# lab-cosmo/torch-pme

Hardware: AMD Instinct MI355X
Metric: atom-steps/sec (energy+forces) (higher is better)
Workload: dtype f32

## Files before the change

torch-pme_amd/csrc/api.hip:

```cpp
#include <dlfcn.h>

#include <cmath>
#include <cstring>
#include <map>
#include <string>
#include <vector>

#include "host.h"

namespace mipme {

static thread_local char g_error[512] = "";

static thread_local const char* g_last_cosched = "";
void note_cosched_kernel(const char* name) { g_last_cosched = name ? name : ""; }
static thread_local int g_last_slot_fill = 0;
void note_slot_fill(int rider_atoms) { g_last_slot_fill = rider_atoms; }
static thread_local int g_last_cell_riders = 0;
void note_cell_riders(int n) { g_last_cell_riders = n; }
void set_error(const char* fmt, ...) {
  va_list ap;
  va_start(ap, fmt);
  vsnprintf(g_error, sizeof(g_error), fmt, ap);
  va_end(ap);
// ... 572 lines not shown
      qv[u] = i < n ? q[i] : T(0);
    }
#pragma unroll
    for (int u = 0; u < kMatchUnroll; ++u) {
      const double v = fabs(double(qv[u]));
      if (v > best) {
        best = v;
        bi = base + u * stride;
      }
    }
  }
#pragma unroll
  for (int off = 32; off > 0; off >>= 1) {
    const double ov = __shfl_xor(best, off, 64);
    const long long oi = __shfl_xor(bi, off, 64);
    if (ov > best || (ov == best && oi < bi)) { best = ov; bi = oi; }
  }
  if (lane == 0) { s_val[wave] = best; s_idx[wave] = bi; }
  __syncthreads();
  if (threadIdx.x == 0) {
    for (int w = 1; w < int(blockDim.x >> 6); ++w)
      if (s_val[w] > s_val[0] || (s_val[w] == s_val[0] && s_idx[w] < s_idx[0])) { s_val[0] = s_val[w]; s_idx[0] = s_idx[w]; }
  }
  __syncthreads();
  const long long k = s_idx[0];
  const bool usable = s_val[0] > 0.0;
  const T scale = usable ? g[k] / q[k] : T(0);
  const double sd = double(scale);
  const double tol = 8.0 * (sizeof(T) == 4 ? 1.1920929e-7 : 2.220446049250313e-16);
  int bad = (usable && isfinite(sd)) ? 0 : 1;
  for (int64_t base = threadIdx.x; base < n; base += stride * kMatchUnroll) {
    T qv[kMatchUnroll], gv[kMatchUnroll];
#pragma unroll
    for (int u = 0; u < kMatchUnroll; ++u) {
      const int64_t i = base + u * stride;
      qv[u] = i < n ? q[i] : T(0);
      gv[u] = i < n ? g[i] : T(0);
    }
#pragma unroll
    for (int u = 0; u < kMatchUnroll; ++u) {
      const double e = sd * double(qv[u]);
      if (!(fabs(double(gv[u]) - e) <= tol * fabs(e))) bad = 1;
    }
  }
  bad = __any(bad) ? 1 : 0;
  if (lane == 0) s_bad[wave] = bad;
  __syncthreads();
  if (threadIdx.x == 0) {
    int any = 0;
    for (int w = 0; w < int(blockDim.x >> 6); ++w) any |= s_bad[w];
    result[0] = scale;
    result[1] = any ? T(0) : T(1);
    if (host_flag) __hip_atomic_store(host_flag, any ? 0 : 1, __ATOMIC_RELEASE, __HIP_MEMORY_SCOPE_SYSTEM);
  }
}

template <typename T>
__global__ __launch_bounds__(64) void values_equal_kernel(int n, const T* __restrict__ a, const T* __restrict__ b, int* host_flag) {
  bool same = true;
  for (int i = threadIdx.x; i < n; i += 64) same = same && (a[i] == b[i]);
  const bool all = __builtin_amdgcn_ballot_w64(!same) == 0;
  if (threadIdx.x == 0) __hip_atomic_store(host_flag, all ? 1 : 0, __ATOMIC_RELEASE, __HIP_MEMORY_SCOPE_SYSTEM);
}

__device__ __forceinline__ void checksum_words(const uint4 v, unsigned j, unsigned long long& a, unsigned long long& b) {
  constexpr unsigned C1 = 0x9e3779b1u, C2 = 0x85ebca6bu;
  const unsigned k1 = (j + 1u) * C1, k2 = (j + 1u) * C2;
  a += (unsigned long long)v.x * k1 + (unsigned long long)v.y * (k1 + C1) + (unsigned long long)v.z * (k1 + 2u * C1) +
       (unsigned long long)v.w * (k1 + 3u * C1);
  b += (unsigned long long)v.x * k2 + (unsigned long long)v.y * (k2 + C2) + (unsigned long long)v.z * (k2 + 2u * C2) +
       (unsigned long long)v.w * (k2 + 3u * C2);
}

static constexpr int kChecksumBlocks = 256;

__global__ __launch_bounds__(256) void checksum_kernel(const uint4* __restrict__ data, int64_t n_vec, const unsigned* __restrict__ tail,
                                                       int n_tail, unsigned long long* __restrict__ sums,
                                                       const unsigned long long* __restrict__ expect, int* host_flag) {
  unsigned long long a = 0, b = 0;
  const int64_t stride = int64_t(gridDim.x) * blockDim.x;
  int64_t i = int64_t(blockIdx.x) * blockDim.x + threadIdx.x;
  for (; i + 7 * stride < n_vec; i += 8 * stride) {
    uint4 v[8];
#pragma unroll
    for (int u = 0; u < 8; ++u) v[u] = data[i + u * stride];
#pragma unroll
    for (int u = 0; u < 8; ++u) checksum_words(v[u], unsigned(4 * (i + u * stride)), a, b);
  }
  for (; i < n_vec; i += stride) checksum_words(data[i], unsigned(4 * i), a, b);
  if (blockIdx.x == 0 && int(threadIdx.x) < n_tail) {
    const unsigned j = unsigned(4 * n_vec) + threadIdx.x;
    a += (unsigned long long)tail[threadIdx.x] * ((j + 1u) * 0x9e3779b1u);
    b += (unsigned long long)tail[threadIdx.x] * ((j + 1u) * 0x85ebca6bu);
  }
  __shared__ unsigned long long red[4][2];
  __shared__ bool last;
  auto block_sum = [&](unsigned long long& x, unsigned long long& y) {
#pragma unroll
    for (int off = 32; off > 0; off >>= 1) {
      x += __shfl_xor(x, off, 64);
      y += __shfl_xor(y, off, 64);
    }
    __syncthreads();
    if ((threadIdx.x & 63) == 0) {
      red[threadIdx.x >> 6][0] = x;
      red[threadIdx.x >> 6][1] = y;
    }
    __syncthreads();
    x = red[0][0] + red[1][0] + red[2][0] + red[3][0];
    y = red[0][1] + red[1][1] + red[2][1] + red[3][1];
  };
  block_sum(a, b);
  unsigned long long* part = sums + 3;
  if (threadIdx.x == 0) {
    __hip_atomic_store(&part[2 * blockIdx.x], a, __ATOMIC_RELAXED, __HIP_MEMORY_SCOPE_AGENT);
    __hip_atomic_store(&part[2 * blockIdx.x + 1], b, __ATOMIC_RELAXED, __HIP_MEMORY_SCOPE_AGENT);
    last = __hip_atomic_fetch_add(&sums[2], 1ull, __ATOMIC_ACQ_REL, __HIP_MEMORY_SCOPE_AGENT) == (unsigned long long)(gridDim.x - 1);
  }
  __syncthreads();
  if (!last) return;
  unsigned long long ta = 0, tb = 0;
  for (unsigned k = threadIdx.x; k < gridDim.x; k += blockDim.x) {
    ta += __hip_atomic_load(&part[2 * k], __ATOMIC_RELAXED, __HIP_MEMORY_SCOPE_AGENT);
    tb += __hip_atomic_load(&part[2 * k + 1], __ATOMIC_RELAXED, __HIP_MEMORY_SCOPE_AGENT);
  }
  block_sum(ta, tb);
  if (threadIdx.x == 0) {
    const unsigned long long s0 = sums[0] + ta, s1 = sums[1] + tb;
    sums[0] = s0;
    sums[1] = s1;
    sums[2] = 0;
    if (host_flag) {
      const int same = expect && s0 == expect[0] && s1 == expect[1];
      __hip_atomic_store(host_flag, same ? 1 : 0, __ATOMIC_RELEASE, __HIP_MEMORY_SCOPE_SYSTEM);
    }
  }
}

template <typename T>
__global__ __launch_bounds__(256) void energy_select_kernel(int64_t N, const T* __restrict__ verdict, const T* __restrict__ q,
                                                           const T* __restrict__ force, const T* __restrict__ field, T f,
                                                           T* __restrict__ grad_mesh, T* __restrict__ grad_pair) {
  if (verdict[1] != T(1)) return;
  const T s = verdict[0];
  for (int64_t t = int64_t(blockIdx.x) * blockDim.x + threadIdx.x; t < 3 * N; t += int64_t(gridDim.x) * blockDim.x) {
    const T sq = s * q[t / 3];
    if (grad_mesh) grad_mesh[t] = sq * field[t];
    if (grad_pair) grad_pair[t] = sq * f * force[t];
  }
}

template <typename T>
__global__ __launch_bounds__(256) void energy_select_sum_kernel(int64_t N, const T* __restrict__ verdict, const T* __restrict__ q,
                                                               const T* __restrict__ force, const T* __restrict__ field, T f,
                                                               const T* grad_mesh, const T* grad_pair, T* out) {
  const bool match = verdict[1] == T(1);
  const T s = verdict[0];
  for (int64_t t = int64_t(blockIdx.x) * blockDim.x + threadIdx.x; t < 3 * N; t += int64_t(gridDim.x) * blockDim.x)
    out[t] = match ? s * q[t / 3] * (f * force[t] + field[t]) : grad_mesh[t] + grad_pair[t];
}

template <typename T>
__global__ __launch_bounds__(256) void energy_select_contract_kernel(int64_t N, const T* __restrict__ verdict,
                                                                    const T* __restrict__ tail_q, T* grad_q,
                                                                    const T* __restrict__ tail_cell, int cell_off,
                                                                    const T* cell_mesh, const T* cell_pair, T* grad_cell) {
  const bool match = verdict[1] == T(1);
  const T s = verdict[0];
  if (grad_cell && blockIdx.x == 0 && threadIdx.x < 9) {
    const int i = threadIdx.x;
    grad_cell[i] = match ? s * tail_cell[cell_off + i] : cell_mesh[i] + (cell_pair ? cell_pair[i] : T(0));
  }
  if (!grad_q || !match) return;
  const T h = T(0.5) * s;
  for (int64_t t = int64_t(blockIdx.x) * blockDim.x + threadIdx.x; t < N; t += int64_t(gridDim.x) * blockDim.x)
    grad_q[t] = h * tail_q[t];
}

static double axis_length(const mipme_mesh_t* m, int axis) {
  const double* a = m->cell + 3 * axis;
  return std::sqrt(a[0] * a[0] + a[1] * a[1] + a[2] * a[2]);
}

template <typename T>
static int slab_forward_t(hipStream_t st, int axis, const mipme_mesh_t* m, double pref, int64_t N, const void* pos,
                          const void* q, void* moments, void* pot) {
  if (N == 0) return MIPME_OK;
  const int C = m->n_channels;
  const double c0 = pref * 4.0 * 3.14159265358979323846 / m->volume;
  slab_moments_kernel<T><<<1, 1024, 0, st>>>(axis, N, C, (const T*)pos, (const T*)q, (const T*)nullptr, (double*)moments);
  MIPME_LAUNCH_CHECK();
  slab_forward_kernel<T><<<unsigned((N + 255) / 256), 256, 0, st>>>(axis, N, C, c0, axis_length(m, axis), (const T*)pos,
                                                                    (const double*)moments, (T*)pot);
  MIPME_LAUNCH_CHECK();
  return MIPME_OK;
}

template <typename T>
static int slab_backward_t(hipStream_t st, int axis, const mipme_mesh_t* m, double pref, int64_t N, const void* pos,
                           const void* q, const void* g, void* moments, void* grad_pos, void* grad_q, void* grad_cell) {
  if (N == 0) return MIPME_OK;
  const int C = m->n_channels;
  const double c0 = pref * 4.0 * 3.14159265358979323846 / m->volume;
  const double Lz = axis_length(m, axis);
  slab_moments_kernel<T><<<1, 1024, 0, st>>>(axis, N, C, (const T*)pos, (const T*)q, (const T*)g, (double*)moments);
  MIPME_LAUNCH_CHECK();
  if (grad_pos || grad_q) {
    slab_backward_kernel<T><<<unsigned((N + 255) / 256), 256, 0, st>>>(
        axis, N, C, c0, Lz, (const T*)pos, (const T*)q, (const T*)g, (const double*)moments, (T*)grad_pos, (T*)grad_q);
    MIPME_LAUNCH_CHECK();
  }
  if (grad_cell) {
    slab_cell_kernel<T><<<1, 64, 0, st>>>(axis, C, *m, c0, Lz, (const double*)moments, (T*)grad_cell);
    MIPME_LAUNCH_CHECK();
  }
  return MIPME_OK;
}

}

template <typename A>
static int load_args(const A* in, A& out, const char* what) {
  MIPME_REQUIRE(in != nullptr, "%s: NULL argument struct", what);
  MIPME_REQUIRE(in->version == MIPME_ARGS_VERSION, "%s: argument struct version %u, library expects %u", what, in->version,
                unsigned(MIPME_ARGS_VERSION));
  MIPME_REQUIRE(in->size >= 16 && in->size <= 4096, "%s: implausible argument struct size %u", what, in->size);
  memset(&out, 0, sizeof(A));
  memcpy(&out, in, in->size < sizeof(A) ? in->size : sizeof(A));
  return MIPME_OK;
}


using namespace mipme;

static int check_slab(int slab, const mipme_mesh_t* mesh, const mipme_potential_t* pot, bool has_tail, const char* who) {
  if (!slab) return MIPME_OK;
  MIPME_REQUIRE(slab >= 1 && slab <= 3, "%s: slab must be 0 (off) or the non-periodic axis + 1, got %d", who, slab);
  MIPME_REQUIRE(mesh->n_channels == 1, "%s: the slab term of the gather tail serves one channel, the mesh has %d (use "
                "mipme_slab_forward / mipme_slab_backward)", who, int(mesh->n_channels));
  MIPME_REQUIRE(has_tail, "%s: slab rides on the gather tail (out_energy, out_grad_positions); without it use mipme_slab_forward", who);
  MIPME_REQUIRE(pot && (pot->kind == MIPME_COULOMB || pot->exponent == 1), "%s: the slab term exists for 1/r only", who);
  return MIPME_OK;
}

static int md_check(const mipme_md_args_t* in, mipme_md_args_t& a, const char* who) {
  MIPME_REQUIRE(in && in->size >= 16 && in->version == 1, "%s: NULL or unversioned argument struct", who);
  std::memset(&a, 0, sizeof(a));
  std::memcpy(&a, in, std::min<size_t>(in->size, sizeof(a)));
  int rc;
  if ((rc = validate_mesh(a.mesh))) return rc;
  MIPME_REQUIRE(a.dtype == MIPME_F32 || a.dtype == MIPME_F64, "invalid dtype %d", a.dtype);
  MIPME_REQUIRE(a.pot && a.pot->smearing > 0, "Must specify smearing to use a potential with PMECalculator");
  MIPME_REQUIRE(live_supported(a.mesh, a.n_atoms, a.dtype), "%s: mesh / atom count outside the live-bin kernels' range", who);
  MIPME_REQUIRE(a.records && a.atom_bins && a.live_lists, "%s: NULL buffer", who);
  return MIPME_OK;
}

template <typename T>
static int md_step_t(const mipme_md_args_t& a) {
  int rc;
  hipStream_t st = (hipStream_t)a.stream;
  const mipme_mesh_t* m = a.mesh;
  double self_c, bg_c;
  correction_terms(a.pot, self_c, bg_c);
  fft_plan_begin_step(a.plan);
  mipme_sr_job_t job{};
  job.n_atoms = a.n_atoms;
  job.row_ptr = a.row_ptr;
  job.entries_shift = a.words;
  job.entries = a.words;
  job.positions = nullptr;
  job.cell = a.cell;
  job.charges = nullptr;
  job.pot = a.pot;
  job.full_list = 0;
  job.shift_format = a.shift_format;
  job.records = const_cast<void*>(a.records);
  job.out = a.potentials;
  job.force = a.pair_force;
  job.dist_out = nullptr;
  GatherTailHost tail{};
  tail.force = a.pair_force;
  tail.force_scale = 1.0;
  tail.seed = a.grad_seed;
  tail.grad_pos = a.grad_positions;
  tail.energy = a.energy;
  if ((rc = tail_attach_plan_scratch(tail, a.plan))) return rc;
  CellWork cw{};
  if (a.grad_cell) {
    cw = cell_work_layout(m, a.n_atoms, a.cell_work);
    tail.rpart = cw.rpart;
  }
  tail.grad_q = a.grad_charges;
  tail.aux_seed = a.aux_seed;
  tail.live_flags = a.host_flags;
  if (a.slab) {
    tail_attach_slab(tail, m, a.pot, a.slab);
    STAGE(st, "slab_moments", slab_moments_blocks<T>(st, a.n_atoms, (const T*)a.records + (a.slab - 1), 4, (const T*)a.records + 3, 4,
                                                     tail.slab_mom));
  }
  if (a.energy_log && (rc = tail_attach_energy_log(tail, a.energy_log, a.energy_log_cursor, a.energy_log_capacity,
                                                   "energy_log needs energy_log_cursor")))
    return rc;
  STAGE(st, "spread+rspace_forward", live_spread<T>(st, m, a.n_atoms, a.records, a.atom_bins, a.live_lists, a.rho_mesh, &job, a.host_flags,
                                                     a.grad_cell ? cw.cwave : nullptr));
  int64_t n_sr_part = 0;
  const void* sr_part = bins_epart(m, a.n_atoms, a.dtype, a.atom_bins, &n_sr_part);
  const ConvCell cc{a.G_deriv, cw.cwave, cw.n_waves, cw.wbuf, cw.rows, int(cw.n_riders), nullptr, nullptr, nullptr, nullptr};
  STAGE(st, "convolve_xfused", convolve_xfused(a.plan, st, a.rho_mesh, a.G, a.hat_work, a.phi_mesh, a.dc, 0, m, a.pot, nullptr,
                                               const_cast<void*>(tail.epart_k), sr_part, n_sr_part, nullptr, a.nan_flag,
                                               a.grad_cell ? &cc : nullptr));
  STAGE(st, "gather+energy+forces",
        live_gather<T>(st, m, a.n_atoms, a.records, a.atom_bins, a.live_lists, a.phi_mesh, a.dc, self_c, bg_c, a.potentials, nullptr,
                       &tail, a.nan_flag));
  if (a.grad_cell)
    STAGE(st, "cell_finalize",
          cell_tail_finalize_impl<T>(st, m, bg_c, 0.5, cw.n_riders, cw.n_bricks, cw.rows, cw.rpart, a.dc,
                                     a.aux_seed ? a.aux_seed : a.grad_seed, a.grad_cell, &tail));
  return MIPME_OK;
}


template <typename T>
static int scaled_match_wide_t(hipStream_t st, int64_t n, const void* g, const void* q, void* result, void* host_flag, void* work) {
  const int64_t nb = (n + 1024 * kMatchRegs - 1) / (1024 * kMatchRegs);
  MIPME_REQUIRE(nb < (int64_t(1) << 24), "mipme_scaled_match_wide: too many values");
  scaled_match_small_kernel<T, true><<<unsigned(nb), 1024, 0, st>>>(n, (const T*)g, (const T*)q, nullptr, nullptr, (double*)work);
  MIPME_LAUNCH_CHECK();
  scaled_match_combine_kernel<T><<<1, 256, 0, st>>>(int(nb), (const double*)work, (T*)result, (int*)host_flag);
  MIPME_LAUNCH_CHECK();
  return MIPME_OK;
}

extern "C" {

const char* mipme_last_error(void) { return g_error; }
const char* mipme_last_cosched_kernel(void) { return g_last_cosched; }
int mipme_last_slot_fill(void) { return g_last_slot_fill; }
int mipme_last_cell_riders(void) { return g_last_cell_riders; }
int mipme_version(void) { return MIPME_VERSION; }

int mipme_fft_plan_create(int dtype, int nx, int ny, int nz, int batch, mipme_fft_plan** out) {
  return fft_plan_create(dtype, nx, ny, nz, batch, out);
}
int mipme_fft_plan_destroy(mipme_fft_plan* plan) { return fft_plan_destroy(plan); }

int mipme_kfilter_build(void* stream, int dtype, const mipme_mesh_t* mesh, const mipme_potential_t* pot, void* G) {
  int rc = validate_mesh(mesh);
  if (rc) return rc;
  MIPME_REQUIRE(G != nullptr, "G is NULL");
  hipStream_t st = (hipStream_t)stream;
  DT_SWITCH(dtype, kfilter_build_impl<float>(st, mesh, pot, G), kfilter_build_impl<double>(st, mesh, pot, G));
}

int mipme_kfilter_build_deriv(void* stream, int dtype, const mipme_mesh_t* mesh, const mipme_potential_t* pot, void* G_deriv) {
  int rc = validate_mesh(mesh);
  if (rc) return rc;
  MIPME_REQUIRE(G_deriv != nullptr, "G_deriv is NULL");
  hipStream_t st = (hipStream_t)stream;
  DT_SWITCH(dtype, kfilter_deriv_impl<float>(st, mesh, pot, G_deriv), kfilter_deriv_impl<double>(st, mesh, pot, G_deriv));
}

int64_t mipme_cell_tail_work(const mipme_fft_plan* plan, const mipme_mesh_t* mesh, int64_t n_atoms) {
  if (!plan || !mesh || validate_mesh(mesh) || n_atoms < 0) return 0;
  return cell_work_layout(mesh, n_atoms, nullptr).total;
}

int mipme_convolve(mipme_fft_plan* plan, void* stream, const void* mesh_in, const void* G, void* hat_out, void* hat_work,
                   void* mesh_out, void* dc_out) {
  TraceRange _tr("mipme_convolve");
  MIPME_REQUIRE(plan != nullptr, "FFT plan is NULL");
  MIPME_REQUIRE(mesh_in && G && hat_out && hat_work && mesh_out, "NULL buffer passed to mipme_convolve");
  hipStream_t st = (hipStream_t)stream;
  const FftDims d = fft_plan_dims(plan);
  const int64_t Mh = int64_t(d.nx) * d.ny * (d.nz / 2 + 1);
  int rc;
  if ((rc = fft_forward(plan, st, mesh_in, hat_out))) return rc;
  if (d.dtype == MIPME_F32)
    rc = apply_filter_impl<float>(st, Mh, d.batch, hat_out, G, hat_work, dc_out);
  else
    rc = apply_filter_impl<double>(st, Mh, d.batch, hat_out, G, hat_work, dc_out);
  if (rc) return rc;
  return fft_inverse(plan, st, hat_work, mesh_out);
}

int mipme_spread(void* stream, int dtype, const mipme_mesh_t* mesh, int64_t n_atoms, const void* positions,
                 const void* values, void* mesh_out) {
  TraceRange _tr("mipme_spread");
  int rc = validate_mesh(mesh);
  if (rc) return rc;
  MIPME_REQUIRE(n_atoms >= 0 && mesh_out && (n_atoms == 0 || (positions && values)), "NULL buffer passed to mipme_spread");
  hipStream_t st = (hipStream_t)stream;
  DT_SWITCH(dtype, spread_impl<float>(st, mesh, n_atoms, positions, values, 1.0, mesh_out),
            spread_impl<double>(st, mesh, n_atoms, positions, values, 1.0, mesh_out));
}

int mipme_gather(void* stream, int dtype, const mipme_mesh_t* mesh, int64_t n_atoms, const void* positions,
                 const void* mesh_in, void* out) {
  TraceRange _tr("mipme_gather");
  int rc = validate_mesh(mesh);
  if (rc) return rc;
  MIPME_REQUIRE(n_atoms >= 0 && mesh_in && (n_atoms == 0 || (positions && out)), "NULL buffer passed to mipme_gather");
  hipStream_t st = (hipStream_t)stream;
  DT_SWITCH(dtype, gather_impl<float>(st, mesh, n_atoms, positions, mesh_in, out),
            gather_impl<double>(st, mesh, n_atoms, positions, mesh_in, out));
}

int mipme_kspace_forward(const mipme_kspace_forward_args_t* args_in) {
  TraceRange _tr("mipme_kspace_forward");
  mipme_kspace_forward_args_t a;
  int rc = load_args(args_in, a, "mipme_kspace_forward");
  if (rc) return rc;
  if ((rc = validate_mesh(a.mesh))) return rc;
  if ((rc = check_slab(a.slab, a.mesh, a.pot, a.out_energy && a.out_grad_positions, "mipme_kspace_forward"))) return rc;
  if ((rc = check_plan(a.plan, a.dtype, a.mesh))) return rc;
  const mipme_mesh_t* mesh = a.mesh;
  MIPME_REQUIRE(a.pot && a.pot->smearing > 0, "Must specify smearing to use a potential with PMECalculator");
  MIPME_REQUIRE(a.G && a.rho_mesh && a.hat_work && a.phi_mesh && a.dc, "NULL work buffer passed to mipme_kspace_forward");
  MIPME_REQUIRE(a.rho_hat || fft_plan_xfused(a.plan), "rho_hat may only be NULL for plans with a power-of-two nx");
  MIPME_REQUIRE(!a.out_cell_partials || !a.rho_hat, "out_cell_partials is produced by the fused convolution (rho_hat == NULL)");
  MIPME_REQUIRE(!a.out_rho_hat || (!a.rho_hat && mesh->n_channels == 1),
                "out_rho_hat is written by the fused convolution (rho_hat == NULL) of a single-channel mesh");
  MIPME_REQUIRE(a.n_atoms == 0 || (a.positions && a.charges && a.out_lr), "NULL atom buffer passed to mipme_kspace_forward");
  MIPME_REQUIRE(!a.atom_bins || bricks_supported(mesh, a.dtype), "atom bins passed for a mesh the brick kernels do not support");
  MIPME_REQUIRE(!a.out_field || (a.atom_bins && mesh->n_channels == 1), "out_field needs atom bins and a single channel");
  MIPME_REQUIRE(!a.out_records || (a.atom_bins && mesh->n_channels == 1), "out_records needs atom bins and a single channel");
  if (a.sr_job) {
    MIPME_REQUIRE(a.atom_bins && a.out_records && mesh->n_channels == 1 && a.accumulate_out && !a.gather_wait_event,
                  "sr_job needs atom bins, out_records, a single channel and accumulate_out = 1 without a wait event");
    MIPME_REQUIRE(a.sr_job->n_atoms == a.n_atoms && a.sr_job->records == a.out_records && a.sr_job->out == a.out_lr,
                  "sr_job must describe the atoms, records and output of the same call");
    MIPME_REQUIRE(a.sr_job->row_ptr && a.sr_job->entries_shift && a.sr_job->entries && a.sr_job->positions &&
                      a.sr_job->charges && a.sr_job->pot, "NULL buffer in sr_job");
  }
  GatherTailHost tail{}, *tp = nullptr;
  if (a.out_energy || a.out_grad_positions) {
    MIPME_REQUIRE(a.out_energy && a.out_grad_positions && a.sr_job && a.sr_job->force && a.out_field && a.n_atoms > 0,
                  "the gather tail (out_energy, out_grad_positions) needs both outputs, sr_job with force sums and out_field");
    tail.force = a.sr_job->force;
    tail.force_scale = a.sr_job->full_list ? 0.5 : 1.0;
    tail.seed = a.grad_seed;
    tail.grad_pos = a.out_grad_positions;
    tail.energy = a.out_energy;
    MIPME_REQUIRE(!a.rho_hat && mesh->n_channels == 1 && sr_job_fusable(a.sr_job),
                  "the gather tail needs the fused convolution (rho_hat == NULL), one channel and a co-schedulable sr_job");
    if ((rc = tail_attach_plan_scratch(tail, a.plan))) return rc;
    tp = &tail;
  }
  if (a.energy_log && (rc = tail_attach_energy_log(tail, a.energy_log, tp ? a.energy_log_cursor : nullptr, a.energy_log_capacity,
                                                   "energy_log rides on the gather tail (out_energy, out_grad_positions) and "
                                                   "needs energy_log_cursor")))
    return rc;
  if (a.out_grad_charges || a.out_grad_cell) {
    MIPME_REQUIRE(tp, "out_grad_charges / out_grad_cell ride on the gather tail (out_energy, out_grad_positions)");
    MIPME_REQUIRE(!a.out_grad_charges || !a.sr_job->full_list || (a.sr_job->shift_format & MIPME_ROWS_PADDED),
                  "out_grad_charges = 2 s V needs a half list (a full list need not be symmetric)");
    tail.grad_q = a.out_grad_charges;
    tail.aux_seed = a.aux_seed;
    if (a.out_grad_cell) {
      const int p = a.pot->kind == MIPME_COULOMB ? 1 : a.pot->exponent;
      MIPME_REQUIRE(a.G_deriv && a.cell_work, "out_grad_cell needs G_deriv (mipme_kfilter_build_deriv) and cell_work");
      MIPME_REQUIRE((a.sr_job->shift_format & 0xff) == 2 && !a.sr_job->dist_out && (p == 1 || p == 6),
                    "out_grad_cell needs 4-byte entries (shift_format 2), no dist_out, and 1/r or 1/r^6");
      MIPME_REQUIRE(!a.out_cell_partials, "out_grad_cell replaces out_cell_partials");
      tail.rpart = cell_work_layout(mesh, a.n_atoms, a.cell_work).rpart;
      tail.records = a.out_records;
    }
  }
  if (a.slab) {
    tail_attach_slab(tail, mesh, a.pot, a.slab);
    tail.records = a.out_records;
  }
  DT_SWITCH(a.dtype, kspace_forward_t<float>(a, tp), kspace_forward_t<double>(a, tp));
}

int mipme_md_supported(const mipme_mesh_t* mesh, const mipme_potential_t* pot, int64_t n_atoms, int dtype) {
  if (!mesh || !pot || validate_mesh(mesh) || pot->smearing <= 0 || pot->exclusion_radius > 0) return 0;
  const int p = pot->kind == MIPME_COULOMB ? 1 : pot->exponent;
  if (p != 1 && p != 6) return 0;
  if (mesh->nx < 2 || (mesh->nx & (mesh->nx - 1))) return 0;
  return live_supported(mesh, n_atoms, dtype) ? 1 : 0;
}

int64_t mipme_md_lists_ints(const mipme_mesh_t* mesh, int64_t n_atoms) {
  if (!mesh || validate_mesh(mesh) || n_atoms <= 0) return 0;
  return live_lists_ints(mesh, n_atoms);
}

int mipme_md_rebin(const mipme_md_args_t* args_in) {
  TraceRange _tr("mipme_md_rebin");
  mipme_md_args_t a;
  int rc = md_check(args_in, a, "mipme_md_rebin");
  if (rc) return rc;
  hipStream_t st = (hipStream_t)a.stream;
  DT_SWITCH(a.dtype, live_rebin<float>(st, a.mesh, a.n_atoms, a.records, a.atom_bins, a.live_lists, a.host_flags),
            live_rebin<double>(st, a.mesh, a.n_atoms, a.records, a.atom_bins, a.live_lists, a.host_flags));
}

int mipme_md_step(const mipme_md_args_t* args_in) {
  TraceRange _tr("mipme_md_step");
  mipme_md_args_t a;
  int rc = md_check(args_in, a, "mipme_md_step");
  if (rc) return rc;
  if ((rc = check_plan(a.plan, a.dtype, a.mesh))) return rc;
  MIPME_REQUIRE(fft_plan_xfused(a.plan), "mipme_md_step needs a plan with a power-of-two nx");
  MIPME_REQUIRE(mipme_md_supported(a.mesh, a.pot, a.n_atoms, a.dtype), "mipme_md_step: potential / mesh outside its range");
  MIPME_REQUIRE(a.cell && a.G && a.rho_mesh && a.hat_work && a.phi_mesh && a.dc && a.row_ptr && a.words && a.potentials &&
                    a.pair_force && a.energy && a.grad_positions, "NULL buffer passed to mipme_md_step");
  MIPME_REQUIRE((a.shift_format & 0xff) == 2, "mipme_md_step reads 4-byte entries (shift_format 2, with or without MIPME_ROWS_PADDED)");
  if ((rc = check_slab(a.slab, a.mesh, a.pot, true, "mipme_md_step"))) return rc;
  if (a.grad_cell) {
    const int p = a.pot->kind == MIPME_COULOMB ? 1 : a.pot->exponent;
    MIPME_REQUIRE(a.G_deriv && a.cell_work, "grad_cell needs G_deriv (mipme_kfilter_build_deriv) and cell_work");
    MIPME_REQUIRE(p == 1 || p == 6, "grad_cell: the pair kernels form the cell sums for 1/r and 1/r^6");
  }
  DT_SWITCH(a.dtype, md_step_t<float>(a), md_step_t<double>(a));
}

int mipme_kspace_backward(const mipme_kspace_backward_args_t* args_in) {
  TraceRange _tr("mipme_kspace_backward");
  mipme_kspace_backward_args_t a;
  int rc = load_args(args_in, a, "mipme_kspace_backward");
  if (rc) return rc;
  if ((rc = validate_mesh(a.mesh))) return rc;
  if ((rc = check_plan(a.plan, a.dtype, a.mesh))) return rc;
  MIPME_REQUIRE(a.pot && a.pot->smearing > 0, "Must specify smearing to use a potential with PMECalculator");
  MIPME_REQUIRE(a.G && a.phi_mesh && (a.grad_scale || (a.psi_mesh && a.hat_work && a.chi_mesh && a.dc)),
                "NULL work buffer passed to mipme_kspace_backward");
  MIPME_REQUIRE(a.grad_scale || a.psi_hat || ((!a.grad_cell || a.G_deriv) && fft_plan_xfused(a.plan)),
                "psi_hat may only be NULL for plans with a power-of-two nx, and with a cell gradient only together with G_deriv");
  MIPME_REQUIRE(a.n_atoms == 0 || (a.positions && a.charges && a.grad_out), "NULL atom buffer passed to mipme_kspace_backward");
  MIPME_REQUIRE(!a.atom_bins || bricks_supported(a.mesh, a.dtype), "atom bins passed for a mesh the brick kernels do not support");
  DT_SWITCH(a.dtype, kspace_backward_t<float>(a), kspace_backward_t<double>(a));
}

int mipme_fft_plan_xfused(const mipme_fft_plan* plan) { return plan && fft_plan_xfused(plan) ? 1 : 0; }

int64_t mipme_fft_plan_kgrid_blocks(const mipme_fft_plan* plan) { return plan ? xconv_blocks(plan) : 0; }

int mipme_fft_r2c(mipme_fft_plan* plan, void* stream, int dtype, const mipme_mesh_t* mesh, const void* mesh_in, void* hat) {
  int rc = validate_mesh(mesh);
  if (rc) return rc;
  if ((rc = check_plan(plan, dtype, mesh))) return rc;
  MIPME_REQUIRE(mesh_in && hat, "NULL buffer passed to mipme_fft_r2c");
  return fft_forward(plan, (hipStream_t)stream, mesh_in, hat);
}

int mipme_plane_spread_parts(const mipme_mesh_t* mesh, int64_t n_atoms, int dtype) {
  if (!mesh || validate_mesh(mesh) || !bricks_supported(mesh, dtype)) return 0;
  if (mesh->nx < 2 || (mesh->nx & (mesh->nx - 1)) || plane_bins_capacity(mesh, n_atoms, dtype) <= 0) return 0;
  return plane_bands(mesh, dtype) > 1 ? 1 : plane_spread_parts_setting();
}

int64_t mipme_atom_bins_bytes(const mipme_mesh_t* mesh, int64_t n_atoms, int dtype) {
  if (!mesh || n_atoms < 0) return 0;
  return bins_bytes(mesh, n_atoms, dtype);
}

int mipme_profile_enable(int on) {
  for (auto& e : g_prof) {
    (void)hipEventDestroy(e.a);
    (void)hipEventDestroy(e.b);
  }
  g_prof.clear();
  g_prof_on = on != 0;
  return MIPME_OK;
}

int64_t mipme_profile_report(char* buf, int64_t buflen) {
  std::map<std::string, std::pair<long, double>> agg;
  for (auto& e : g_prof) {
    float ms = 0.f;
    if (hipEventSynchronize(e.b) == hipSuccess && hipEventElapsedTime(&ms, e.a, e.b) == hipSuccess) {
      auto& a = agg[e.name];
      a.first += 1;
      a.second += ms / float(e.reps > 0 ? e.reps : 1);
    }
  }
  std::string out;
  char line[256];
  for (auto& kv : agg) {
    snprintf(line, sizeof(line), "%s %ld %.6f\n", kv.first.c_str(), kv.second.first, kv.second.second);
    out += line;
  }
  if (buf && buflen > 0) {
    const size_t n = out.size() < size_t(buflen - 1) ? out.size() : size_t(buflen - 1);
    memcpy(buf, out.data(), n);
    buf[n] = 0;
  }
  return int64_t(out.size());
}

int64_t mipme_cellgrad_partials_size(const mipme_mesh_t* mesh, int64_t n_atoms) {
  (void)n_atoms;
  if (!mesh) return 0;
  const int64_t xmax = int64_t(mesh->ny) * (mesh->nz / 2 + 1) * mesh->n_channels;
  const int64_t Mh = int64_t(mesh->nx) * mesh->ny * (mesh->nz / 2 + 1);
  const int64_t fused = 37 * 256 + Mh;
  return std::max<int64_t>(12 * std::max<int64_t>(cellgrad_blocks(mesh), xmax), fused) + cellgrad_scratch_doubles();
}

int mipme_slab_forward(void* stream, int dtype, int axis, const mipme_mesh_t* mesh, double prefactor, int64_t n_atoms,
                       const void* positions, const void* charges, void* moments, void* pot) {
  MIPME_REQUIRE(mesh && axis >= 0 && axis < 3 && moments, "invalid arguments to mipme_slab_forward");
  hipStream_t st = (hipStream_t)stream;
  DT_SWITCH(dtype, slab_forward_t<float>(st, axis, mesh, prefactor, n_atoms, positions, charges, moments, pot),
            slab_forward_t<double>(st, axis, mesh, prefactor, n_atoms, positions, charges, moments, pot));
}
// ... 282 lines not shown
```

torch-pme_amd/csrc/bricks_device.h:

```cpp
#ifndef MIPME_BRICKS_DEVICE_H
#define MIPME_BRICKS_DEVICE_H
#include <algorithm>
#include <cmath>
#include <cstdlib>

#include <rocprim/device/device_radix_sort.hpp>

#include "host.h"
#include <map>
#include <utility>

#include "rows_body.h"
#include "fft_lds.h"

namespace mipme {

static constexpr int BRICK = 8;
static constexpr int BRICK_PTS = BRICK * BRICK * BRICK;

#define MIPME_SGPR_CAP __attribute__((amdgpu_num_sgpr(80)))
static inline int spread_stage_rows(int order, size_t real_bytes);
static inline size_t spread_row_reals(int, size_t) { return 3 * BRICK; }

struct BrickGeom {
// ... 784 lines not shown
            w1[2][t] = wr[N + t];
          }
          const T v = (args.qs ? args.qs[si] : val[int64_t(orig) * C + c]) * scale;
          const int r3[3] = {rz, rx, ry};
#if MIPME_STAGE_SELECT
#pragma unroll
          for (int ax = 0; ax < 3; ++ax) {
#pragma unroll
            for (int k = 0; k < BRICK; ++k) {
              T w = T(0);
#pragma unroll
              for (int t = 0; t < N; ++t) w = (k - r3[ax] == t) ? w1[ax][t] : w;
              dst[ax * BRICK + k] = ax == 1 ? w * v : w;
            }
          }
#else
#pragma unroll
          for (int k = 0; k < SW; ++k) dst[k] = T(0);
#pragma unroll
          for (int ax = 0; ax < 3; ++ax) {
#pragma unroll
            for (int t = 0; t < N; ++t) {
              const int k = r3[ax] + t;
              if (unsigned(k) < unsigned(BRICK)) dst[ax * BRICK + k] = ax == 1 ? w1[ax][t] * v : w1[ax][t];
            }
          }
#endif
        } else if (PAD_ROWS && tid < nst + PAD_ROWS) {
          T* dst = stage + tid * SW;
#pragma unroll
          for (int k = 0; k < SW; ++k) dst[k] = T(0);
        }
        __syncthreads();
        MIPME_WG_PHASE(3);
        constexpr int UC = MIPME_SPREAD_UC;
        const int nstc = __builtin_amdgcn_readfirstlane(nst);
        const int wave_u = __builtin_amdgcn_readfirstlane(wave);
        for (int sv0 = wave_u; sv0 < nstc; sv0 += WAVES * UC) {
#if MIPME_SPREAD_PADROWS
          T wz[UC][BRICK], fx[UC], fy[UC];
          const T* sw = stage + sv0 * SW;
#pragma unroll
          for (int u = 0; u < UC; ++u) {
            const T* su = sw + u * WAVES * SW;
            fx[u] = su[BRICK + px];
            fy[u] = su[2 * BRICK + py];
            load_row8<T>(su, wz[u]);
          }
#pragma unroll
          for (int u = 0; u < UC; ++u) fma_row8<T>(acc, fx[u] * fy[u], wz[u]);
#else
          T wxy[UC], wz[UC][BRICK], fx[UC], fy[UC];
          bool live[UC];
#pragma unroll
          for (int u = 0; u < UC; ++u) {
            const int sv = sv0 + u * WAVES;
            live[u] = sv < nstc;
            const T* sw = stage + (live[u] ? sv : sv0) * SW;
            fx[u] = sw[BRICK + px];
            fy[u] = sw[2 * BRICK + py];
            load_row8<T>(sw, wz[u]);
          }
#pragma unroll
          for (int u = 0; u < UC; ++u) {
            wxy[u] = live[u] ? fx[u] * fy[u] : T(0);
            fma_row8<T>(acc, wxy[u], wz[u]);
          }
#endif
        }
        __syncthreads();
      }
    }
    MIPME_WG_PHASE(4);
#pragma unroll
    for (int pz = 0; pz < BRICK; ++pz) part[wave * BRICK_PTS + (px * BRICK + py) * BRICK + pz] = acc[pz];
    __syncthreads();
    for (int k = tid; k < BRICK_PTS; k += THREADS) {
      T v = T(0);
#pragma unroll
      for (int w = 0; w < WAVES; ++w) v += part[w * BRICK_PTS + k];
      const int qx = k / (BRICK * BRICK), qy = (k / BRICK) % BRICK, qz = k % BRICK;
      const int gx = ox + qx, gy = oy + qy, gz = oz + qz;
      if (gx < g.nx && gy < g.ny && gz < g.nz) mesh[c * M + gx * plane + int64_t(gy) * g.nz + gz] = v;
    }
    __syncthreads();
    MIPME_WG_PHASE(5);
  }
}

template <int N, typename T>
__global__ __launch_bounds__(SPREAD_THREADS) void spread_brick_kernel(SpreadArgs<T> a) {
  MIPME_SKIP_IF_SET(a.skip);
  const unsigned b = brick_of(a.bg, blockIdx.x);
  if (b < unsigned(a.bg.nb)) spread_brick_body<N, T>(a, b);
}
template <int N, typename T>
__global__ __launch_bounds__(SPREAD_THREADS_SPARSE) void spread_brick_sparse_kernel(SpreadArgs<T> a) {
  MIPME_SKIP_IF_SET(a.skip);
  const unsigned b = brick_of(a.bg, blockIdx.x);
  if (b < unsigned(a.bg.nb)) spread_brick_body<N, T, SPREAD_THREADS_SPARSE>(a, b);
}


static constexpr unsigned kBrickPatternMin = 2048;
struct CoSlot {
  bool brick;
  unsigned slot;
};
__host__ __device__ inline unsigned cosched_periods(unsigned n_pad, unsigned n_rows_pad, unsigned a) {
  const unsigned nb8 = n_pad >> 3, nr8 = n_rows_pad >> 3, need = (nr8 + a - 1) / a;
  return nb8 < need ? nb8 : need;
}
__host__ __device__ inline unsigned cosched_grid(unsigned n_pad, unsigned n_rows_pad, unsigned a) {
  if (a == 0) return n_pad + n_rows_pad;
  const unsigned P = cosched_periods(n_pad, n_rows_pad, a);
  const unsigned left_b = n_pad - 8u * P, rows_done = 8u * a * P;
  return P * 8u * (1u + a) + left_b + (n_rows_pad > rows_done ? n_rows_pad - rows_done : 0u);
}
__device__ __forceinline__ CoSlot cosched_slot(unsigned b, unsigned n_pad, unsigned n_rows_pad, unsigned a) {
  if (a == 0) return CoSlot{b < n_pad, b < n_pad ? b : b - n_pad};
  const unsigned P = cosched_periods(n_pad, n_rows_pad, a), period = 8u * (1u + a);
  if (b < P * period) {
    const unsigned p = b / period, r = b - p * period;
    return r < 8u ? CoSlot{true, 8u * p + r} : CoSlot{false, 8u * a * p + (r - 8u)};
  }
  const unsigned rest = b - P * period;
  return (n_pad >> 3) > P ? CoSlot{true, 8u * P + rest} : CoSlot{false, 8u * a * P + rest};
}

static inline unsigned brick_pattern(const BrickGeom& bg, unsigned n_spread, unsigned n_row_blocks, bool fp32) {
  static const int pattern_env = [] { const char* e = getenv("MIPME_BRICK_PATTERN"); return e ? atoi(e) : -1; }();
  unsigned pattern = 0;
  if (bg.xcd && n_spread > 0) {
    if (pattern_env >= 0)
      pattern = unsigned(pattern_env);
    else if (fp32 && n_spread >= kBrickPatternMin) {
      const double ratio = double(pad8(n_row_blocks)) / double(pad8(n_spread));
      const unsigned a = unsigned(ratio + 0.5);
      if (a >= 1 && std::fabs(ratio - double(a)) <= 0.15 * double(a)) pattern = a;
    }
  }
  return pattern;
}

template <typename T, int PFAST, bool COMPACT, bool CELL, int BS = SPREAD_THREADS>
__device__ __forceinline__ void cosched_row_block(const FusedRowsArgs<T>& ra, unsigned r, char* smem_rows) {
  AtomRecord<T>* tab = reinterpret_cast<AtomRecord<T>*>(smem_rows);
  bool done = false;
  if constexpr (COMPACT && std::is_same<T, float>::value) {
    if (CELL || !ra.dist_out) {
      sr_rows_pk_body<PFAST, BS, CELL>(ra, r, tab);
      done = true;
    }
  }
#if MIPME_ROW_LANES == 16
  if constexpr (COMPACT && std::is_same<T, double>::value && (PFAST == 1 || PFAST == 6)) {
    if (CELL || !ra.dist_out) {
      sr_rows_f64_body<BS, CELL, PFAST>(ra, r, smem_rows);
      done = true;
    }
  }
#endif
  if constexpr (!CELL) {
    if (!done) sr_fused_rows_body<T, kPotForce, false, PFAST, false, true, BS, 0, COMPACT>(ra, r, tab);
  }
}

template <int N, typename T, int PFAST, bool COMPACT, bool CELL>
__device__ __forceinline__ void spread_rows_body(const SpreadArgs<T>& sa, const FusedRowsArgs<T>& ra, unsigned n_spread,
                                                 unsigned pattern) {
  MIPME_WG_STAMP(0);
  const unsigned n_pad = sa.bg.xcd ? pad8(n_spread) : n_spread;
  const unsigned n_row_blocks = unsigned((ra.N + kRowsPerSpreadBlock - 1) / kRowsPerSpreadBlock);
  const unsigned n_rows_pad = sa.bg.xcd ? pad8(n_row_blocks) : n_row_blocks;
  const CoSlot cs = cosched_slot(blockIdx.x, n_pad, n_rows_pad, pattern);
  extern __shared__ __attribute__((aligned(16))) char smem_rows[];
  if (cs.brick) {
    const unsigned b = brick_of(sa.bg, cs.slot);
    if (cs.slot < n_pad && b < n_spread) spread_brick_body<N, T>(sa, b);
  } else if (cs.slot < n_rows_pad) {
    const unsigned r = sa.bg.xcd ? xcd_contiguous(cs.slot, n_row_blocks) : cs.slot;
    if (r < n_row_blocks) cosched_row_block<T, PFAST, COMPACT, CELL>(ra, r, smem_rows);
  }
#ifdef MIPME_WG_TIMELINE
  __syncthreads();
#endif
  MIPME_WG_STAMP(1);
}

template <int N, typename T, int PFAST, bool COMPACT, bool CELL = false>
__global__ __launch_bounds__(SPREAD_THREADS, (sizeof(T) == 4 && COMPACT) ? (CELL ? MIPME_CELL_WAVES : 6) : 1) void spread_rows_kernel(
    SpreadArgs<T> sa, FusedRowsArgs<T> ra, unsigned n_spread, unsigned pattern) {
  spread_rows_body<N, T, PFAST, COMPACT, CELL>(sa, ra, n_spread, pattern);
}
template <int N, typename T, int PFAST, bool COMPACT, bool CELL = false>
__global__ __launch_bounds__(SPREAD_THREADS, (sizeof(T) == 4 && COMPACT) ? (CELL ? MIPME_CELL_WAVES : 6) : 1) MIPME_SGPR_CAP void spread_rows_capped_kernel(
    SpreadArgs<T> sa, FusedRowsArgs<T> ra, unsigned n_spread, unsigned pattern) {
  spread_rows_body<N, T, PFAST, COMPACT, CELL>(sa, ra, n_spread, pattern);
}
template <int N, typename T, bool CELL>
constexpr bool spread_rows_sgpr_capped() {
#ifdef MIPME_SGPR_CAP_OFF
  return false;
#else
  return sizeof(T) == 4 && N == 5 && !CELL;
#endif
}

template <typename T, int PFAST, bool COMPACT, bool CELL = false>
__global__ __launch_bounds__(256) void rows_only_kernel(FusedRowsArgs<T> ra, int xcd) {
  constexpr bool F64_BODY = COMPACT && std::is_same<T, double>::value && (PFAST == 1 || PFAST == 6) && kRowLanes == 16;
  __shared__ __attribute__((aligned(16))) char tab_raw[F64_BODY ? kRowsF64LdsBytes : sizeof(AtomRecord<T>) * kShiftTableSize];
  AtomRecord<T>* tab = reinterpret_cast<AtomRecord<T>*>(tab_raw);
  constexpr int BS = 256;
  const unsigned n_row_blocks = unsigned((ra.N + BS / kRowLanes - 1) / (BS / kRowLanes));
  const unsigned r = xcd ? xcd_contiguous(blockIdx.x, n_row_blocks) : blockIdx.x;
  if (r >= n_row_blocks) return;
  if constexpr (COMPACT && std::is_same<T, float>::value) {
    if (CELL || !ra.dist_out) {
      sr_rows_pk_body<PFAST, BS, CELL>(ra, r, tab);
      return;
    }
  }
#if MIPME_ROW_LANES == 16
  if constexpr (F64_BODY) {
    if (CELL || !ra.dist_out) {
      sr_rows_f64_body<BS, CELL, PFAST>(ra, r, tab_raw);
      return;
    }
  }
#endif
  if constexpr (!CELL) sr_fused_rows_body<T, kPotForce, false, PFAST, false, true, BS, 0, COMPACT>(ra, r, tab);
}

template <typename T>
static inline bool rows_cell_supported(int pfast, int shift_format, const void* dist_out) {
  if ((shift_format & kShiftFormatMask) != kShiftTable32 || dist_out || kRowLanes != 16) return false;
  return pfast == 1 || pfast == 6;
}

template <typename T>
struct PlaneArgs {
  Cplx<T>* hat = nullptr;
  int logny = 0, loglz = 0;
  int tile_off = 0, tw_off = 0;
  int misc_off = 0;
  int parts = 1;
  Cplx<T>* hat_more = nullptr;
  int64_t more_stride = 0;
  int band_rows = 0, bands = 1;
};

static constexpr size_t kPlaneLdsCosched = 39 * 1024;
static inline size_t plane_tile_bytes(int ny, int nz, size_t real_bytes) { return 2 * real_bytes * size_t(ny) * (size_t(nz / 2) + 1); }
static inline size_t plane_tw_bytes(int ny, int nz, size_t real_bytes) {
  const size_t Lz = size_t(nz / 2), Ltab = size_t(ny) > Lz ? size_t(ny) : Lz;
  return 2 * real_bytes * (Ltab / 2 + (Lz + 1));
}
template <typename T>
static inline void plane_lds_layout(int rows, int nz, PlaneArgs<T>& pa, size_t& total, bool ystage = true) {
  const size_t acc = sizeof(double) * size_t(rows) * nz, tile = plane_tile_bytes(rows, nz, sizeof(T));
  const size_t tile_off = sizeof(T) == 4 ? 0 : acc;
  const size_t tw_off = sizeof(T) == 4 ? (acc > tile ? acc : tile) : acc + tile;
  pa.tile_off = int(tile_off);
  pa.tw_off = int(tw_off);
  pa.misc_off = int(tw_off + plane_tw_bytes(ystage ? rows : 0, nz, sizeof(T)));
  total = size_t(pa.misc_off) + 640;
}
static inline int plane_band_rows(const mipme_mesh_t* m, int dtype) {
  static const bool bands_env = env_flag("MIPME_PLANE_BANDS", true);
  for (int rows = m->ny; rows >= 4 && rows * kPlaneSub >= m->ny; rows >>= 1) {
    size_t need = 0;
    if (dtype == MIPME_F32) {
      PlaneArgs<float> pa;
      plane_lds_layout<float>(rows, m->nz, pa, need, rows == m->ny);
    } else {
      PlaneArgs<double> pa;
      plane_lds_layout<double>(rows, m->nz, pa, need, rows == m->ny);
    }
    if (need <= kPlaneLdsCosched) return rows;
    if (!bands_env) break;
  }
  return 0;
}
static inline bool plane_fits_cosched(const mipme_mesh_t* m, int dtype) { return plane_band_rows(m, dtype) == m->ny; }

static inline bool sparse_bricks(int64_t n_atoms, int nb);
static int plane_list_capacity(const mipme_mesh_t* m, int64_t N, int dtype) {
  static const bool plane_env = env_flag("MIPME_PLANE_SPREAD", true);
  if (!plane_env || deterministic_mode() || m->n_channels != 1 || N <= 0) return 0;
  const bool pow2 = (m->ny & (m->ny - 1)) == 0 && (m->nz & (m->nz - 1)) == 0 && m->nz >= 4 && m->ny >= 2;
  if (!pow2 || m->nx < 2 * BRICK) return 0;
  if (m->nx > (1 << 11) || m->ny > (1 << kPlanePackBits) || m->nz > (1 << kPlanePackBits)) return 0;
  if (sparse_bricks(N, make_brick_geom(m).nb)) return 0;
  const int band_rows = plane_band_rows(m, dtype);
  if (band_rows == 0) return 0;
  if (band_rows < m->ny && m->ny / kPlaneSub < 8) return 0;
  const int64_t lists = int64_t(m->nx) * kPlaneSub, mean = (N + lists - 1) / lists, all = (N + 15) / 16 * 16;
  int64_t cap = (4 * mean + 32 + 15) / 16 * 16;
  if (cap > all) cap = all;
  return int(cap);
}

template <int N, typename T>
struct PlaneItem {
  T vx;
  int my, mz;
  T wy[N], wz[N];
};

template <int N, typename T>
struct PlaneRaw {
  T w[plane_entry_words<N, T>()];
};

template <int N, typename T>
__device__ __forceinline__ void plane_raw_load(PlaneRaw<N, T>& r, bool ok, const T* __restrict__ base, int64_t idx) {
  constexpr int EW = plane_entry_words<N, T>(), V = 16 / int(sizeof(T));
  struct alignas(16) Chunk {
    T e[V];
  };
  const Chunk* src = reinterpret_cast<const Chunk*>(base + (ok ? idx : 0) * EW);
#pragma unroll
  for (int k = 0; k < EW / V; ++k) {
    const Chunk c = src[k];
#pragma unroll
    for (int u = 0; u < V; ++u) r.w[k * V + u] = c.e[u];
  }
  if constexpr (!plane_entry_fat<N, T>()) {
#pragma unroll
    for (int t = 3; t < EW; ++t) r.w[t] = ok ? r.w[t] : T(0);
  }
}
template <typename T>
__device__ __forceinline__ int plane_raw_packed(T w0) {
  if constexpr (sizeof(T) == 4)
    return __float_as_int(w0);
  else
    return int(__double_as_longlong(w0));
}

template <int SCHEME, int N, typename T>
__device__ __forceinline__ void plane_item_make(PlaneItem<N, T>& it, const PlaneRaw<N, T>& r, int tt, T scale) {
  constexpr bool FAT = plane_entry_fat<N, T>();
  const int packed = plane_raw_packed(r.w[0]);
  it.my = (packed >> kPlanePackBits) & ((1 << kPlanePackBits) - 1);
  it.mz = packed & ((1 << kPlanePackBits) - 1);
  T qwx[N];
#pragma unroll
  for (int t = 0; t < N; ++t) qwx[t] = r.w[(FAT ? 1 : 3) + t];
  it.vx = pick<N, T>(qwx, tt) * scale;
  if constexpr (FAT) {
#pragma unroll
    for (int t = 0; t < N; ++t) {
      it.wy[t] = r.w[1 + N + t];
      it.wz[t] = r.w[1 + 2 * N + t];
    }
  } else {
    T unused[N];
    weights_1d<SCHEME, N, false, T>(r.w[1], it.wy, unused);
    weights_1d<SCHEME, N, false, T>(r.w[2], it.wz, unused);
  }
}

static constexpr unsigned kFxMagicHi = 0x43380000u;
template <int N, typename T, bool BANDED>
__device__ __forceinline__ void plane_item_scatter(double* __restrict__ acc, const Geom& g, const PlaneItem<N, T>& it, double fx_scale,
                                                   int row_lo, int rows) {
  constexpr int s0 = stencil_start<N>();
  int zo[N];
#pragma unroll
  for (int k = 0; k < N; ++k) zo[k] = wrap1(it.mz + s0 + k, g.nz);
#pragma unroll
  for (int j = 0; j < N; ++j) {
    int r = wrap1(it.my + s0 + j, g.ny);
    if constexpr (BANDED) {
      r -= row_lo;
      if (unsigned(r) >= unsigned(rows)) continue;
    }
    const int row = r * g.nz;
    const T ay = it.vx * it.wy[j];
#pragma unroll
    for (int k = 0; k < N; ++k) {
      if constexpr (sizeof(T) == 4) {
        const double t = __builtin_fma(double(ay * it.wz[k]), fx_scale, 6755399441055744.0);
        const unsigned long long bits = (unsigned long long)__double_as_longlong(t) - ((unsigned long long)kFxMagicHi << 32);
        atomicAdd(reinterpret_cast<unsigned long long*>(&acc[row + zo[k]]), bits);
      } else {
        atomicAdd(&acc[row + zo[k]], double(ay * it.wz[k]));
      }
    }
  }
}

template <int SCHEME, int N, typename T, bool BANDED = false>
__device__ __forceinline__ void plane_spread_yz_body(const SpreadArgs<T>& args, const PlaneArgs<T>& pa, unsigned item,
                                                     char* smem) {
  constexpr bool banded = BANDED;
  const int n_bands = banded ? pa.bands : 1;
  const unsigned unit = item / unsigned(pa.parts);
  const int part = int(item - unit * unsigned(pa.parts));
  const unsigned plane = banded ? unit / unsigned(n_bands) : unit;
  const int band = banded ? int(unit - plane * unsigned(n_bands)) : 0;
  const Geom& g = args.g;
  const int rows = banded ? pa.band_rows : g.ny, row_lo = band * rows;
  const BinIndex& bins = args.bins;
  const T* __restrict__ plist = (const T*)bins.plist;
  const T* __restrict__ pover = (const T*)bins.pover;
  const int tid = threadIdx.x, nthr = blockDim.x;
  constexpr int s0 = stencil_start<N>();
  MIPME_WG_PHASE(0);
  double* acc = reinterpret_cast<double*>(smem);
  const int npts = rows * g.nz;
  const int x0 = int(plane);
  const int spb = kPlaneSub / n_bands;
  const int SUBS = banded ? min(spb + 2, kPlaneSub) : kPlaneSub;
  const int sub0 = banded ? band * spb - 1 : 0;
  const int NL = N * SUBS;
  auto list_of = [&](int l) __attribute__((always_inline)) {
    return posmod(x0 - s0 - l / SUBS, g.nx) * kPlaneSub + ((sub0 + (l % SUBS)) & (kPlaneSub - 1));
  };
  int my_count = 0;
  if (tid < NL) my_count = bins.plive[list_of(tid)];
  float my_wmax = 0.f;
  if (sizeof(T) == 4 && tid < bins.n_wmax) my_wmax = bins.wmax[tid];
  for (int i = tid; i < npts; i += nthr) acc[i] = 0.0;
  const YzTile<T> yt = banded ? yz_tile_setup<T, false>(rows, g.nz, smem + pa.tile_off, smem + pa.tw_off)
                              : yz_tile_setup<T, true>(g.ny, g.nz, smem + pa.tile_off, smem + pa.tw_off);
  if (args.from_live) {
    const int n_items = g.nx * n_bands * pa.parts;
    for (int b = int(item) + tid * n_items; b <= bins.nb; b += n_items * nthr) bins.snap[b] = bin_count_of(bins, b, true);
  }
  int* lst = reinterpret_cast<int*>(smem + pa.misc_off);
  static_assert(N * kPlaneSub < 64, "bookkeeping of the plane lists");
  double* fxs = reinterpret_cast<double*>(lst + 128);
  float* wred = reinterpret_cast<float*>(lst + 132);
  if constexpr (sizeof(T) == 4) {
    float a = my_wmax;
    bool bad = !(my_wmax == my_wmax);
    for (int i = tid + nthr; i < bins.n_wmax; i += nthr) {
      const float w = bins.wmax[i];
      bad |= !(w == w);
      a = fmaxf(a, w);
    }
    a = fmaxf(a, dpp_mov<0xB1>(a));
    a = fmaxf(a, dpp_mov<0x4E>(a));
    a = fmaxf(a, dpp_mov<0x141>(a));
    a = fmaxf(a, dpp_mov<0x140>(a));
    a = fmaxf(fmaxf(read_lane(a, 0), read_lane(a, 16)), fmaxf(read_lane(a, 32), read_lane(a, 48)));
    if (__builtin_amdgcn_ballot_w64(bad) != 0) a = __builtin_nanf("");
    if ((tid & 63) == 0) wred[tid >> 6] = a;
  }
  if (tid < NL) lst[64 + tid] = min(my_count, bins.pcap);
  __syncthreads();
  if (tid <= NL) {
    int run = 0;
    for (int u = 0; u < tid; ++u) run += lst[64 + u];
    lst[tid] = run;
  }
  if constexpr (sizeof(T) == 4) {
    if (tid == 64) {
      float qmax = 0.f;
      bool bad = false;
      for (int w = 0; w < (nthr >> 6); ++w) {
        bad |= !(wred[w] == wred[w]);
        qmax = fmaxf(qmax, wred[w]);
      }
      int n_atoms = bins.plive[g.nx * kPlaneSub] + 1;
      for (int u = 0; u < NL; ++u) n_atoms += lst[64 + u];
      int e = 0;
      const double bd = double(qmax) * 1.00001 * fabs(double(args.scale)) * double(n_atoms);
      (void)frexp(bd, &e);
      const bool finite = !bad && bd == bd && bd < 1e300;
      fxs[0] = finite ? ldexp(1.0, 50 - e) : __builtin_nan("");
      fxs[1] = finite ? ldexp(1.0, e - 50) : __builtin_nan("");
    }
  }
  __syncthreads();
  MIPME_WG_PHASE(1);
  const double fx_scale = sizeof(T) == 4 ? fxs[0] : 1.0;
  auto guard_item = [&](const PlaneItem<N, T>& it) __attribute__((always_inline)) {
    if constexpr (sizeof(T) == 4) {
      const T chk = it.vx * it.wy[0] * it.wz[0];
      if (!(__builtin_fabsf(chk) <= 3.0e38f)) fxs[1] = __builtin_nan("");
    }
  };
  const int total = lst[NL];
  const int lo = int(int64_t(total) * part / pa.parts), hi = int(int64_t(total) * (part + 1) / pa.parts);
  const int n_batches = (hi - lo + nthr - 1) / nthr;
  constexpr bool FAT = plane_entry_fat<N, T>();
  const int lane = tid & 63;
  const int lst_lane = lane <= NL ? lst[lane] : 0x7fffffff;
  auto entry_of = [&](int b, int& tt) __attribute__((always_inline)) -> int64_t {
    const int gidx = lo + b * nthr + tid;
    const int g0 = __builtin_amdgcn_readfirstlane(gidx);
    const int l0 = __builtin_popcountll(__builtin_amdgcn_ballot_w64(lane >= 1 && lane < NL && lst_lane <= g0));
    int l = l0, first = __builtin_amdgcn_readlane(lst_lane, l0);
    for (int u = l0 + 1; u < NL; ++u) {
      const int bnd = __builtin_amdgcn_readlane(lst_lane, u);
      if (bnd > g0 + 63) break;
      l += gidx >= bnd ? 1 : 0;
      first = gidx >= bnd ? bnd : first;
    }
    tt = l / SUBS;
    if (b >= n_batches || gidx >= hi) {
      if constexpr (FAT) tt = -1;
      return -1;
    }
    return int64_t(list_of(l)) * bins.pcap + (gidx - first);
  };
  constexpr int DEPTH = FAT ? 1 : 2;
  int tt0 = 0, tt1 = 0;
  PlaneRaw<N, T> r0, r1;
  {
    const int64_t e0 = entry_of(0, tt0);
    plane_raw_load<N, T>(r0, e0 >= 0, plist, e0);
    if constexpr (DEPTH == 2) {
      const int64_t e1 = entry_of(1, tt1);
      plane_raw_load<N, T>(r1, e1 >= 0, plist, e1);
    }
  }
  for (int b = 0; b < n_batches; ++b) {
    int ttn = 0;
    const int64_t en = entry_of(b + DEPTH, ttn);
    PlaneRaw<N, T> rn;
    plane_raw_load<N, T>(rn, en >= 0, plist, en);
    PlaneItem<N, T> cur;
    plane_item_make<SCHEME, N, T>(cur, r0, tt0, args.scale);
    if (cur.vx != T(0)) {
      guard_item(cur);
      plane_item_scatter<N, T, BANDED>(acc, g, cur, fx_scale, row_lo, rows);
    }
    if constexpr (DEPTH == 2) {
      r0 = r1;
      tt0 = tt1;
      r1 = rn;
      tt1 = ttn;
    } else {
      r0 = rn;
      tt0 = ttn;
    }
  }
  if (part == 0) {
    const int oc = bins.plive[g.nx * kPlaneSub];
    for (int i = tid; i < oc; i += nthr) {
      PlaneRaw<N, T> r;
      plane_raw_load<N, T>(r, true, pover, i);
      int d = x0 - (plane_raw_packed(r.w[0]) >> (2 * kPlanePackBits)) - s0;
      d += d < 0 ? g.nx : 0;
      d -= d >= g.nx ? g.nx : 0;
      if (d < N) {
        PlaneItem<N, T> it;
        plane_item_make<SCHEME, N, T>(it, r, d, args.scale);
        guard_item(it);
        plane_item_scatter<N, T, BANDED>(acc, g, it, fx_scale, row_lo, rows);
      }
    }
  }
  __syncthreads();
  MIPME_WG_PHASE(2);
  const double fx_inv = sizeof(T) == 4 ? fxs[1] : 1.0;
  {
    const int Lz = yt.Lz, RZ = yt.RZ, npairs = rows * Lz;
    constexpr int CH = 4;
    for (int base = 0; base < npairs; base += CH * nthr) {
      Cplx<T> v[CH];
#pragma unroll
      for (int u = 0; u < CH; ++u) {
        const int idx = base + u * nthr + tid;
        if constexpr (sizeof(T) == 4) {
          const long long* ai = reinterpret_cast<const long long*>(acc);
          v[u] = idx < npairs ? Cplx<T>{T(double(ai[2 * idx]) * fx_inv), T(double(ai[2 * idx + 1]) * fx_inv)} : Cplx<T>{T(0), T(0)};
        } else {
          v[u] = idx < npairs ? Cplx<T>{T(acc[2 * idx]), T(acc[2 * idx + 1])} : Cplx<T>{T(0), T(0)};
        }
      }
      __syncthreads();
#pragma unroll
      for (int u = 0; u < CH; ++u) {
        const int idx = base + u * nthr + tid;
        if (idx < npairs) {
          const int y = idx / Lz, j = idx - y * Lz;
          const int jr = pa.loglz ? int(__brev(unsigned(j)) >> (32 - pa.loglz)) : 0;
          yt.tile[y * RZ + jr] = v[u];
        }
      }
      __syncthreads();
    }
  }
  MIPME_WG_PHASE(3);
  Cplx<T>* dst = part == 0 ? pa.hat : pa.hat_more + int64_t(part - 1) * pa.more_stride;
  if (banded)
    yz_forward_finish<T, false>(yt, rows, g.nz, 0, pa.loglz, dst + (int64_t(plane) * g.ny + row_lo) * yt.RZ);
  else
    yz_forward_finish<T, true>(yt, g.ny, g.nz, pa.logny, pa.loglz, dst + int64_t(plane) * g.ny * yt.RZ);
  MIPME_WG_PHASE(4);
}

template <int SCHEME, int N, typename T, bool BANDED = false>
__global__ __launch_bounds__(1024) void plane_spread_kernel(SpreadArgs<T> sa, PlaneArgs<T> pa) {
  MIPME_SKIP_IF_SET(sa.skip);
  extern __shared__ __attribute__((aligned(16))) char smem_plane[];
  plane_spread_yz_body<SCHEME, N, T, BANDED>(sa, pa, blockIdx.x, smem_plane);
}

template <int SCHEME, int N, typename T, int PFAST, bool COMPACT, bool CELL, bool BANDED>
__device__ __forceinline__ void plane_rows_body(const SpreadArgs<T>& sa, const PlaneArgs<T>& pa, const FusedRowsArgs<T>& ra,
                                                unsigned n_planes, unsigned n_row_blocks) {
  MIPME_WG_STAMP(0);
  extern __shared__ __attribute__((aligned(16))) char smem_pr[];
  const unsigned n_pad = pad8(n_planes);
  if (blockIdx.x < n_pad) {
    const unsigned p = xcd_contiguous(blockIdx.x, n_planes);
    if (p < n_planes) plane_spread_yz_body<SCHEME, N, T, BANDED>(sa, pa, p, smem_pr);
  } else {
    const unsigned r = xcd_contiguous(blockIdx.x - n_pad, n_row_blocks);
    if (r < n_row_blocks) cosched_row_block<T, PFAST, COMPACT, CELL>(ra, r, smem_pr);
  }
#ifdef MIPME_WG_TIMELINE
  __syncthreads();
#endif
  MIPME_WG_STAMP(1);
}
template <int SCHEME, int N, typename T, int PFAST, bool COMPACT, bool CELL = false, bool BANDED = false>
__global__ __launch_bounds__(SPREAD_THREADS, (sizeof(T) == 4 && COMPACT) ? (CELL ? MIPME_CELL_WAVES : 6) : 1) void plane_rows_kernel(
    SpreadArgs<T> sa, PlaneArgs<T> pa, FusedRowsArgs<T> ra, unsigned n_planes ,
    unsigned n_row_blocks) {
  plane_rows_body<SCHEME, N, T, PFAST, COMPACT, CELL, BANDED>(sa, pa, ra, n_planes, n_row_blocks);
}
template <int SCHEME, int N, typename T, int PFAST, bool COMPACT, bool CELL = false, bool BANDED = false>
__global__ __launch_bounds__(SPREAD_THREADS, (sizeof(T) == 4 && COMPACT) ? (CELL ? MIPME_CELL_WAVES : 6) : 1) MIPME_SGPR_CAP void plane_rows_capped_kernel(
    SpreadArgs<T> sa, PlaneArgs<T> pa, FusedRowsArgs<T> ra, unsigned n_planes, unsigned n_row_blocks) {
  plane_rows_body<SCHEME, N, T, PFAST, COMPACT, CELL, BANDED>(sa, pa, ra, n_planes, n_row_blocks);
}

static constexpr int GATHER_THREADS = 512;

static constexpr int GATHER_THREADS_SPARSE = 128;
static constexpr int kSparseBrickAtoms = 40;
static constexpr int kSparseMinBricks = 4096;
static inline bool sparse_bricks(int64_t n_atoms, int nb) {
  static const bool force = env_flag("MIPME_SPARSE_FORCE", false);
  return force || (n_atoms <= int64_t(kSparseBrickAtoms) * nb && nb >= kSparseMinBricks);
}

template <int N, int NT, typename T, int THREADS = GATHER_THREADS>
__device__ __forceinline__ void load_tiles(const Geom& g, int ox, int oy, int oz, const T* __restrict__ m0,
                                           const T* __restrict__ m1, T* tile) {
  constexpr int TL = BRICK + N - 1;
  constexpr int s0 = stencil_start<N>();
  const int64_t plane = int64_t(g.ny) * g.nz;
  for (int k = threadIdx.x; k < TL * TL * TL; k += THREADS) {
    const int tx = k / (TL * TL), ty = (k / TL) % TL, tz = k % TL;
    const int gx = wrap1(ox + s0 + tx, g.nx), gy = wrap1(oy + s0 + ty, g.ny), gz = wrap1(oz + s0 + tz, g.nz);
    const int64_t gi = gx * plane + int64_t(gy) * g.nz + gz;
    tile[k] = m0[gi];
    if constexpr (NT == 2) tile[TL * TL * TL + k] = m1[gi];
  }
}

static constexpr int kGatherLanes = 8;

template <typename T>
struct GatherTail {
  const T* force;
  T force_scale;
  const T* seed;
  T* grad_pos;
  T* energy;
  const double* epart_sr;
  const double* epart_k;
  int n_sr, n_k;
  T* grad_q;
  double* rpart;
  const AtomRecord<T>* rec4;
  const T* aux_seed;
  const int* live_flags;
  double* elog = nullptr;
  int* elog_cursor = nullptr;
  int elog_cap = 0, elog_stride = 1;
  const double* slab_mom = nullptr;
  double slab_c0 = 0.0, slab_L = 0.0;
  int slab_axis = 0;
};
template <typename T>
__device__ __forceinline__ T slab_coord(const AtomRecord<T>& r, int axis) {
  return axis == 0 ? r.x : (axis == 1 ? r.y : r.z);
}
template <typename T>
static GatherTail<T> make_gather_tail(const GatherTailHost& th, const double* epart_sr, int n_sr, const void* rec4,
                                      const void* live_flags) {
  GatherTail<T> tail;
  tail.force = (const T*)th.force;
  tail.force_scale = T(th.force_scale);
  tail.seed = (const T*)th.seed;
  tail.grad_pos = (T*)th.grad_pos;
  tail.energy = (T*)th.energy;
  tail.epart_sr = epart_sr;
  tail.n_sr = n_sr;
  tail.epart_k = (const double*)th.epart_k;
  tail.n_k = int(th.n_k);
  tail.grad_q = (T*)th.grad_q;
  tail.rpart = th.rpart;
  tail.rec4 = (const AtomRecord<T>*)rec4;
  tail.aux_seed = (const T*)th.aux_seed;
  tail.live_flags = (const int*)live_flags;
  tail.elog = th.elog;
  tail.elog_cursor = th.elog_cursor;
  tail.elog_cap = th.elog_cap;
  if (th.slab) {
    tail.slab_mom = th.slab_mom;
    tail.slab_c0 = th.slab_c0;
    tail.slab_L = th.slab_L;
    tail.slab_axis = th.slab - 1;
  }
  return tail;
}

template <int THREADS>
__device__ __forceinline__ void tail_rpart(double (&r3)[3], double* __restrict__ rpart, unsigned block) {
  __shared__ double rred[THREADS / 64][9];
  const int lane = threadIdx.x & 63, wave = threadIdx.x >> 6;
#pragma unroll
  for (int c = 0; c < 3; ++c) {
    double v = r3[c];
    v += __shfl_xor(v, 8, 64);
    v += __shfl_xor(v, 16, 64);
    v += __shfl_xor(v, 32, 64);
    if (lane < 3) rred[wave][3 * c + lane] = v;
  }
  __syncthreads();
  if (threadIdx.x < 9) {
    double v = 0.0;
    for (int w = 0; w < THREADS / 64; ++w) v += rred[w][threadIdx.x];
    rpart[9 * int64_t(block) + threadIdx.x] = v;
  }
}

template <typename T, int THREADS, bool SLAB = false>
__device__ __forceinline__ void tail_energy(const GatherTail<T>& tail, const T* __restrict__ qsum, T inv_vol, T self_c,
                                            T bg_c) {
  __shared__ double tred[THREADS / 64][3];
  double v[3] = {0.0, 0.0, 0.0};
  for (int i = threadIdx.x; i < tail.n_sr; i += THREADS) {
    v[0] += tail.epart_sr[2 * i];
    v[1] += tail.epart_sr[2 * i + 1];
  }
  for (int i = threadIdx.x; i < tail.n_k; i += THREADS) v[2] += tail.epart_k[i];
  const int lane = threadIdx.x & 63, wave = threadIdx.x >> 6;
#pragma unroll
  for (int k = 0; k < 3; ++k) {
    double x = v[k];
#pragma unroll
    for (int off = 32; off > 0; off >>= 1) x += __shfl_xor(x, off, 64);
    if (lane == 0) tred[wave][k] = x;
  }
  __syncthreads();
  if (threadIdx.x == 0) {
    double t[3] = {0.0, 0.0, 0.0};
    for (int w = 0; w < THREADS / 64; ++w)
      for (int k = 0; k < 3; ++k) t[k] += tred[w][k];
    const double Q = double(qsum[0]);
    double e = t[0] + 0.5 * double(inv_vol) * t[2] - 0.5 * double(self_c) * t[1] - double(bg_c) * double(inv_vol) * Q * Q;
    if constexpr (SLAB) {
      const double sQ = tail.slab_mom[0], sM = tail.slab_mom[1], sM2 = tail.slab_mom[2];
      e += 0.5 * tail.slab_c0 * (sM * sM - sQ * sM2 - sQ * sQ * tail.slab_L * tail.slab_L / 12.0);
    }
    if (tail.live_flags && (__hip_atomic_load(tail.live_flags, __ATOMIC_RELAXED, __HIP_MEMORY_SCOPE_SYSTEM) & 2)) e = __builtin_nan("");
    tail.energy[0] = T(e);
    if (tail.elog) {
      const int k = tail.elog_cursor[0];
      tail.elog[int64_t(unsigned(k) % unsigned(tail.elog_cap)) * tail.elog_stride] = double(T(e));
      tail.elog_cursor[0] = k + 1;
    }
  }
}

template <int N, bool FIELD, typename T, bool TAIL = false, int THREADS = GATHER_THREADS, bool SLAB = false>
__device__ __forceinline__ void gather_brick_body(const Geom& g, const BrickGeom& bg, int C, const BinIndex& bins,
                                                  const int4* __restrict__ rec, const T* __restrict__ wts,
                                                  const T* __restrict__ mesh, const T* __restrict__ q,
                                                  const T* __restrict__ qsum, T inv_vol, T self_c, T bg_c, bool accumulate,
                                                  T* __restrict__ out, T* __restrict__ raw, T* __restrict__ field,
                                                  unsigned block, const GatherTail<T>* tail = nullptr,
                                                  int* __restrict__ nan_flag = nullptr) {
  static_assert(N <= kGatherLanes, "one lane per z point of the stencil");
  static_assert(!TAIL || FIELD, "the tail needs the mesh field");
  static_assert(!SLAB || TAIL, "the slab term rides in the tail");
  constexpr int LANES = kGatherLanes;
  constexpr int GROUPS = THREADS / LANES;
  constexpr int TL = BRICK + N - 1;
  __shared__ T tile[TL * TL * TL];
  int bx, by, bz;
  brick_coords(bg, block, bx, by, bz);
  const int ox = bx * BRICK, oy = by * BRICK, oz = bz * BRICK;
  const int beg = int(block) * bins.cap, end = beg + bins.snap[block];
  const int n_over = bins.snap[bins.nb];
  if (bins.live && threadIdx.x == 0) {
    bins.live[block] = 0;
    if (block == 0) bins.live[bins.nb] = 0;
    if (bins.plive) {
      for (int i = int(block); i <= g.nx * kPlaneSub; i += bins.nb) bins.plive[i] = 0;
    }
  }
  T seed = T(1), seed_aux = T(1);
  if constexpr (TAIL) {
    if (tail->seed) seed = tail->seed[0];
    seed_aux = tail->aux_seed ? tail->aux_seed[0] : seed;
    if (block == 0) tail_energy<T, THREADS, SLAB>(*tail, qsum, inv_vol, self_c, bg_c);
  }
  T fA = T(0), fB = T(0), pA = T(0), pB = T(0), pK = T(0);
  if constexpr (SLAB) {
    const double sQ = tail->slab_mom[0], sM = tail->slab_mom[1], sM2 = tail->slab_mom[2], c0 = tail->slab_c0;
    fA = T(c0 * sM);
    fB = T(c0 * sQ);
    pA = T(0.5 * c0 * sM);
    pB = T(0.25 * c0 * sQ);
    pK = T(-0.5 * c0 * (0.5 * sM2 + sQ * tail->slab_L * tail->slab_L / 12.0));
  }
  double r3[3] = {0.0, 0.0, 0.0};
  if (beg == end && n_over == 0) {
    if constexpr (TAIL) {
      if (tail->rpart && threadIdx.x < 9) tail->rpart[9 * int64_t(block) + threadIdx.x] = 0.0;
    }
    return;
  }
  const int main_iters = (end - beg + GROUPS - 1) / GROUPS, over_iters = (n_over + GROUPS - 1) / GROUPS;
  const int64_t M = int64_t(g.nx) * g.ny * g.nz;
  const int l = threadIdx.x % LANES, grp = threadIdx.x / LANES;
  const bool lane_active = l < N;
  const int tz = lane_active ? l : 0;
  for (int c = 0; c < C; ++c) {
    if (c > 0) __syncthreads();
    bool staged = false;
    for (int it = 0; it < main_iters + over_iters; ++it) {
      bool valid;
      int id;
      if (it < main_iters) {
        const int idx = beg + it * GROUPS + grp;
        valid = idx < end;
        id = valid ? idx : beg;
      } else {
        const int k = (it - main_iters) * GROUPS + grp;
        valid = k < n_over && bins.over_brick[k < n_over ? k : 0] == int(block);
        id = int(bins.over_base) + (k < n_over ? k : 0);
      }
      int4 a = rec[id];
      if (!valid) a = make_int4(ox, oy, oz, 0);
      const T* wr = wts + int64_t(id) * wts_stride<N, T>();
      T wx[N], wy[N], dwx[FIELD ? N : 1], dwy[FIELD ? N : 1];
#pragma unroll
      for (int t = 0; t < N; ++t) {
        wx[t] = wr[t];
        wy[t] = wr[N + t];
        if constexpr (FIELD) {
          dwx[t] = wr[3 * N + t];
          dwy[t] = wr[4 * N + t];
        }
      }
      const T wzv = lane_active ? wr[2 * N + tz] : T(0);
// ... 298 lines not shown
```

torch-pme_amd/csrc/host.h:

```cpp
#pragma once

#include <algorithm>
#include <climits>
#include <cmath>

#include "common.h"

namespace mipme {

template <typename T>
constexpr int dtype_of() {
  return sizeof(T) == 4 ? MIPME_F32 : MIPME_F64;
}

#define DT_SWITCH(dtype, CALL_F32, CALL_F64)                    \
  do {                                                          \
    if ((dtype) == MIPME_F32) return CALL_F32;                  \
    if ((dtype) == MIPME_F64) return CALL_F64;                  \
    mipme::set_error("invalid dtype %d", int(dtype));           \
    return MIPME_EINVAL;                                        \
  } while (0)

inline unsigned stride_grid(int64_t n, int block) {
  return unsigned(std::max<int64_t>(1, std::min<int64_t>((n + block - 1) / block, 2048)));
}

template <typename T> int spread_impl(hipStream_t st, const mipme_mesh_t* m, int64_t n_atoms, const void* pos, const void* val, double scale,
                                      void* mesh);
template <typename T> int gather_impl(hipStream_t st, const mipme_mesh_t* m, int64_t n_atoms, const void* pos, const void* mesh, void* out);
template <typename T> int gather_epilogue_impl(hipStream_t st, const mipme_mesh_t* m, int64_t n_atoms, const void* pos, const void* mesh,
                                               const void* q, const void* qsum, double self_c, double bg_c, void* out, void* raw,
                                               int accumulate, void* nan_flag);
template <typename T> int gather_grad_impl(hipStream_t st, const mipme_mesh_t* m, int64_t n_atoms, const void* pos, const void* q,
                                           const void* gout, const void* phi, const void* chi, const void* gsum_dc, const void* gscale,
                                           double self_c, double bg_c, void* grad_pos, void* grad_q);

struct FftDims { int dtype, nx, ny, nz, batch; };
int fft_plan_create(int dtype, int nx, int ny, int nz, int batch, mipme_fft_plan** out);
int fft_plan_destroy(mipme_fft_plan* p);
FftDims fft_plan_dims(const mipme_fft_plan* p);
int fft_plan_batch(const mipme_fft_plan* p);
bool fft_plan_xfused(const mipme_fft_plan* p);
int* fft_plan_brick_count(const mipme_fft_plan* p);
int fft_forward(mipme_fft_plan* p, hipStream_t st, const void* in, void* out);
int fft_inverse(mipme_fft_plan* p, hipStream_t st, void* in, void* out);
int64_t xconv_blocks(const mipme_fft_plan* p);
int convolve_xfused(mipme_fft_plan* p, hipStream_t st, const void* mesh_in, const void* G, void* hat, void* mesh_out,
                    void* dc, int64_t G_stride, const mipme_mesh_t* cell_mesh, const mipme_potential_t* cell_pot,
                    void* cell_partials, void* epart, const void* sr_part, int64_t n_sr_part, const RowRideHost* rh,
                    void* err_flag, const ConvCell* cc);
void fft_plan_begin_step(mipme_fft_plan* p);
bool fft_plan_plane_forward_ok(const mipme_fft_plan* p);
bool fft_plan_plane_forward_ok_batched(const mipme_fft_plan* p);
void fft_plan_set_forward_done(mipme_fft_plan* p, bool done, int parts);
void fft_plan_set_forward_ycols(mipme_fft_plan* p, bool pending);
void* fft_plan_hat_parts(mipme_fft_plan* p, hipStream_t st, int n_more);
int fft_plan_tail_scratch(mipme_fft_plan* p, int64_t bytes, void** out);
template <typename T> int kfilter_build_impl(hipStream_t st, const mipme_mesh_t* m, const mipme_potential_t* pot, void* G);
template <typename T> int kfilter_deriv_impl(hipStream_t st, const mipme_mesh_t* m, const mipme_potential_t* pot, void* D);
template <typename T> int apply_filter_impl(hipStream_t st, int64_t Mh, int C, const void* hat, const void* G, void* out, void* dc);
template <typename T> int apply_filter_cellgrad_impl(hipStream_t st, const mipme_mesh_t* m, const mipme_potential_t* pot, const void* psi_hat,
                                                     const void* rho_hat, const void* G, void* out, void* dc, void* partials);
int64_t cellgrad_blocks(const mipme_mesh_t* m);
int64_t cellgrad_scratch_doubles();
template <typename T> int cellgrad_finalize_impl(hipStream_t st, const mipme_mesh_t* m, double bg, int64_t n_atoms, void* partials,
                                                 const void* pos, const void* grad_pos, const void* gout, const void* phi_atoms,
                                                 const void* rho_dc, const void* psi_dc, const void* energy_scale, void* grad_cell,
                                                 int64_t kgrid_blocks, const void* field, const void* q);
template <typename T> int cell_tail_finalize_impl(hipStream_t st, const mipme_mesh_t* m, double bg, double pair_scale, int64_t n_rows,
                                                  int64_t n_bricks, const void* rows, const void* rpart, const void* dc, const void* seed, void* out,
                                                  const GatherTailHost* slab = nullptr);

template <typename T, typename I> int rspace_forward_impl(hipStream_t st, int64_t P, int64_t N, int C, const void* pairs, const void* dist, const void* q,
                                                          const void* mask, int full, const mipme_potential_t* pot, int accumulate, void* out);
template <typename T, typename I> int rspace_backward_impl(hipStream_t st, int64_t P, int64_t N, int C, const void* pairs, const void* dist,
                                                           const void* q, const void* mask, int full, const mipme_potential_t* pot, const void* g,
                                                           const void* gscale, void* grad_d, void* grad_q);
template <typename T, typename I> int distance_forward_impl(hipStream_t st, int64_t P, const void* pairs, const void* pos, const void* cell,
                                                            const void* shifts, void* out);
template <typename T, typename I> int distance_backward_impl(hipStream_t st, int64_t P, int64_t N, const void* pairs, const void* pos, const void* cell,
                                                             const void* shifts, const void* grad_d, void* partials, void* grad_pos, void* grad_cell);
template <typename T> int pack_pair_shifts_impl(hipStream_t st, int64_t P, const void* shifts, void* packed, void* flag);
template <typename T> int distance_forward_packed_impl(hipStream_t st, int64_t P, const void* pairs, const void* packed, const void* pos,
                                                       const void* cell, void* out);
int64_t pair_partials_blocks(int64_t P);

bool bricks_supported(const mipme_mesh_t* m, int dtype);
int64_t bins_bytes(const mipme_mesh_t* m, int64_t N, int dtype);
int plane_bins_capacity(const mipme_mesh_t* m, int64_t N, int dtype);
int plane_bands(const mipme_mesh_t* m, int dtype);
const void* bins_epart(const mipme_mesh_t* m, int64_t N, int dtype, void* bins, int64_t* n);
bool sr_job_fusable(const mipme_sr_job_t* job);
template <typename T> int bins_build(hipStream_t st, const mipme_mesh_t* m, int64_t n_atoms, const void* pos, void* bins, int* live,
                                     const void* q, void* atom_rec, bool plane_lists = false, bool defer_slots = false);
bool plane_spread_runs(const mipme_mesh_t* m, int64_t N, int dtype, const mipme_sr_job_t* job, const PlaneHost* ph, bool forward);
bool bins_defer_slots(const mipme_mesh_t* m, int64_t N, int dtype, const mipme_sr_job_t* job, const PlaneHost* ph);
SlotRider bins_slot_rider(const mipme_mesh_t* m, int64_t N, int dtype, void* bins, const void* pos, const void* q);
template <typename T> int spread_bricks(hipStream_t st, const mipme_mesh_t* m, int64_t N, void* bins, const void* val, double scale, void* mesh,
                                        int* clear_count, const mipme_sr_job_t* job, bool want_epart, double* cpart, const PlaneHost* ph = nullptr,
                                        bool* used_planes = nullptr);
template <typename T> int gather_bricks(hipStream_t st, const mipme_mesh_t* m, int64_t N, void* bins, const void* mesh, const void* q,
                                        const void* qsum, double self_c, double bg_c, void* out, void* raw, int accumulate, void* field,
                                        const GatherTailHost* th, void* nan_flag, int* live);
template <typename T> int gather_grad_bricks(hipStream_t st, const mipme_mesh_t* m, int64_t N, void* bins, const void* q, const void* gout,
                                             const void* phi, const void* chi, const void* psi_dc, const void* gscale, double self_c,
                                             double bg_c, void* grad_pos, void* grad_q);

bool live_supported(const mipme_mesh_t* m, int64_t N, int dtype);
int64_t live_lists_ints(const mipme_mesh_t* m, int64_t N);
template <typename T> int live_rebin(hipStream_t st, const mipme_mesh_t* m, int64_t N, const void* rec4, void* bins, void* lists, void* host_flags);
template <typename T> int live_spread(hipStream_t st, const mipme_mesh_t* m, int64_t N, const void* rec4, void* bins, void* lists, void* mesh,
                                      const mipme_sr_job_t* job, void* host_flags, double* cpart);
template <typename T> int live_gather(hipStream_t st, const mipme_mesh_t* m, int64_t N, const void* rec4, void* bins, void* lists, const void* mesh,
                                      const void* qsum, double self_c, double bg_c, void* out, void* field, const GatherTailHost* th, void* nan_flag);

inline void correction_terms(const mipme_potential_t* pot, double& self_c, double& bg_c) {
  const int p = pot->kind == MIPME_COULOMB ? 1 : pot->exponent;
  const double two_s2 = 2.0 * pot->smearing * pot->smearing;
  self_c = pot->prefactor / std::tgamma(0.5 * p + 1.0) / std::pow(two_s2, 0.5 * p);
  if (p >= 3)
    bg_c = 0.0;
  else
    bg_c = pot->prefactor * std::pow(3.14159265358979323846, 1.5) * std::pow(two_s2, 0.5 * (3 - p)) /
           ((3 - p) * std::tgamma(0.5 * p));
}

static constexpr int kPlanePartsMax = 8;
inline int plane_spread_parts_setting() {
  static const int parts_env = [] { const char* e = getenv("MIPME_PLANE_PARTS"); return e ? atoi(e) : 2; }();
  return parts_env < 1 ? 1 : (parts_env > kPlanePartsMax ? kPlanePartsMax : parts_env);
}

inline int tail_attach_plan_scratch(GatherTailHost& tail, mipme_fft_plan* plan) {
  void* scratch = nullptr;
  tail.n_k = xconv_blocks(plan);
  tail.sr_reduced = 1;
  const int rc = fft_plan_tail_scratch(plan, int64_t(sizeof(double)) * (3 * tail.n_k + kSlabWork), &scratch);
  tail.epart_k = scratch;
  tail.slab_mom = scratch ? (double*)scratch + 3 * tail.n_k : nullptr;
  return rc;
}

inline void tail_attach_slab(GatherTailHost& tail, const mipme_mesh_t* m, const mipme_potential_t* pot, int slab) {
  const double* a = m->cell + 3 * (slab - 1);
  tail.slab = slab;
  tail.slab_c0 = pot->prefactor * 4.0 * 3.14159265358979323846 / m->volume;
  tail.slab_L = std::sqrt(a[0] * a[0] + a[1] * a[1] + a[2] * a[2]);
}

inline int tail_attach_energy_log(GatherTailHost& tail, void* log, void* cursor, int64_t capacity, const char* needs) {
  MIPME_REQUIRE(cursor && capacity > 0 && capacity <= INT_MAX, "%s and a capacity > 0 (at most %d)", needs, INT_MAX);
  tail.elog = (double*)log;
  tail.elog_cursor = (int*)cursor;
  tail.elog_cap = int(capacity);
  return MIPME_OK;
}

struct CellWork {
  int64_t n_riders, n_bricks, n_waves;
  double *rows, *rpart, *cwave;
  void* wbuf;
  int64_t total;
};
inline CellWork cell_work_layout(const mipme_mesh_t* m, int64_t N, void* base) {
  CellWork w;
  const int64_t Mh = int64_t(m->nx) * m->ny * (m->nz / 2 + 1);
  w.n_riders = std::min<int64_t>(256, std::max<int64_t>(8, Mh / 2048));
  w.n_bricks = int64_t((m->nx + 7) / 8) * ((m->ny + 7) / 8) * ((m->nz + 7) / 8);
  w.n_waves = (N + 3) / 4;
  double* b = (double*)base;
  w.rows = b;
  w.rpart = w.rows + 25 * w.n_riders;
  w.cwave = w.rpart + 9 * w.n_bricks;
  w.wbuf = w.cwave + 9 * w.n_waves;
  w.total = 25 * w.n_riders + 9 * w.n_bricks + 9 * w.n_waves + Mh;
  return w;
}

struct FrameCellRec {
  mipme_mesh_t mesh;
  double bg, pair_scale;
  const void* wbuf;
  const void* dG4;
  const double* cwave;
  double* rows;
  const double* rpart;
  const void* dc;
  const void* seed;
  void* out;
  int n_waves, n_riders, n_bricks, _pad;
  const double* slab_mom;
  double slab_c0, slab_L;
  int slab_axis, _pad_slab;
};
template <typename T> int frames_cell_riders(hipStream_t st, const FrameCellRec* recs, int n_frames, int n_riders, int nx, int ny,
                                             int nzh, const double* epart_k, int n_k);
template <typename T> int frames_cell_finalize(hipStream_t st, const FrameCellRec* recs, int n_frames);
template <typename T> int frames_slab_cell_finalize(hipStream_t st, const FrameCellRec* recs, int n_frames);

inline int64_t frames_cell_stride(const mipme_mesh_t* m, int64_t N) {
  const CellWork w = cell_work_layout(m, N, nullptr);
  const int64_t rows_per_block = 32, waves_per_block = 8;
  const int64_t waves = (N + rows_per_block - 1) / rows_per_block * waves_per_block;
  return 25 * w.n_riders + 9 * w.n_bricks + 9 * waves + int64_t(m->nx) * m->ny * (m->nz / 2 + 1);
}
inline CellWork frames_cell_layout(const mipme_mesh_t* m, int64_t N, int n_frames, int frame, void* base, int64_t stride,
                                   size_t real_bytes) {
  CellWork w = cell_work_layout(m, N, nullptr);
  const int64_t Mh = int64_t(m->nx) * m->ny * (m->nz / 2 + 1);
  w.wbuf = (char*)base + size_t(frame) * size_t(Mh) * real_bytes;
  w.rows = (double*)base + int64_t(n_frames) * Mh + int64_t(frame) * (stride - Mh);
  w.rpart = w.rows + 25 * w.n_riders;
  w.cwave = w.rpart + 9 * w.n_bricks;
  w.total = stride;
  return w;
}

}
```

torch-pme_amd/csrc/live.hip:

```cpp
#include "bricks_device.h"

namespace mipme {
static constexpr int kLiveMargin = 1;
enum LiveFlags { kLiveListOverflow = 1, kLiveMoved = 2 };

struct LiveLists {
  int* counters;
  int* count;
  int* atoms;
  int lcap;
  int4* rec_now;
  int4* home_rec;
  int* host_flags;
};

static inline int live_list_capacity(const mipme_mesh_t* m, int64_t N) {
  double frac = 1.0;
  const int ns[3] = {m->nx, m->ny, m->nz};
  for (int d = 0; d < 3; ++d) frac *= std::min(1.0, double(BRICK + m->order - 1 + 2 * kLiveMargin) / ns[d]);
  const int64_t want = (int64_t(2.0 * frac * double(N)) + 64 + 63) / 64 * 64;
  const int64_t all = (N + 63) / 64 * 64;
  return int(std::min<int64_t>(want, std::max<int64_t>(all, 64)));
}
static inline int64_t live_slots(const mipme_mesh_t* m, int64_t N) {
  const BrickGeom bg = make_brick_geom(m);
  return int64_t(bg.nb) * bin_capacity(bg.nb, N) + N;
}
int64_t live_lists_ints(const mipme_mesh_t* m, int64_t N) {
  const BrickGeom bg = make_brick_geom(m);
  const int64_t head = ((8 + (bg.nb + 1) + bg.nb + int64_t(bg.nb) * live_list_capacity(m, N)) + 3) / 4 * 4;
  return head + 4 * live_slots(m, N) + 4 * N;
}
static inline LiveLists live_view(const mipme_mesh_t* m, int64_t N, void* lists, void* host_flags) {
  const BrickGeom bg = make_brick_geom(m);
  int* b = (int*)lists;
  LiveLists l;
  l.counters = b + 8;
  l.count = l.counters + (bg.nb + 1);
  l.atoms = l.count + bg.nb;
  l.lcap = live_list_capacity(m, N);
  const int64_t head = ((8 + (bg.nb + 1) + bg.nb + int64_t(bg.nb) * l.lcap) + 3) / 4 * 4;
  l.rec_now = (int4*)(b + head);
  l.home_rec = l.rec_now + live_slots(m, N);
  l.host_flags = (int*)host_flags;
  return l;
}

template <int N, bool DERIV, typename T>
__device__ __forceinline__ void live_axis(int scheme, T x, T (&w)[N], T (&dw)[N]) {
  if constexpr (N <= 2) {
    weights_1d<MIPME_P3M, N, DERIV, T>(x, w, dw);
  } else if constexpr (N >= 6) {
    weights_1d<MIPME_LAGRANGE, N, DERIV, T>(x, w, dw);
  } else {
    if (scheme == MIPME_P3M)
      weights_1d<MIPME_P3M, N, DERIV, T>(x, w, dw);
    else
      weights_1d<MIPME_LAGRANGE, N, DERIV, T>(x, w, dw);
  }
}
template <int N, typename T>
__device__ __forceinline__ void live_coords(const Geom& g, const AtomRecord<T>& r, int& mx, int& my, int& mz, T& x0, T& x1, T& x2) {
  const double rx = double(r.x), ry = double(r.y), rz = double(r.z);
  const double ux = double(g.nx) * (rx * g.inv[0] + ry * g.inv[3] + rz * g.inv[6]);
  const double uy = double(g.ny) * (rx * g.inv[1] + ry * g.inv[4] + rz * g.inv[7]);
  const double uz = double(g.nz) * (rx * g.inv[2] + ry * g.inv[5] + rz * g.inv[8]);
  int m;
  double x;
  split_runtime(ux, (N % 2) == 0, m, x);
  mx = posmod(m, g.nx);
  x0 = T(x);
  split_runtime(uy, (N % 2) == 0, m, x);
  my = posmod(m, g.ny);
  x1 = T(x);
  split_runtime(uz, (N % 2) == 0, m, x);
  mz = posmod(m, g.nz);
  x2 = T(x);
}

template <typename T>
__global__ __launch_bounds__(256) void live_bin_kernel(Geom g, BrickGeom bg, bool even, BinIndex bi, int* __restrict__ counters,
                                                      int64_t Natoms, const AtomRecord<T>* __restrict__ rec4,
                                                      int* __restrict__ over_brick, int4* __restrict__ rec,
                                                      int4* __restrict__ home_rec) {
  const int64_t i = int64_t(blockIdx.x) * blockDim.x + threadIdx.x;
  if (i >= Natoms) return;
  const AtomRecord<T> r = rec4[i];
  const T p3[3] = {r.x, r.y, r.z};
  int m[3];
  double x[3];
  atom_mesh_coords<T>(g, even, p3, 0, m, x);
  const int b = ((m[0] / BRICK) * bg.nby + m[1] / BRICK) * bg.nbz + m[2] / BRICK;
  const int lane = threadIdx.x & 63;
  unsigned long long remaining = __ballot(true);
  int my_leader = lane, my_rank = 0, my_count = 1;
  while (remaining) {
    const int leader = __ffsll((long long)remaining) - 1;
    const int b0 = __shfl(b, leader, 64);
    const unsigned long long peers = __ballot(b == b0) & remaining;
    if (b == b0) {
      my_leader = leader;
      my_rank = __popcll(peers & ((1ull << lane) - 1ull));
      my_count = __popcll(peers);
    }
    remaining &= ~peers;
  }
  int base = 0;
  if (my_leader == lane) base = atomicAdd(&counters[b], my_count);
  base = __shfl(base, my_leader, 64);
  const int slot = base + my_rank;
  int64_t dst;
  if (slot < bi.cap) {
    dst = int64_t(b) * bi.cap + slot;
  } else {
    const int k = atomicAdd(&counters[bi.nb], 1);
    over_brick[k] = b;
    dst = bi.over_base + k;
  }
  rec[dst] = make_int4(m[0], m[1], m[2], int(i));
  home_rec[i] = make_int4(m[0], m[1], m[2], int(dst));
}

__global__ void live_snapshot_kernel(BinIndex bi, int* __restrict__ counters) {
  const int b = blockIdx.x * blockDim.x + threadIdx.x;
  if (b > bi.nb) return;
  const int c = counters[b];
  bi.snap[b] = b == bi.nb ? c : min(c, bi.cap);
  counters[b] = 0;
}

__device__ __forceinline__ bool live_reach(int m, int s0, int origin, int nmesh, int order) {
  const int r = rel_start(m, s0, origin, nmesh, order);
  return r <= BRICK - 1 + kLiveMargin || r >= nmesh - order + 1 - kLiveMargin;
}

template <int N>
__global__ __launch_bounds__(SPREAD_THREADS) void live_lists_kernel(Geom g, BrickGeom bg, BinIndex bins,
                                                                   const int4* __restrict__ rec, LiveLists ll) {
  __shared__ int n_list;
  __shared__ int keys[4096];
  const unsigned block = brick_of(bg, blockIdx.x);
  if (block >= unsigned(bg.nb)) return;
  int bx, by, bz;
  brick_coords(bg, block, bx, by, bz);
  const int ox = bx * BRICK, oy = by * BRICK, oz = bz * BRICK;
  const int tid = threadIdx.x, sub = tid % SPREAD_GROUP, grp = tid / SPREAD_GROUP;
  constexpr int s0 = stencil_start<N>();
  int* __restrict__ out = ll.atoms + int64_t(block) * ll.lcap;
  if (tid == 0) n_list = 0;
  __syncthreads();
  if (grp < 28) {
    int start, len;
    if (grp < 27) {
      const int dx = grp / 9 - 1, dy = (grp / 3) % 3 - 1, dz = grp % 3 - 1;
      const int nbr = (wrap1(bx + dx, bg.nbx) * bg.nby + wrap1(by + dy, bg.nby)) * bg.nbz + wrap1(bz + dz, bg.nbz);
      start = nbr * bins.cap;
      len = bins.snap[nbr];
    } else {
      start = int(bins.over_base);
      len = bins.snap[bins.nb];
    }
    for (int k = sub; k < len; k += SPREAD_GROUP) {
      const int4 a = rec[start + k];
      if (live_reach(a.x, s0, ox, g.nx, N) && live_reach(a.y, s0, oy, g.ny, N) && live_reach(a.z, s0, oz, g.nz, N)) {
        const int dst = atomicAdd(&n_list, 1);
        if (dst < ll.lcap) out[dst] = a.w;
      }
    }
  }
  __syncthreads();
  const int n = n_list;
  if (n > ll.lcap) {
    if (tid == 0) {
      ll.count[block] = ll.lcap;
      if (ll.host_flags) atomicOr(ll.host_flags, kLiveListOverflow);
    }
    return;
  }
  if (tid == 0) ll.count[block] = n;
  if (n > 1 && n <= 4096) {
    for (int k = tid; k < n; k += SPREAD_THREADS) keys[k] = out[k];
    __syncthreads();
    for (int k = tid; k < n; k += SPREAD_THREADS) {
      const int me = keys[k];
      int r = 0;
      for (int v = 0; v < n; ++v) r += keys[v] < me;
      out[r] = me;
    }
  }
}

template <typename T>
struct LiveSpreadArgs {
  Geom g;
  BrickGeom bg;
  int scheme;
  const int* count;
  const int* atoms;
  int lcap;
  const AtomRecord<T>* rec4;
  T* mesh;
  int stage_rows;
  int64_t n_atoms;
  const int4* home_rec;
  int4* rec_now;
  T* wts;
  int* host_flags;
};

template <int N, typename T>
__device__ __forceinline__ void live_home_body(const LiveSpreadArgs<T>& args, unsigned wg) {
  const int64_t i = int64_t(wg) * SPREAD_THREADS + threadIdx.x;
  if (i >= args.n_atoms) return;
  const Geom& g = args.g;
  const AtomRecord<T> r = args.rec4[i];
  const int4 was = args.home_rec[i];
  int mx, my, mz;
  T x0, x1, x2;
  live_coords<N, T>(g, r, mx, my, mz, x0, x1, x2);
  T wx[N], wy[N], wz[N], dwx[N], dwy[N], dwz[N];
  live_axis<N, true, T>(args.scheme, x0, wx, dwx);
  live_axis<N, true, T>(args.scheme, x1, wy, dwy);
  live_axis<N, true, T>(args.scheme, x2, wz, dwz);
  auto far = [](int now, int then, int n) {
    int d = now - then;
    d = d > n / 2 ? d - n : (d < -(n / 2) ? d + n : d);
    return d > kLiveMargin || d < -kLiveMargin;
  };
  if ((far(mx, was.x, g.nx) || far(my, was.y, g.ny) || far(mz, was.z, g.nz)) && args.host_flags) atomicOr(args.host_flags, kLiveMoved);
  const int64_t slot = was.w;
  args.rec_now[slot] = make_int4(mx, my, mz, int(i));
  store_slot_weights<N, T>(args.wts + slot * wts_stride<N, T>(), wx, wy, wz, dwx, dwy, dwz);
}

template <int N, typename T>
__device__ __forceinline__ void live_spread_body(const LiveSpreadArgs<T>& args, unsigned block) {
  constexpr int THREADS = SPREAD_THREADS, WAVES = SPREAD_WAVES;
  const Geom& g = args.g;
  const BrickGeom& bg = args.bg;
  const int stage_rows = args.stage_rows;
  extern __shared__ __attribute__((aligned(16))) char smem_raw[];
  constexpr int SW = 3 * BRICK;
  constexpr int PAD_ROWS = MIPME_LIVE_PADROWS ? (MIPME_SPREAD_UC - 1) * WAVES : 0;
  T* stage = reinterpret_cast<T*>(smem_raw);
  T* part = stage;
  int bx, by, bz;
  brick_coords(bg, block, bx, by, bz);
  const int ox = bx * BRICK, oy = by * BRICK, oz = bz * BRICK;
  const int tid = threadIdx.x, lane = tid & 63, wave = tid >> 6;
  const int ns = min(args.count[block], args.lcap);
  const int* __restrict__ latoms = args.atoms + int64_t(block) * args.lcap;
  constexpr int s0 = stencil_start<N>();
  const int px = lane >> 3, py = lane & 7;
  const int64_t plane = int64_t(g.ny) * g.nz;
  T acc[BRICK];
#pragma unroll
  for (int k = 0; k < BRICK; ++k) acc[k] = T(0);
  for (int chunk = 0; chunk < ns; chunk += stage_rows) {
    const int nst = min(stage_rows, ns - chunk);
    if (tid < nst) {
      const int atom = latoms[chunk + tid];
      const AtomRecord<T> r = args.rec4[atom];
      int mx, my, mz;
      T x0, x1, x2;
      live_coords<N, T>(g, r, mx, my, mz, x0, x1, x2);
      T wx[N], wy[N], wz[N], unused[N];
      live_axis<N, false, T>(args.scheme, x0, wx, unused);
      live_axis<N, false, T>(args.scheme, x1, wy, unused);
      live_axis<N, false, T>(args.scheme, x2, wz, unused);
      const int rz = rel_start(mz, s0, oz, g.nz, N), rx = rel_start(mx, s0, ox, g.nx, N), ry = rel_start(my, s0, oy, g.ny, N);
      T* dst = stage + tid * SW;
#pragma unroll
      for (int k = 0; k < SW; ++k) dst[k] = T(0);
#pragma unroll
      for (int t = 0; t < N; ++t) {
        if (unsigned(rz + t) < unsigned(BRICK)) dst[rz + t] = wz[t];
        if (unsigned(rx + t) < unsigned(BRICK)) dst[BRICK + rx + t] = wx[t] * r.w;
        if (unsigned(ry + t) < unsigned(BRICK)) dst[2 * BRICK + ry + t] = wy[t];
      }
    } else if (PAD_ROWS && tid < nst + PAD_ROWS) {
      T* dst = stage + tid * SW;
#pragma unroll
      for (int k = 0; k < SW; ++k) dst[k] = T(0);
    }
    __syncthreads();
    constexpr int UC = MIPME_SPREAD_UC;
    const int nstc = __builtin_amdgcn_readfirstlane(nst);
    const int wave_u = __builtin_amdgcn_readfirstlane(wave);
    for (int sv0 = wave_u; sv0 < nstc; sv0 += WAVES * UC) {
#if MIPME_LIVE_PADROWS
      T wz[UC][BRICK], fx[UC], fy[UC];
      const T* sw = stage + sv0 * SW;
#pragma unroll
      for (int u = 0; u < UC; ++u) {
        const T* su = sw + u * WAVES * SW;
        fx[u] = su[BRICK + px];
        fy[u] = su[2 * BRICK + py];
        load_row8<T>(su, wz[u]);
      }
#pragma unroll
      for (int u = 0; u < UC; ++u) fma_row8<T>(acc, fx[u] * fy[u], wz[u]);
#else
      T wxy[UC], wz[UC][BRICK], fx[UC], fy[UC];
      bool live[UC];
#pragma unroll
      for (int u = 0; u < UC; ++u) {
        const int sv = sv0 + u * WAVES;
        live[u] = sv < nstc;
        const T* sw = stage + (live[u] ? sv : sv0) * SW;
        fx[u] = sw[BRICK + px];
        fy[u] = sw[2 * BRICK + py];
        load_row8<T>(sw, wz[u]);
      }
#pragma unroll
      for (int u = 0; u < UC; ++u) {
        wxy[u] = live[u] ? fx[u] * fy[u] : T(0);
        fma_row8<T>(acc, wxy[u], wz[u]);
      }
#endif
    }
    __syncthreads();
  }
#pragma unroll
  for (int pz = 0; pz < BRICK; ++pz) part[wave * BRICK_PTS + (px * BRICK + py) * BRICK + pz] = acc[pz];
  __syncthreads();
  for (int k = tid; k < BRICK_PTS; k += THREADS) {
    T v = T(0);
#pragma unroll
    for (int w = 0; w < WAVES; ++w) v += part[w * BRICK_PTS + k];
    const int qx = k / (BRICK * BRICK), qy = (k / BRICK) % BRICK, qz = k % BRICK;
    const int gx = ox + qx, gy = oy + qy, gz = oz + qz;
    if (gx < g.nx && gy < g.ny && gz < g.nz) args.mesh[gx * plane + int64_t(gy) * g.nz + gz] = v;
  }
}

__host__ __device__ inline unsigned live_home_blocks(int64_t n_atoms, bool xcd) {
  const unsigned n = unsigned((n_atoms + SPREAD_THREADS - 1) / SPREAD_THREADS);
  return xcd ? (n + 7u) / 8u * 8u : n;
}
template <int N, typename T, int PFAST, bool CELL = false>
__global__ __launch_bounds__(SPREAD_THREADS, sizeof(T) == 4 ? (CELL ? MIPME_CELL_WAVES : 8) : 1) void live_spread_rows_kernel(LiveSpreadArgs<T> sa, FusedRowsArgs<T> ra,
                                                                                        unsigned n_spread, unsigned pattern) {
  const unsigned n_home = live_home_blocks(sa.n_atoms, sa.bg.xcd), n_pad = sa.bg.xcd ? pad8(n_spread) : n_spread;
  const unsigned n_row_blocks = unsigned((ra.N + kRowsPerSpreadBlock - 1) / kRowsPerSpreadBlock);
  const unsigned n_rows_pad = sa.bg.xcd ? pad8(n_row_blocks) : n_row_blocks;
  if (blockIdx.x < n_home) {
    live_home_body<N, T>(sa, blockIdx.x);
    return;
  }
  const CoSlot cs = cosched_slot(blockIdx.x - n_home, n_pad, n_rows_pad, pattern);
  if (cs.brick) {
    const unsigned b = brick_of(sa.bg, cs.slot);
    if (cs.slot < n_pad && b < n_spread) live_spread_body<N, T>(sa, b);
  } else if (cs.slot < n_rows_pad) {
    const unsigned r = sa.bg.xcd ? xcd_contiguous(cs.slot, n_row_blocks) : cs.slot;
    if (r < n_row_blocks) {
      extern __shared__ __attribute__((aligned(16))) char smem_rows[];
      AtomRecord<T>* tab = reinterpret_cast<AtomRecord<T>*>(smem_rows);
      if constexpr (std::is_same<T, float>::value)
        sr_rows_pk_body<PFAST, SPREAD_THREADS, CELL>(ra, r, tab);
#if MIPME_ROW_LANES == 16
      else if constexpr (PFAST == 1 || PFAST == 6)
        sr_rows_f64_body<SPREAD_THREADS, CELL, PFAST>(ra, r, smem_rows);
#endif
      else if constexpr (!CELL)
        sr_fused_rows_body<T, kPotForce, false, PFAST, false, true, SPREAD_THREADS, 0, true>(ra, r, tab);
    }
  }
}

template <int N, typename T, bool SLAB = false>
__global__ __launch_bounds__(GATHER_THREADS, (sizeof(T) == 4 && N <= 5) ? MIPME_GATHER_TAIL_WAVES : 1) void live_gather_tail_kernel(Geom g, BrickGeom bg, BinIndex bins,
                                                                         const int4* __restrict__ rec_now,
                                                                         const T* __restrict__ wts,
                                                                         const AtomRecord<T>* __restrict__ rec4,
                                                                         const T* __restrict__ mesh, const T* __restrict__ qsum,
                                                                         T inv_vol, T self_c, T bg_c, T* __restrict__ out,
                                                                         T* __restrict__ field, GatherTail<T> tail,
                                                                         int* __restrict__ nan_flag) {
  static_assert(N <= kGatherLanes, "one lane per z point of the stencil");
  MIPME_WG_STAMP_GATHER(0);
  constexpr int THREADS = GATHER_THREADS, LANES = kGatherLanes, GROUPS = THREADS / LANES, MG = kLiveMargin;
  constexpr int TL = BRICK + N - 1 + 2 * MG;
  __shared__ T tile[TL * TL * TL];
  const unsigned block = brick_of(bg, blockIdx.x);
  if (block >= unsigned(bg.nb)) return;
  int bx, by, bz;
  brick_coords(bg, block, bx, by, bz);
  const int ox = bx * BRICK, oy = by * BRICK, oz = bz * BRICK;
  const int beg = int(block) * bins.cap, end = beg + bins.snap[block];
  const int n_over = bins.snap[bins.nb];
  T seed = T(1);
  if (tail.seed) seed = tail.seed[0];
  const T seed_aux = tail.aux_seed ? tail.aux_seed[0] : seed;
  if (block == 0) tail_energy<T, THREADS, SLAB>(tail, qsum, inv_vol, self_c, bg_c);
  T fA = T(0), fB = T(0), pA = T(0), pB = T(0), pK = T(0);
  if constexpr (SLAB) {
    const double sQ = tail.slab_mom[0], sM = tail.slab_mom[1], sM2 = tail.slab_mom[2], c0 = tail.slab_c0;
    fA = T(c0 * sM);
    fB = T(c0 * sQ);
    pA = T(0.5 * c0 * sM);
    pB = T(0.25 * c0 * sQ);
    pK = T(-0.5 * c0 * (0.5 * sM2 + sQ * tail.slab_L * tail.slab_L / 12.0));
  }
  double r3[3] = {0.0, 0.0, 0.0};
  if (beg == end && n_over == 0) {
    if (tail.rpart && threadIdx.x < 9) tail.rpart[9 * int64_t(block) + threadIdx.x] = 0.0;
    return;
  }
  const int main_iters = (end - beg + GROUPS - 1) / GROUPS, over_iters = (n_over + GROUPS - 1) / GROUPS;
  const int l = threadIdx.x % LANES, grp = threadIdx.x / LANES;
  const bool lane_active = l < N;
  const int tz = lane_active ? l : 0;
  constexpr int s0 = stencil_start<N>();
  const int64_t plane = int64_t(g.ny) * g.nz;
  bool staged = false;
  for (int it = 0; it < main_iters + over_iters; ++it) {
    bool valid;
    int id;
    if (it < main_iters) {
      const int idx = beg + it * GROUPS + grp;
      valid = idx < end;
      id = valid ? idx : beg;
    } else {
      const int k = (it - main_iters) * GROUPS + grp;
      valid = k < n_over && bins.over_brick[k < n_over ? k : 0] == int(block);
      id = int(bins.over_base) + (k < n_over ? k : 0);
    }
    int4 a = rec_now[id];
    if (!valid) a = make_int4(ox, oy, oz, 0);
    const T* wr = wts + int64_t(id) * wts_stride<N, T>();
    T wx[N], wy[N], dwx[N], dwy[N];
#pragma unroll
    for (int t = 0; t < N; ++t) {
      wx[t] = wr[t];
      wy[t] = wr[N + t];
      dwx[t] = wr[3 * N + t];
      dwy[t] = wr[4 * N + t];
    }
    const T wzv = lane_active ? wr[2 * N + tz] : T(0);
    const T dwzv = lane_active ? wr[5 * N + tz] : T(0);
    if (!staged) {
      for (int k = threadIdx.x; k < TL * TL * TL; k += THREADS) {
        const int tx = k / (TL * TL), ty = (k / TL) % TL, tzz = k % TL;
        const int gx = wrap1(ox + s0 - MG + tx, g.nx), gy = wrap1(oy + s0 - MG + ty, g.ny), gz = wrap1(oz + s0 - MG + tzz, g.nz);
        tile[k] = mesh[gx * plane + int64_t(gy) * g.nz + gz];
      }
      staged = true;
    }
    const AtomRecord<T> r_early = rec4[a.w];
    const T q_early = r_early.w;
    const T out_early = out[a.w];
    const T f_early = tail.force[3 * int64_t(a.w) + (l < 3 ? l : 0)];
    if (it == 0) __syncthreads();
    auto tile_start = [&](int m_now, int n, int o) {
      int d = m_now - o;
      d = d > n / 2 ? d - n : (d < -(n / 2) ? d + n : d);
      d += MG;
      return d < 0 ? 0 : (d > BRICK - 1 + 2 * MG ? BRICK - 1 + 2 * MG : d);
    };
    const int rtx = tile_start(a.x, g.nx, ox), rty = tile_start(a.y, g.ny, oy), rtz = tile_start(a.z, g.nz, oz);
    const T* tp = tile + rty * TL + (rtz + tz);
    T sA = T(0), sB = T(0), sC = T(0);
#pragma unroll
    for (int ty = 0; ty < N; ++ty) {
      T sx = T(0), sdx = T(0);
#pragma unroll
      for (int tx = 0; tx < N; ++tx) {
        const T v = tp[(rtx + tx) * TL * TL + ty * TL];
        sx += v * wx[tx];
        sdx += v * dwx[tx];
      }
      sA += sx * wy[ty];
      sB += sdx * wy[ty];
      sC += sx * dwy[ty];
    }
    const T fx = group_sum_b<LANES, T>(sB * wzv) * T(g.nx) * inv_vol;
    const T fy = group_sum_b<LANES, T>(sC * wzv) * T(g.ny) * inv_vol;
    const T fz = group_sum_b<LANES, T>(sA * dwzv) * T(g.nz) * inv_vol;
    const T i0 = T(l == 1 ? g.inv[3] : (l == 2 ? g.inv[6] : g.inv[0])), i1 = T(l == 1 ? g.inv[4] : (l == 2 ? g.inv[7] : g.inv[1])),
            i2 = T(l == 1 ? g.inv[5] : (l == 2 ? g.inv[8] : g.inv[2]));
    const T fc = i0 * fx + i1 * fy + i2 * fz;
    T fs = fc;
    if constexpr (SLAB) {
      if (l == tail.slab_axis) fs += fA - fB * slab_coord(r_early, tail.slab_axis);
    }
    if (l < 3 && valid) {
      const int64_t o = int64_t(a.w);
      if (field) field[3 * o + l] = fs;
      tail.grad_pos[3 * o + l] = seed * q_early * (tail.force_scale * f_early + fs);
      if (tail.rpart) {
        const double gp = double(seed_aux * q_early * fc);
        r3[0] += double(r_early.x) * gp;
        r3[1] += double(r_early.y) * gp;
        r3[2] += double(r_early.z) * gp;
      }
    }
    const T acc = group_sum_b<LANES, T>(sA * wzv);
    if (l == 0 && valid) {
      const T phi = acc * inv_vol;
      T lr = T(0.5) * (phi - self_c * q_early - T(2) * bg_c * inv_vol * qsum[0]);
      if constexpr (SLAB) {
        const T z = slab_coord(r_early, tail.slab_axis);
        lr += z * (pA - pB * z) + pK;
      }
      out[a.w] = out_early + lr;
      if (tail.grad_q) tail.grad_q[a.w] = T(2) * seed_aux * (out_early + lr);
      if (nan_flag && lr != lr) *nan_flag = 1;
    }
  }
  if (tail.rpart) tail_rpart<THREADS>(r3, tail.rpart, block);
#if MIPME_WG_TIMELINE_GATHER
  __syncthreads();
#endif
  MIPME_WG_STAMP_GATHER(1);
}

#define MIPME_DISPATCH_ORDER(ORDER_V, BODY)                       \
  do {                                                            \
    switch (ORDER_V) {                                            \
      case 1: { constexpr int N = 1; BODY; } break;               \
      case 2: { constexpr int N = 2; BODY; } break;               \
      case 3: { constexpr int N = 3; BODY; } break;               \
      case 4: { constexpr int N = 4; BODY; } break;               \
      case 5: { constexpr int N = 5; BODY; } break;               \
      case 6: { constexpr int N = 6; BODY; } break;               \
      case 7: { constexpr int N = 7; BODY; } break;               \
      default: set_error("unsupported interpolation order %d", int(ORDER_V)); return MIPME_EINVAL; \
    }                                                             \
  } while (0)

bool live_supported(const mipme_mesh_t* m, int64_t N, int dtype) {
  if (!bricks_supported(m, dtype) || m->n_channels != 1 || N <= 0) return false;
  const BrickGeom bg = make_brick_geom(m);
  if (sparse_bricks(N, bg.nb)) return false;
  const size_t s = dtype == MIPME_F32 ? 4 : 8;
  const size_t tl = BRICK + m->order - 1 + 2 * kLiveMargin;
  return tl * tl * tl * s <= 60 * 1024 && live_list_capacity(m, N) >= 1;
}

template <typename T>
int live_rebin(hipStream_t st, const mipme_mesh_t* m, int64_t N, const void* rec4, void* bins, void* lists, void* host_flags) {
  const int dtype = dtype_of<T>();
  MIPME_REQUIRE(live_supported(m, N, dtype), "mesh / atom count outside the live-bin kernels' range");
  const Geom g = make_geom(m);
  const BrickGeom bg = make_brick_geom(m);
  BinsView v = bins_view(m, N, dtype, bins);
  const LiveLists ll = live_view(m, N, lists, host_flags);
  live_bin_kernel<T><<<unsigned((N + 255) / 256), 256, 0, st>>>(g, bg, (m->order % 2) == 0, v.idx, ll.counters, N,
                                                              (const AtomRecord<T>*)rec4, v.over_brick, v.rec, ll.home_rec);
  MIPME_LAUNCH_CHECK();
  live_snapshot_kernel<<<unsigned((bg.nb + 1 + 255) / 256), 256, 0, st>>>(v.idx, ll.counters);
  MIPME_LAUNCH_CHECK();
  MIPME_DISPATCH_ORDER(m->order, (live_lists_kernel<N><<<brick_grid(bg), SPREAD_THREADS, 0, st>>>(g, bg, v.idx, v.rec, ll)));
  MIPME_LAUNCH_CHECK();
  return MIPME_OK;
}

template <typename T>
int live_spread(hipStream_t st, const mipme_mesh_t* m, int64_t N, const void* rec4, void* bins, void* lists, void* mesh,
                const mipme_sr_job_t* job, void* host_flags, double* cpart) {
  const int dtype = dtype_of<T>();
  const BrickGeom bg = make_brick_geom(m);
  const BinsView v = bins_view(m, N, dtype, bins);
  const LiveLists ll = live_view(m, N, lists, nullptr);
  const int stage_rows = spread_stage_rows(m->order, sizeof(T));
  const size_t lds = spread_lds_bytes(m->order, sizeof(T), stage_rows, false, true);
  LiveSpreadArgs<T> sa;
  sa.g = make_geom(m);
  sa.bg = bg;
  sa.scheme = m->scheme;
  sa.count = ll.count;
  sa.atoms = ll.atoms;
  sa.lcap = ll.lcap;
  sa.rec4 = (const AtomRecord<T>*)rec4;
  sa.mesh = (T*)mesh;
  sa.stage_rows = stage_rows;
  sa.n_atoms = N;
  sa.home_rec = ll.home_rec;
  sa.rec_now = ll.rec_now;
  sa.wts = (T*)v.wts;
  sa.host_flags = (int*)host_flags;
  MIPME_REQUIRE(job && sr_job_fusable(job) && (job->shift_format & kShiftFormatMask) == kShiftTable32 && !job->dist_out,
                "the live step needs a co-schedulable pair job with 4-byte entries");
  SRPot s;
  int rc = make_srpot(job->pot, s);
  if (rc) return rc;
  const FastRS cf = make_fast_rs(s);
  const int pfast = fast_rs_exponent(s);
  FusedRowsArgs<T> ra = make_fused_rows_args<T>(s, cf, job->n_atoms, job->row_ptr, job->entries_shift, job->entries, nullptr,
                                                job->positions, job->records, job->cell, job->charges, nullptr, 0,
                                                job->full_list ? 0 : 1, job->full_list, 0, job->out, job->force, nullptr, nullptr,
                                                job->shift_format);
  ra.epart = v.epart;
  ra.cpart = cpart;
  MIPME_REQUIRE(!cpart || rows_cell_supported<T>(pfast, job->shift_format, job->dist_out),
                "the cell sums of the pair kernel need 4-byte entries and 1/r or 1/r^6");
  const unsigned n_row_blocks = unsigned((job->n_atoms + kRowsPerSpreadBlock - 1) / kRowsPerSpreadBlock);
  const unsigned n_spread = unsigned(bg.nb);
  const unsigned pattern = brick_pattern(bg, n_spread, n_row_blocks, sizeof(T) == 4);
  const unsigned grid = live_home_blocks(N, bg.xcd) +
                        (bg.xcd ? cosched_grid(pad8(n_spread), pad8(n_row_blocks), pattern) : n_spread + n_row_blocks);
  note_cosched_kernel("live_spread_rows_kernel");
  if (cpart && pfast == 1)
    MIPME_DISPATCH_ORDER(m->order, (live_spread_rows_kernel<N, T, 1, true><<<grid, SPREAD_THREADS, lds, st>>>(sa, ra, n_spread, pattern)));
  else if (cpart) {
    MIPME_DISPATCH_ORDER(m->order, (live_spread_rows_kernel<N, T, 6, true><<<grid, SPREAD_THREADS, lds, st>>>(sa, ra, n_spread, pattern)));
  } else if (pfast == 1)
    MIPME_DISPATCH_ORDER(m->order, (live_spread_rows_kernel<N, T, 1><<<grid, SPREAD_THREADS, lds, st>>>(sa, ra, n_spread, pattern)));
  else
    MIPME_DISPATCH_ORDER(m->order, (live_spread_rows_kernel<N, T, 6><<<grid, SPREAD_THREADS, lds, st>>>(sa, ra, n_spread, pattern)));
  MIPME_LAUNCH_CHECK();
  return MIPME_OK;
}

template <typename T>
int live_gather(hipStream_t st, const mipme_mesh_t* m, int64_t N, const void* rec4, void* bins, void* lists, const void* mesh,
                const void* qsum, double self_c, double bg_c, void* out, void* field, const GatherTailHost* th, void* nan_flag) {
  const int dtype = dtype_of<T>();
  const Geom g = make_geom(m);
  const BrickGeom bg = make_brick_geom(m);
  const BinsView v = bins_view(m, N, dtype, bins);
  const LiveLists ll = live_view(m, N, lists, nullptr);
  MIPME_REQUIRE(th && th->force && th->grad_pos && th->energy && th->epart_k && out && qsum, "NULL buffer passed to the live gather");
  const GatherTail<T> tail =
      make_gather_tail<T>(*th, (const double*)th->epart_k + th->n_k, int(th->n_k), rec4, th->live_flags);
  if (th->slab) {
    MIPME_REQUIRE(tail.slab_mom, "the slab term of the live gather needs the moments");
    MIPME_DISPATCH_ORDER(m->order, (live_gather_tail_kernel<N, T, true><<<brick_grid(bg), GATHER_THREADS, 0, st>>>(
                                       g, bg, v.idx, ll.rec_now, (const T*)v.wts, (const AtomRecord<T>*)rec4, (const T*)mesh,
                                       (const T*)qsum, T(1.0 / m->volume), T(self_c), T(bg_c), (T*)out, (T*)field, tail,
                                       (int*)nan_flag)));
  } else {
    MIPME_DISPATCH_ORDER(m->order, (live_gather_tail_kernel<N, T><<<brick_grid(bg), GATHER_THREADS, 0, st>>>(
                                       g, bg, v.idx, ll.rec_now, (const T*)v.wts, (const AtomRecord<T>*)rec4, (const T*)mesh,
                                       (const T*)qsum, T(1.0 / m->volume), T(self_c), T(bg_c), (T*)out, (T*)field, tail,
                                       (int*)nan_flag)));
  }
  MIPME_LAUNCH_CHECK();
  return MIPME_OK;
}

template int live_rebin<float>(hipStream_t, const mipme_mesh_t*, int64_t, const void*, void*, void*, void*);
template int live_rebin<double>(hipStream_t, const mipme_mesh_t*, int64_t, const void*, void*, void*, void*);
template int live_spread<float>(hipStream_t, const mipme_mesh_t*, int64_t, const void*, void*, void*, void*, const mipme_sr_job_t*,
                                void*, double*);
template int live_spread<double>(hipStream_t, const mipme_mesh_t*, int64_t, const void*, void*, void*, void*, const mipme_sr_job_t*,
                                 void*, double*);
template int live_gather<float>(hipStream_t, const mipme_mesh_t*, int64_t, const void*, void*, void*, const void*, const void*,
                                double, double, void*, void*, const GatherTailHost*, void*);
template int live_gather<double>(hipStream_t, const mipme_mesh_t*, int64_t, const void*, void*, void*, const void*, const void*,
                                 double, double, void*, void*, const GatherTailHost*, void*);

}
```

torch-pme_amd/graphed.py:

```python

from __future__ import annotations

import ctypes as C

import numpy as np
import torch

from . import _lib, ops



def _refuse_spline(calculator, what: str):
    from .potentials import CombinedPotential, SplinePotential

    for cls in (SplinePotential, CombinedPotential):
        if isinstance(getattr(calculator, "potential", None), cls):
            raise TypeError(f"{what} runs the fused kernels, which do not serve a {cls.__name__}: call the calculator eagerly "
                            "-- `calculator(charges, cell, positions, neighbor_indices, neighbor_distances)`")


class _LiveStep:

    def __init__(self, calculator, charges, cell, positions, charge_gradient=False, cell_gradient=False, slab_axis=None):
        lib = self.lib = _lib.load()
        self.slab = 0 if slab_axis is None else int(slab_axis) + 1
        device, dtype = positions.device, positions.dtype
        N = positions.shape[0]
        self.device, self.dtype, self.n_atoms = device, dtype, N
        geom, G = calculator._kspace_setup(cell, dtype, device, speculate=False)
        self.geom, self.G = geom, G
        self.md = geom.desc(1)
        self.pot = calculator.potential._descriptor()
        self.dt = _lib.dtype_code(dtype)
        if charges.shape[1] != 1 or not lib.mipme_md_supported(C.byref(self.md), C.byref(self.pot), N, self.dt):
            raise NotImplementedError("outside the range of the live-bin step")
        self.plan = _lib.get_plan(device, dtype, geom.ns, 1, geom.plan_store)
        if not self.plan.xfused:
            raise NotImplementedError("the live-bin step needs a power-of-two mesh along x")
        self.rec = torch.empty((N, 4), dtype=dtype, device=device)
        self.rec[:, :3] = positions.detach()
        self.rec[:, 3] = charges.detach()[:, 0]
        cdtype = torch.complex64 if dtype == torch.float32 else torch.complex128
        self.cell = cell.detach().to(dtype).contiguous()
        self.rho = torch.empty(geom.ns, dtype=dtype, device=device)
        self.phi = torch.empty(geom.ns, dtype=dtype, device=device)
        self.hat = torch.empty((geom.n_half,), dtype=cdtype, device=device)
        self.dc = torch.empty((1,), dtype=dtype, device=device)
        self.bins = torch.empty((lib.mipme_atom_bins_bytes(C.byref(self.md), N, self.dt),), dtype=torch.uint8, device=device)
        self.lists = torch.zeros((lib.mipme_md_lists_ints(C.byref(self.md), N),), dtype=torch.int32, device=device)
        self.potentials = torch.empty((N,), dtype=dtype, device=device)
        self.pair_force = torch.empty((N, 3), dtype=dtype, device=device)
        self.energy = torch.empty((), dtype=dtype, device=device)
        self.grad = torch.empty((N, 3), dtype=dtype, device=device)
        self.minus_one = torch.tensor(-1.0, dtype=dtype, device=device)
        self.one = torch.tensor(1.0, dtype=dtype, device=device)
        self.grad_q = torch.empty((N, 1), dtype=dtype, device=device) if charge_gradient else None
        self.grad_cell = self.G_deriv = self.cell_work = None
        if cell_gradient:
            self.grad_cell = torch.empty((27,), dtype=dtype, device=device)
            self.G_deriv = ops.filter_derivative(geom, self.pot, dtype, device)
            self.cell_work = torch.empty((lib.mipme_cell_tail_work(self.plan.handle, C.byref(self.md), N),),
                                         dtype=torch.float64, device=device)
        self.flags = torch.zeros((1,), dtype=torch.int32).pin_memory()
        self.flags_np = self.flags.numpy()
        self.nan_flag = calculator._nan_flag_ptr()
        calculator._nan_shape = [1, *geom.ns]
        self.rows = None
        self.log = None

    def _args(self):
        row_ptr, words, fmt = self.rows if self.rows is not None else (self.lists, self.lists, 2)
        return _lib.MdArgs(
            plan=self.plan.handle, stream=_lib.current_stream(self.device), dtype=self.dt, shift_format=fmt,
            mesh=C.pointer(self.md), pot=C.pointer(self.pot), n_atoms=self.n_atoms, records=self.rec.data_ptr(),
            cell=self.cell.data_ptr(), G=self.G.data_ptr(), rho_mesh=self.rho.data_ptr(), hat_work=self.hat.data_ptr(),
            phi_mesh=self.phi.data_ptr(), dc=self.dc.data_ptr(), atom_bins=self.bins.data_ptr(),
            live_lists=self.lists.data_ptr(), row_ptr=row_ptr.data_ptr(), words=words.data_ptr(),
            potentials=self.potentials.data_ptr(), pair_force=self.pair_force.data_ptr(), energy=self.energy.data_ptr(),
            grad_positions=self.grad.data_ptr(), grad_seed=self.minus_one.data_ptr(), nan_flag=self.nan_flag,
            host_flags=self.flags.data_ptr(), grad_charges=_lib.ptr(self.grad_q), grad_cell=_lib.ptr(self.grad_cell),
            G_deriv=_lib.ptr(self.G_deriv), cell_work=_lib.ptr(self.cell_work), aux_seed=self.one.data_ptr(),
            energy_log=None if self.log is None else self.log.values.data_ptr(),
            energy_log_cursor=None if self.log is None else self.log.cursor.data_ptr(),
            energy_log_capacity=0 if self.log is None else self.log.capacity, slab=self.slab)

    def rebin(self):
        with _lib.on_device(self.device):
            a = self._args()
            _lib.check(self.lib.mipme_md_rebin(C.byref(a)))

    def step(self):
        with _lib.on_device(self.device):
            a = self._args()
            _lib.check(self.lib.mipme_md_step(C.byref(a)))

    @property
    def max_displacement(self) -> float:
        inv = np.asarray(self.geom.inv_cell)
        return float(min(1.0 / (self.geom.ns[d] * np.linalg.norm(inv[:, d])) for d in range(3)))

    def moved(self) -> bool:
        f = int(self.flags_np[0])
        if f & 2:
            self.flags_np[0] = f & ~2
            return True
        return False

    def check(self):
        f = int(self.flags_np[0])
        if f:
            self.flags_np[0] = 0
            if f & 2:
                raise RuntimeError("GraphedEnergyForces: an atom has moved more than one mesh point since the last refresh(); "
                                   "the results of that step are invalid (its energy was returned as NaN) -- refresh the "
                                   "neighbour structures sooner, or call the object with check=True")
            raise RuntimeError("GraphedEnergyForces: a brick's atom list overflowed at the last refresh (very non-uniform "
                               "system); construct with live_bins=False")


class EnergyLog:

    def __init__(self, capacity: int, n_frames: int, device):
        if capacity < 1 or n_frames < 1:
            raise ValueError("an energy log needs capacity >= 1 and n_frames >= 1")
        self.capacity, self.n_frames = int(capacity), int(n_frames)
        self.values = torch.zeros((self.capacity, self.n_frames), dtype=torch.float64, device=device)
        self.cursor = torch.zeros((self.n_frames,), dtype=torch.int32, device=device)

    def push(self, energies: torch.Tensor) -> None:
        if energies.numel() != self.n_frames or not energies.is_contiguous():
            raise ValueError(f"the log holds {self.n_frames} energies per evaluation, got a tensor of {tuple(energies.shape)}")
        _lib.require_device(energies, "energies")
        with _lib.on_device(energies.device):
            _lib.check(_lib.load().mipme_energy_log_push(
                _lib.current_stream(energies.device), _lib.dtype_code(energies.dtype), self.n_frames, energies.data_ptr(),
                self.values.data_ptr(), self.cursor.data_ptr(), self.capacity))

    def reset(self) -> None:
        self.cursor.zero_()

    def count(self) -> int:
        return int(self.cursor[0].item())


def _as_energy_log(energy_log, n_frames, device):
    if energy_log is None or isinstance(energy_log, EnergyLog):
        if energy_log is not None and energy_log.n_frames != n_frames:
            raise ValueError(f"the energy log holds {energy_log.n_frames} energies per evaluation, the step produces {n_frames}")
        return energy_log
    return EnergyLog(int(energy_log), n_frames, device)


class GraphedEnergyForces:

    def __init__(self, calculator, charges, cell, positions, neighbor_indices=None, neighbor_shifts=None, warmup: int = 3,
                 cell_gradient: bool = False, store_distances: bool = False, neighbors=None,
                 periodic=(True, True, True), live_bins: bool | None = None, charge_gradient: bool = False,
                 energy_log=None, epilogue=None, slab_correction: bool = False):
        _refuse_spline(calculator, "GraphedEnergyForces" + (" (`neighbors=` included)" if neighbors is not None else ""))
        self.calc = calculator
        self._slab_axis = self._periodic = None
        if slab_correction:
            flags = [bool(p) for p in periodic]
            if len(flags) != 3 or sum(flags) != 2:
                raise ValueError(f"`slab_correction` needs exactly two periodic axes, got periodic={tuple(flags)}")
            desc = calculator.potential._descriptor()
            if not (desc.kind == _lib.COULOMB or desc.exponent == 1):
                raise ValueError("`slab_correction`: the slab term exists for 1/r only (CoulombPotential, or "
                                 "InversePowerLawPotential(exponent=1))")
            if calculator.potential.smearing is None:
                raise ValueError("`slab_correction` belongs to the mesh part: the potential needs a smearing")
            self._slab_axis = flags.index(False)
            self._periodic = torch.tensor(flags, dtype=torch.bool, device=positions.device)
        self.energy_log = _as_energy_log(energy_log, 1, positions.device)
        self._epilogue = epilogue
        self.store_distances = bool(store_distances)
        self.charge_gradient = bool(charge_gradient)
        self.stream = None
        if neighbors is not None:
            if neighbor_indices is not None or neighbor_shifts is not None:
                raise ValueError("give either `neighbors` or `neighbor_indices` / `neighbor_shifts`")
            if store_distances:
                raise ValueError("a device neighbour stream has no pair order to store distances in")
        elif neighbor_indices is None or neighbor_shifts is None:
            raise ValueError("`neighbor_indices` and `neighbor_shifts` (or `neighbors`) are required")
        self.q = charges.detach()
        self.cell_gradient = bool(cell_gradient)
        self.cell = cell.detach().clone() if cell_gradient else cell.detach()
        self.pos = positions.detach().clone().requires_grad_(True)
        device = positions.device
        self._minus_one = torch.tensor(-1.0, dtype=positions.dtype, device=device)
        self._one = torch.tensor(1.0, dtype=positions.dtype, device=device)
        self._fused_contract = True
        self.charge_grad = self.cell_grad = None
        self._warmup = max(1, warmup)
        self.refresh_graph = None
        self._live = None
        if neighbors is not None and live_bins is not False and hasattr(calculator, "_kspace_setup") \
                and calculator.potential.smearing is not None:
            try:
                live = _LiveStep(calculator, self.q, self.cell, self.pos, self.charge_gradient, self.cell_gradient,
                                 slab_axis=self._slab_axis)
                live.rebin()
                torch.cuda.current_stream(device).synchronize()
                live.check()
                self._live = live
                self.pos = live.rec[:, :3]
            except (NotImplementedError, RuntimeError):
                if live_bins:
                    raise
                self._live = None
        if neighbors is not None:
            from .neighbors import NeighborStream

            if isinstance(neighbors, NeighborStream) and self._live is not None:
                raise ValueError("with live bins the neighbour stream is built on the object's own records: pass the cutoff")
            if isinstance(neighbors, NeighborStream):
                if neighbors.n_atoms != self.pos.shape[0] or neighbors.dtype != self.pos.dtype:
                    raise ValueError("`neighbors` was built for other positions")
                self.stream = neighbors
                self.stream.positions = self.pos
                self.stream.update()
            else:
                self.stream = NeighborStream(self.pos, self.cell, float(neighbors), periodic=periodic)
            self.stream.check(synchronize=True)
            self._capture_refresh()
            self._capture(self.stream.indices, None)
        else:
            self._capture(neighbor_indices, neighbor_shifts)

    def _capture_refresh(self):
        device = self.pos.device
        side = torch.cuda.Stream(device)
        side.wait_stream(torch.cuda.current_stream(device))
        if self._live is not None:
            self._live.rows = (self.stream.row_ptr, self.stream.words, 2 | _lib.ROWS_PADDED)
        with torch.cuda.stream(side):
            self._refresh_eager()
        torch.cuda.current_stream(device).wait_stream(side)
        torch.cuda.synchronize(device)
        self.refresh_graph = torch.cuda.CUDAGraph()
        with torch.cuda.graph(self.refresh_graph):
            self._refresh_eager()

    def _refresh_eager(self):
        self.stream.update()
        if self._live is not None:
            self._live.rebin()

    def refresh(self, positions: torch.Tensor | None = None, check: bool = False) -> None:
        if self.stream is None:
            raise RuntimeError("refresh() needs the `neighbors=` form; use recapture() with a new list otherwise")
        self._deferred_check()
        if positions is not None:
            with torch.no_grad():
                self.pos.copy_(positions)
        self.refresh_graph.replay()
        if check:
            torch.cuda.current_stream(self.pos.device).synchronize()
            self._deferred_check(recover=True)

    def _deferred_check(self, recover: bool = False):
        if self._live is not None:
            self._live.check()
        st = self.stream
        if st is None or not int(st._host_np[1]):
            return
        if recover and int(st._host_np[1]) == 1:
            st.grow()
            st.check(synchronize=True)
            self._capture_refresh()
            self._capture(st.indices, None)
            return
        st.check()

    def recapture(self, neighbor_indices, neighbor_shifts, positions: torch.Tensor | None = None) -> None:
        if positions is not None:
            with torch.no_grad():
                self.pos.copy_(positions)
        self._capture(neighbor_indices, neighbor_shifts)

    def _capture_live(self):
        device = self.pos.device
        side = torch.cuda.Stream(device)
        side.wait_stream(torch.cuda.current_stream(device))
        self._live.log = None
        with torch.cuda.stream(side):
            for _ in range(self._warmup):
                self._live.step()
        torch.cuda.current_stream(device).wait_stream(side)
        torch.cuda.synchronize(device)
        self._keepalive = [self._live, self.stream, getattr(self.calc, "_cache", None)]
        self._live.log = self.energy_log
        self.graph = torch.cuda.CUDAGraph()
        with torch.cuda.graph(self.graph):
            self._live.step()
            self.energy = self._live.energy
            if self._epilogue is not None:
                self._epilogue(self)
        self.energy, self.forces, self.distances = self._live.energy, self._live.grad, None
        self.charge_grad = self._live.grad_q
        self.cell_grad = None if self._live.grad_cell is None else self._live.grad_cell[18:27].view(3, 3)
        self.pairs, self.shifts = self.stream.indices, None

    def _capture(self, neighbor_indices, neighbor_shifts):
        if self._live is not None:
            return self._capture_live()
        calculator, device, warmup = self.calc, self.pos.device, self._warmup
        self.pairs = neighbor_indices
        self.shifts = None if neighbor_shifts is None else neighbor_shifts.to(self.pos.dtype).contiguous()
        side = torch.cuda.Stream(device)
        side.wait_stream(torch.cuda.current_stream(device))
        with torch.cuda.stream(side):
            for it in range(max(1, warmup) + 1):
                self.pos.grad = self.cell.grad = self.q.grad = None
                self._eval()
                if it == 0 and (self.charge_gradient or self.cell_gradient) and self._fused_contract:
                    t = self._tail
                    ok = t is not None and (t["grad_q"] is not None or not self.charge_gradient) and (
                        t["grad_cell"] is not None or not self.cell_gradient)
                    if not ok:
                        self._fused_contract = False
                        if self.charge_gradient:
                            self.q = self.q.clone().requires_grad_(True)
                        if self.cell_gradient:
                            self.cell.requires_grad_(True)
        torch.cuda.current_stream(device).wait_stream(side)
        torch.cuda.synchronize(device)
        self.pos.grad = self.cell.grad = self.q.grad = None
        topo = ops.get_topology(self.pairs, self.pos.shape[0]) if ops.PAIR_MODE == "rows" else None
        self._keepalive = [
            topo,
            getattr(calculator, "_cache", None),
            ops._dot_scratch(device, self.q.data_ptr()),
        ]
        if isinstance(topo, ops.PairTopology):
            self._keepalive += [topo.row_ptr, topo.entries, topo._ent32, topo._ent_sh, topo._packed, topo._pair_sh]
        elif topo is not None:
            self._keepalive += [self.stream.row_ptr, self.stream.words]
        self.graph = torch.cuda.CUDAGraph()
        with torch.cuda.graph(self.graph):
            self.energy = self._eval(log=self.energy_log)
            self.forces = self.pos.grad
            if self.energy_log is not None and not (self._tail is not None and self._tail.get("logged")):
                self.energy_log.push(self.energy.reshape(1))
            if self._epilogue is not None:
                self._epilogue(self)
            if self._fused_contract:
                t = self._tail
                self._keepalive.append(t)
                self.charge_grad = t["grad_q"] if self.charge_gradient else None
                self.cell_grad = t["grad_cell"][18:27].view(3, 3) if self.cell_gradient else None
            else:
                self.charge_grad = -self.q.grad if self.charge_gradient else None
                self.cell_grad = -self.cell.grad if self.cell_gradient else None

    def _eval(self, log=None):
        if self.stream is not None:
            d = self.stream.distances(self.pos, self.cell)
        else:
            d = ops.pair_distances(self.pos, self.pairs, self.cell, self.shifts,
                                   deferred=True if self.store_distances else "virtual")
        self.distances = d.detach() if self.store_distances else None
        fused = self._fused_contract
        with ops.seed_promise(self._minus_one, charges=fused and self.charge_gradient, cell=fused and self.cell_gradient,
                              aux_seed=self._one, energy_log=log):
            if self._periodic is None:
                V = self.calc(self.q, self.cell, self.pos, self.pairs, d)
            else:
                V = self.calc(self.q, self.cell, self.pos, self.pairs, d, periodic=self._periodic)
        self._tail = getattr(V.grad_fn, "tail", None)
        E = ops.weighted_sum(V, self.q)
        E.backward(self._minus_one)
        return E.detach()

    @property
    def max_displacement(self):
        return None if self._live is None else self._live.max_displacement

    def set_charges(self, charges: torch.Tensor) -> None:
        with torch.no_grad():
            if self._live is not None:
                self._live.rec[:, 3] = charges.detach()[:, 0]
            self.q.copy_(charges.detach())

    def __call__(self, positions: torch.Tensor | None = None, check: bool = False):
        self._deferred_check()
        self.calc.check()
        if positions is not None:
            with torch.no_grad():
                self.pos.copy_(positions)
        self.graph.replay()
        if check and self._live is not None:
            torch.cuda.current_stream(self.pos.device).synchronize()
            if self._live.moved():
                self.refresh(check=True)
                self.graph.replay()
                torch.cuda.current_stream(self.pos.device).synchronize()
                self._deferred_check()
        out = (self.energy, self.forces)
        if self.charge_gradient:
            out += (self.charge_grad,)
        if self.cell_gradient:
            out += (self.cell_grad,)
        return out


class _FramesFunction(torch.autograd.Function):

    @staticmethod
    def forward(ctx, batch, *positions):
        batch._launch_forward()
        ctx.batch = batch
        return batch.energies.detach()

    @staticmethod
    @torch.autograd.function.once_differentiable
    def backward(ctx, g):
        batch = ctx.batch
        if g.data_ptr() != batch._minus_one.data_ptr():
            batch._launch_backward(g.contiguous())
        return (None, *(b.detach() for b in batch._grad_pos))


class GraphedFrameBatch:

    def __init__(self, calculator, frames, warmup: int = 2, store_distances: bool = False, energy_log=None, epilogue=None,
                 charge_gradient: bool = False, cell_gradient: bool = False, periodic=None, slab_correction: bool = False):
        _refuse_spline(calculator, "GraphedFrameBatch")
        frames = list(frames)
        slab = self._slab_codes(calculator, len(frames), periodic, slab_correction)
        lib = _lib.load()
        self.calc = calculator
        self.store_distances = bool(store_distances)
        self.charge_gradient, self.cell_gradient = bool(charge_gradient), bool(cell_gradient)
        if self.cell_gradient and self.store_distances:
            raise ValueError("GraphedFrameBatch: `cell_gradient` and `store_distances` exclude each other (the pair kernels "
                             "that form the cell sums keep the distances in registers)")
        F = self.n_frames = len(frames)
        if F == 0:
            raise ValueError("no frames")
        q0, _, p0, _, _ = frames[0]
        device, dtype = p0.device, p0.dtype
        _lib.require_device(p0, "positions")
        self.device, self.dtype = device, dtype
        dt = self._dt = _lib.dtype_code(dtype)
        self._pot = calculator.potential._descriptor()
        full = bool(calculator.full_neighbor_list)
        self.pos, self._keep, geoms, Gs = [], [], [], []
        for q, cell, pos, pairs, shifts in frames:
            if q.shape[1] != 1:
                raise ValueError("the frames path handles a single charge channel")
            geom, G = calculator._kspace_setup(cell, dtype, device, speculate=False)
            geoms.append(geom)
            Gs.append(G.reshape(-1))
        ns = geoms[0].ns
        if any(g.ns != ns for g in geoms):
            raise ValueError(f"all frames must give the same mesh, got {[g.ns for g in geoms]}")
        self.ns = ns
        M, Mh = geoms[0].n_mesh, geoms[0].n_half
        cdtype = torch.complex64 if dtype == torch.float32 else torch.complex128
        self._G = torch.stack(Gs).contiguous()
        self._rho = torch.empty((F,) + ns, dtype=dtype, device=device)
        self._phi = torch.empty((F,) + ns, dtype=dtype, device=device)
        self._hat = torch.empty((F, Mh), dtype=cdtype, device=device)
        self._dc = torch.empty((F,), dtype=dtype, device=device)
        self.energies = torch.empty((F,), dtype=dtype, device=device)
        self._plan = _lib.FFTPlan(device, dtype, ns, F)
        self._frames = (_lib.Frame * F)()
        self._minus_one = torch.full((F,), -1.0, dtype=dtype, device=device)
        self._grad_pos, self.distances = [], []
        compact_ok, ent_streams = True, []
        for k, (q, cell, pos, pairs, shifts) in enumerate(frames):
            N, P = pos.shape[0], pairs.shape[0]
            p = pos.detach().clone().contiguous().requires_grad_(True)
            qc = q.detach().reshape(-1).contiguous()
            cl = cell.detach().to(dtype).contiguous()
            sh = shifts.to(dtype).contiguous()
            topo = ops.get_topology(pairs, N)
            ent_sh, fmt = topo.entries_with_shifts(sh, shifts, table=True)
            if ent_sh is None or fmt != 1:
                raise ValueError(f"frame {k}: cell shifts must be integers in [-3, 3] for the frames path")
            ent32 = topo.compact_entries(sh, shifts)
            compact_ok = compact_ok and ent32 is not None
            ent_streams.append((ent_sh, ent32))
            md = geoms[k].desc(1)
            nbytes = lib.mipme_atom_bins_bytes(C.byref(md), N, dt)
            if nbytes <= 0:
                raise ValueError(f"frame {k}: mesh {ns} is outside the brick kernels' range")
            nb = ((ns[0] + 7) // 8) * ((ns[1] + 7) // 8) * ((ns[2] + 7) // 8)
            buf = dict(
                bins=torch.empty((nbytes,), dtype=torch.uint8, device=device),
                counters=torch.zeros((max(nb + 1, int(lib.mipme_frames_counter_ints(C.byref(md), N, dt))),), dtype=torch.int32,
                                     device=device),
                records=torch.empty((N, 4), dtype=dtype, device=device),
                out=torch.empty((N,), dtype=dtype, device=device),
                force=torch.empty((N, 3), dtype=dtype, device=device),
                field=torch.empty((N, 3), dtype=dtype, device=device),
                grad=torch.empty((N, 3), dtype=dtype, device=device),
                dist=(torch.empty((P,), dtype=dtype, device=device)
                      if self.store_distances and topo.sorted_by_first and P > 0 else None),
            )
            f = self._frames[k]
            f.n_atoms, f.positions, f.charges, f.cell, f.mesh = N, p.data_ptr(), qc.data_ptr(), cl.data_ptr(), md
            f.atom_bins, f.brick_counters = buf["bins"].data_ptr(), buf["counters"].data_ptr()
            f.counter_ints = int(buf["counters"].numel())
            f.row_ptr, f.entries_shift, f.entries = topo.row_ptr.data_ptr(), ent_sh.data_ptr(), topo.entries.data_ptr()
            f.full_list, f.shift_format = int(full), int(fmt)
            f.records = buf["records"].data_ptr()
            f.rho_mesh, f.phi_mesh, f.dc = self._rho[k].data_ptr(), self._phi[k].data_ptr(), self._dc[k:].data_ptr()
            f.out, f.force, f.field = buf["out"].data_ptr(), buf["force"].data_ptr(), buf["field"].data_ptr()
            f.dist_out = _lib.ptr(buf["dist"])
            f.energy, f.grad_positions = self.energies[k:].data_ptr(), buf["grad"].data_ptr()
            f.use_tail, f.grad_seed = 1, self._minus_one[k:].data_ptr()
            self.pos.append(p)
            self._grad_pos.append(buf["grad"])
            self.distances.append(buf["dist"])
            self._keep.append((qc, cl, sh, topo, ent_sh, ent32, buf, pairs))
        if compact_ok:
            for k, (_, ent32) in enumerate(ent_streams):
                self._frames[k].entries_shift, self._frames[k].shift_format = ent32.data_ptr(), 2
        elif self.cell_gradient:
            bad = [k for k, (_, ent32) in enumerate(ent_streams) if ent32 is None]
            raise ValueError(f"GraphedFrameBatch: `cell_gradient` needs 4-byte pair entries in every frame; the cell shifts or "
                             f"the atom count of frame(s) {bad} do not fit them")
        nbytes = lib.mipme_frames_table_bytes(dt, F)
        host = np.zeros((nbytes,), dtype=np.uint8)
        _lib.check(lib.mipme_frames_table_build(dt, F, self._frames, C.byref(self._pot), host.ctypes.data, nbytes))
        self.charge_grads = self.cell_grads = self._cell_work = None
        if self.charge_gradient or self.cell_gradient:
            self._one = torch.ones((1,), dtype=dtype, device=device)
            ptrs = lambda tensors: (C.c_void_p * F)(*(t.data_ptr() for t in tensors))
            gq = gc = None
            G_deriv, G_deriv_stride, work_stride = None, 0, 0
            if self.charge_gradient:
                self.charge_grads = [torch.empty((f.n_atoms, 1), dtype=dtype, device=device) for f in self._frames]
                gq = ptrs(self.charge_grads)
            if self.cell_gradient:
                self._grad_cell = torch.empty((F, 27), dtype=dtype, device=device)
                self.cell_grads = self._grad_cell[:, 18:27].view(F, 3, 3)
                self._G_deriv = torch.stack([ops.filter_derivative(g, self._pot, dtype, device).reshape(-1) for g in geoms]).contiguous()
                G_deriv, G_deriv_stride = self._G_deriv.data_ptr(), self._G_deriv.shape[1]
                work_stride = max(int(lib.mipme_frames_cell_work(C.byref(f.mesh), f.n_atoms)) for f in self._frames)
                self._cell_work = torch.empty((F * work_stride,), dtype=torch.float64, device=device)
                gc = ptrs(self._grad_cell)
            _lib.check(lib.mipme_frames_table_contract(
                dt, F, self._frames, C.byref(self._pot), host.ctypes.data, nbytes, gq, gc, G_deriv, G_deriv_stride,
                _lib.ptr(self._cell_work), work_stride, self._one.data_ptr()))
        self.slab_axes = None if slab is None else [c - 1 if c else None for c in slab]
        self._slab = self._slab_work = None
        if slab is not None:
            self._slab = (C.c_int32 * F)(*slab)
            self._slab_stride = int(lib.mipme_frames_slab_work())
            self._slab_work = torch.zeros((F * self._slab_stride,), dtype=torch.float64, device=device)
            _lib.check(lib.mipme_frames_table_slab(dt, F, self._frames, C.byref(self._pot), host.ctypes.data, nbytes, self._slab,
                                                   self._slab_work.data_ptr(), self._slab_stride))
        self.energy_log = _as_energy_log(energy_log, F, device)
        if self.energy_log is not None:
            _lib.check(lib.mipme_frames_table_energy_log(dt, F, host.ctypes.data, nbytes, self.energy_log.values.data_ptr(),
                                                         self.energy_log.cursor.data_ptr(), self.energy_log.capacity))
        self._table = torch.from_numpy(host).to(device)
        side = torch.cuda.Stream(device)
        side.wait_stream(torch.cuda.current_stream(device))
        with torch.cuda.stream(side):
            for _ in range(max(1, warmup)):
                self._eval()
        torch.cuda.current_stream(device).wait_stream(side)
        torch.cuda.synchronize(device)
        if self.energy_log is not None:
            self.energy_log.reset()
        self.graph = torch.cuda.CUDAGraph()
        with torch.cuda.graph(self.graph):
            self._eval()
            if epilogue is not None:
                epilogue(self)
        self.forces = [p.grad for p in self.pos]

    @staticmethod
    def _slab_codes(calculator, n_frames, periodic, slab_correction):
        if not slab_correction:
            if periodic is not None:
                raise ValueError("GraphedFrameBatch: `periodic` only selects the frames and axes of `slab_correction=True` (the batch "
                                 "takes explicit pair lists, there is no neighbour list for it to shape)")
            return None
        if periodic is None:
            raise ValueError("GraphedFrameBatch: `slab_correction` needs `periodic`: one triple of booleans for every frame, or one "
                             "per frame")
        per = list(periodic)
        if len(per) == 3 and all(isinstance(p, (bool, int, np.bool_)) or (torch.is_tensor(p) and p.ndim == 0) for p in per):
            per = [per] * n_frames
        if len(per) != n_frames:
            raise ValueError(f"GraphedFrameBatch: `periodic` must be one triple or one triple per frame ({n_frames}), got {len(per)}")
        codes = []
        for k, triple in enumerate(per):
            flags = [bool(p) for p in triple]
            if len(flags) != 3 or sum(flags) < 2:
                raise ValueError(f"frame {k}: `slab_correction` needs exactly two periodic axes (or three: a fully periodic frame), "
                                 f"got periodic={tuple(flags)}")
            codes.append(0 if all(flags) else flags.index(False) + 1)
        desc = calculator.potential._descriptor()
        if not (desc.kind == _lib.COULOMB or desc.exponent == 1):
            raise ValueError("`slab_correction`: the slab term exists for 1/r only (CoulombPotential, or "
                             "InversePowerLawPotential(exponent=1))")
        if calculator.potential.smearing is None:
            raise ValueError("`slab_correction` belongs to the mesh part: the potential needs a smearing")
        return codes if any(codes) else None

    def _launch_forward(self):
        if self._slab is not None or self.charge_gradient or self.cell_gradient:
            with _lib.on_device(self.device):
                a = _lib.FramesStepArgs(
                    plan=self._plan.handle, stream=_lib.current_stream(self.device), dtype=self._dt, n_frames=self.n_frames,
                    frames=self._frames, pot=C.pointer(self._pot), device_table=self._table.data_ptr(), G=self._G.data_ptr(),
                    G_stride=self._G.shape[1], rho_mesh_all=self._rho.data_ptr(), hat_work_all=self._hat.data_ptr(),
                    phi_mesh_all=self._phi.data_ptr(), dc_all=self._dc.data_ptr(), cell_work=_lib.ptr(self._cell_work),
                    cell_gradient=int(self.cell_gradient))
                if self._slab is not None:
                    s = _lib.FramesSlabStepArgs(step=a, slab=self._slab, slab_work=self._slab_work.data_ptr(),
                                                slab_work_stride=self._slab_stride)
                    _lib.check(_lib.load().mipme_frames_slab_step(C.byref(s)))
                else:
                    _lib.check(_lib.load().mipme_frames_step(C.byref(a)))
            return
        with _lib.on_device(self.device):
            _lib.check(_lib.load().mipme_frames_forward(
                self._plan.handle, _lib.current_stream(self.device), self._dt, self.n_frames, self._frames,
                C.byref(self._pot), self._table.data_ptr(), self._G.data_ptr(), self._G.shape[1], self._rho.data_ptr(),
                self._hat.data_ptr(), self._phi.data_ptr(), self._dc.data_ptr()))

    def _launch_backward(self, g):
        with _lib.on_device(self.device):
            _lib.check(_lib.load().mipme_frames_backward(
                _lib.current_stream(self.device), self._dt, self.n_frames, self._frames, self._table.data_ptr(),
                g.data_ptr()))

    def _eval(self):
        for p in self.pos:
            p.grad = None
        E = _FramesFunction.apply(self, *self.pos)
        E.backward(self._minus_one)
        return E

    def __call__(self, positions=None):
        if positions is not None:
            with torch.no_grad():
                for buf, new in zip(self.pos, positions):
                    buf.copy_(new)
        self.calc.check()
        self.graph.replay()
        out = (self.energies, self.forces)
        if self.charge_gradient:
            out += (self.charge_grads,)
        if self.cell_gradient:
            out += (self.cell_grads,)
        return out


def _combined_refusal(pot) -> str | None:
    from .potentials import CombinedPotential, CoulombPotential, InversePowerLawPotential, SplinePotential

    members = list(pot.potentials)
    if len(members) > _lib.COMBINED_MAX_TERMS:
        return f"it has {len(members)} members, the kernels take at most {_lib.COMBINED_MAX_TERMS}"
    for k, m in enumerate(members):
        if isinstance(m, CombinedPotential):
            return f"member {k} is itself a CombinedPotential (nested combinations are not served)"
        if isinstance(m, SplinePotential):
            return f"member {k} is a SplinePotential; the kernels know CoulombPotential and InversePowerLawPotential members"
        if type(m) not in (CoulombPotential, InversePowerLawPotential):
            return (f"member {k} is a {type(m).__name__}; the kernels know exactly CoulombPotential and "
                    "InversePowerLawPotential members")
        if m.exclusion_radius is not None:
            return f"member {k} has an exclusion radius"
    if any(m.smearing is None for m in members):
        return "its members are direct potentials (`smearing=None`): the step is the range-separated mesh calculation"
    return None


class GraphedCombinedStep:

    def __init__(self, calculator, charges, cell, positions, neighbor_indices, neighbor_shifts, weight_gradient: bool = True,
                 charge_gradient: bool = False, warmup: int = 3):
        from . import analytic, combined
        from .potentials import CombinedPotential

        pot = getattr(calculator, "potential", None)
# ... 118 lines not shown
```

Measured before the change: 597.6 million.

## Add live plane-spread path fusing spread with forward yz FFT in live-bin mode

```diff
diff --git a/torch-pme_amd/csrc/api.hip b/torch-pme_amd/csrc/api.hip
--- a/torch-pme_amd/csrc/api.hip
+++ b/torch-pme_amd/csrc/api.hip
@@ -898,8 +898,23 @@
   if (a.energy_log && (rc = tail_attach_energy_log(tail, a.energy_log, a.energy_log_cursor, a.energy_log_capacity,
                                                    "energy_log needs energy_log_cursor")))
     return rc;
+  PlaneHost ph;
+  bool planes = false;
+  if (fft_plan_plane_forward_ok(a.plan)) {
+    ph.hat = a.hat_work;
+    ph.keep_mesh = false;
+    ph.slot_values = true;
+    if (a.grad_cell || !live_planes_run(m, a.n_atoms, a.dtype, &job, &ph, a.host_flags)) ph.hat = nullptr;
+    ph.parts = ph.hat ? plane_spread_parts_setting() : 1;
+    if (ph.parts > 1) {
+      ph.hat_more = fft_plan_hat_parts(a.plan, st, kPlanePartsMax - 1);
+      ph.more_stride = int64_t(m->nx) * m->ny * (m->nz / 2 + 1);
+      if (!ph.hat_more) ph.parts = 1;
+    }
+  }
   STAGE(st, "spread+rspace_forward", live_spread<T>(st, m, a.n_atoms, a.records, a.atom_bins, a.live_lists, a.rho_mesh, &job, a.host_flags,
-                                                     a.grad_cell ? cw.cwave : nullptr));
+                                                     a.grad_cell ? cw.cwave : nullptr, &ph, &planes));
+  fft_plan_set_forward_done(a.plan, planes, planes ? ph.parts_used : 1);
   int64_t n_sr_part = 0;
   const void* sr_part = bins_epart(m, a.n_atoms, a.dtype, a.atom_bins, &n_sr_part);
   const ConvCell cc{a.G_deriv, cw.cwave, cw.n_waves, cw.wbuf, cw.rows, int(cw.n_riders), nullptr, nullptr, nullptr, nullptr};
diff --git a/torch-pme_amd/csrc/bricks_device.h b/torch-pme_amd/csrc/bricks_device.h
--- a/torch-pme_amd/csrc/bricks_device.h
+++ b/torch-pme_amd/csrc/bricks_device.h
@@ -1110,6 +1110,39 @@
   return int(cap);
 }
 
+static constexpr int kLiveMargin = 1;
+template <int N, bool DERIV, typename T>
+__device__ __forceinline__ void live_axis(int scheme, T x, T (&w)[N], T (&dw)[N]) {
+  if constexpr (N <= 2) {
+    weights_1d<MIPME_P3M, N, DERIV, T>(x, w, dw);
+  } else if constexpr (N >= 6) {
+    weights_1d<MIPME_LAGRANGE, N, DERIV, T>(x, w, dw);
+  } else {
+    if (scheme == MIPME_P3M)
+      weights_1d<MIPME_P3M, N, DERIV, T>(x, w, dw);
+    else
+      weights_1d<MIPME_LAGRANGE, N, DERIV, T>(x, w, dw);
+  }
+}
+template <int N, typename T>
+__device__ __forceinline__ void live_coords(const Geom& g, const AtomRecord<T>& r, int& mx, int& my, int& mz, T& x0, T& x1, T& x2) {
+  const double rx = double(r.x), ry = double(r.y), rz = double(r.z);
+  const double ux = double(g.nx) * (rx * g.inv[0] + ry * g.inv[3] + rz * g.inv[6]);
+  const double uy = double(g.ny) * (rx * g.inv[1] + ry * g.inv[4] + rz * g.inv[7]);
+  const double uz = double(g.nz) * (rx * g.inv[2] + ry * g.inv[5] + rz * g.inv[8]);
+  int m;
+  double x;
+  split_runtime(ux, (N % 2) == 0, m, x);
+  mx = posmod(m, g.nx);
+  x0 = T(x);
+  split_runtime(uy, (N % 2) == 0, m, x);
+  my = posmod(m, g.ny);
+  x1 = T(x);
+  split_runtime(uz, (N % 2) == 0, m, x);
+  mz = posmod(m, g.nz);
+  x2 = T(x);
+}
+
 template <int N, typename T>
 struct PlaneItem {
   T vx;
@@ -1201,9 +1234,21 @@
   }
 }
 
-template <int SCHEME, int N, typename T, bool BANDED = false>
-__device__ __forceinline__ void plane_spread_yz_body(const SpreadArgs<T>& args, const PlaneArgs<T>& pa, unsigned item,
-                                                     char* smem) {
+template <typename T>
+struct LivePlaneArgs {
+  Geom g;
+  BinIndex bins;
+  bool from_live = false;
+  T scale = T(1);
+  int scheme = 0;
+  const AtomRecord<T>* rec4 = nullptr;
+  int n_atoms = 0;
+  double invn[9];
+};
+
+template <int SCHEME, int N, typename T, bool BANDED = false, bool LIVE = false, typename SA = SpreadArgs<T>>
+__device__ __forceinline__ void plane_spread_yz_body(const SA& args, const PlaneArgs<T>& pa, unsigned item, char* smem) {
+  static_assert(!(LIVE && BANDED), "live planes are whole planes");
   constexpr bool banded = BANDED;
   const int n_bands = banded ? pa.bands : 1;
   const unsigned unit = item / unsigned(pa.parts);
@@ -1224,9 +1269,10 @@
   const int spb = kPlaneSub / n_bands;
   const int SUBS = banded ? min(spb + 2, kPlaneSub) : kPlaneSub;
   const int sub0 = banded ? band * spb - 1 : 0;
-  const int NL = N * SUBS;
+  constexpr int XL = LIVE ? N + 2 * kLiveMargin : N, XM = LIVE ? kLiveMargin : 0;
+  const int NL = XL * SUBS;
   auto list_of = [&](int l) __attribute__((always_inline)) {
-    return posmod(x0 - s0 - l / SUBS, g.nx) * kPlaneSub + ((sub0 + (l % SUBS)) & (kPlaneSub - 1));
+    return posmod(x0 - s0 + XM - l / SUBS, g.nx) * kPlaneSub + ((sub0 + (l % SUBS)) & (kPlaneSub - 1));
   };
   int my_count = 0;
   if (tid < NL) my_count = bins.plive[list_of(tid)];
@@ -1235,12 +1281,12 @@
   for (int i = tid; i < npts; i += nthr) acc[i] = 0.0;
   const YzTile<T> yt = banded ? yz_tile_setup<T, false>(rows, g.nz, smem + pa.tile_off, smem + pa.tw_off)
                               : yz_tile_setup<T, true>(g.ny, g.nz, smem + pa.tile_off, smem + pa.tw_off);
-  if (args.from_live) {
+  if (!LIVE && args.from_live) {
     const int n_items = g.nx * n_bands * pa.parts;
     for (int b = int(item) + tid * n_items; b <= bins.nb; b += n_items * nthr) bins.snap[b] = bin_count_of(bins, b, true);
   }
   int* lst = reinterpret_cast<int*>(smem + pa.misc_off);
-  static_assert(N * kPlaneSub < 64, "bookkeeping of the plane lists");
+  static_assert(XL * kPlaneSub < 64, "bookkeeping of the plane lists");
   double* fxs = reinterpret_cast<double*>(lst + 128);
   float* wred = reinterpret_cast<float*>(lst + 132);
   if constexpr (sizeof(T) == 4) {
@@ -1296,7 +1342,7 @@
   const int total = lst[NL];
   const int lo = int(int64_t(total) * part / pa.parts), hi = int(int64_t(total) * (part + 1) / pa.parts);
   const int n_batches = (hi - lo + nthr - 1) / nthr;
-  constexpr bool FAT = plane_entry_fat<N, T>();
+  constexpr bool FAT = !LIVE && plane_entry_fat<N, T>();
   const int lane = tid & 63;
   const int lst_lane = lane <= NL ? lst[lane] : 0x7fffffff;
   auto entry_of = [&](int b, int& tt) __attribute__((always_inline)) -> int64_t {
@@ -1317,6 +1363,64 @@
     }
     return int64_t(list_of(l)) * bins.pcap + (gidx - first);
   };
+  if constexpr (LIVE) {
+    const int* __restrict__ alist = reinterpret_cast<const int*>(bins.plist);
+    const int* __restrict__ aover = reinterpret_cast<const int*>(bins.pover);
+    const unsigned last_atom = unsigned(args.n_atoms - 1);
+    auto index_of = [&](int b) __attribute__((always_inline)) -> int {
+      int unused_tt;
+      const int64_t e = entry_of(b, unused_tt);
+      return e >= 0 ? alist[e] : -1;
+    };
+    auto record_of = [&](int atom) __attribute__((always_inline)) -> AtomRecord<T> {
+      AtomRecord<T> r = args.rec4[min(unsigned(atom < 0 ? 0 : atom), last_atom)];
+      r.w = atom < 0 ? T(0) : r.w;
+      return r;
+    };
+    auto scatter_atom = [&](const AtomRecord<T>& r) __attribute__((always_inline)) {
+      const double rx = double(r.x), ry = double(r.y), rz = double(r.z);
+      int mx, my, mz;
+      double xd;
+      split_runtime(rx * args.invn[0] + ry * args.invn[3] + rz * args.invn[6], (N % 2) == 0, mx, xd);
+      const T x0f = T(xd);
+      split_runtime(rx * args.invn[1] + ry * args.invn[4] + rz * args.invn[7], (N % 2) == 0, my, xd);
+      const T x1f = T(xd);
+      split_runtime(rx * args.invn[2] + ry * args.invn[5] + rz * args.invn[8], (N % 2) == 0, mz, xd);
+      const T x2f = T(xd);
+      mx &= g.nx - 1;
+      my &= g.ny - 1;
+      mz &= g.nz - 1;
+      const int tt = (x0 - mx - s0) & (g.nx - 1);
+      if (r.w != T(0) && tt < N) {
+        PlaneItem<N, T> it;
+        T wx[N], unused[N];
+        live_axis<N, false, T>(args.scheme, x0f, wx, unused);
+        live_axis<N, false, T>(args.scheme, x1f, it.wy, unused);
+        live_axis<N, false, T>(args.scheme, x2f, it.wz, unused);
+        it.my = my;
+        it.mz = mz;
+        it.vx = r.w * pick<N, T>(wx, tt) * args.scale;
+        if (it.vx != T(0)) {
+          guard_item(it);
+          plane_item_scatter<N, T, false>(acc, g, it, fx_scale, row_lo, rows);
+        }
+      }
+    };
+    int i1 = index_of(0);
+    AtomRecord<T> r0 = record_of(i1);
+    i1 = index_of(1);
+    for (int b = 0; b < n_batches; ++b) {
+      const int i2 = index_of(b + 2);
+      const AtomRecord<T> r1 = record_of(i1);
+      scatter_atom(r0);
+      r0 = r1;
+      i1 = i2;
+    }
+    if (part == 0) {
+      const int oc = min(bins.plive[g.nx * kPlaneSub], args.n_atoms);
+      for (int i = tid; i < oc; i += nthr) scatter_atom(record_of(aover[i]));
+    }
+  } else {
   constexpr int DEPTH = FAT ? 1 : 2;
   int tt0 = 0, tt1 = 0;
   PlaneRaw<N, T> r0, r1;
@@ -1364,6 +1468,7 @@
         plane_item_scatter<N, T, BANDED>(acc, g, it, fx_scale, row_lo, rows);
       }
     }
+  }
   }
   __syncthreads();
   MIPME_WG_PHASE(2);
diff --git a/torch-pme_amd/csrc/host.h b/torch-pme_amd/csrc/host.h
--- a/torch-pme_amd/csrc/host.h
+++ b/torch-pme_amd/csrc/host.h
@@ -108,9 +108,10 @@
 
 bool live_supported(const mipme_mesh_t* m, int64_t N, int dtype);
 int64_t live_lists_ints(const mipme_mesh_t* m, int64_t N);
+bool live_planes_run(const mipme_mesh_t* m, int64_t N, int dtype, const mipme_sr_job_t* job, const PlaneHost* ph, const void* host_flags);
 template <typename T> int live_rebin(hipStream_t st, const mipme_mesh_t* m, int64_t N, const void* rec4, void* bins, void* lists, void* host_flags);
 template <typename T> int live_spread(hipStream_t st, const mipme_mesh_t* m, int64_t N, const void* rec4, void* bins, void* lists, void* mesh,
-                                      const mipme_sr_job_t* job, void* host_flags, double* cpart);
+                                      const mipme_sr_job_t* job, void* host_flags, double* cpart, const PlaneHost* ph, bool* used_planes);
 template <typename T> int live_gather(hipStream_t st, const mipme_mesh_t* m, int64_t N, const void* rec4, void* bins, void* lists, const void* mesh,
                                       const void* qsum, double self_c, double bg_c, void* out, void* field, const GatherTailHost* th, void* nan_flag);
 
diff --git a/torch-pme_amd/csrc/live.hip b/torch-pme_amd/csrc/live.hip
--- a/torch-pme_amd/csrc/live.hip
+++ b/torch-pme_amd/csrc/live.hip
@@ -1,8 +1,7 @@
 #include "bricks_device.h"
 
 namespace mipme {
-static constexpr int kLiveMargin = 1;
-enum LiveFlags { kLiveListOverflow = 1, kLiveMoved = 2 };
+enum LiveFlags { kLiveListOverflow = 1, kLiveMoved = 2, kLivePlaneOverflow = 4 };
 
 struct LiveLists {
   int* counters;
@@ -12,6 +11,12 @@
   int4* rec_now;
   int4* home_rec;
   int* host_flags;
+  int pcap;
+  int* pl_live;
+  int* pl_count;
+  int* pl_atoms;
+  int* pl_over;
+  float* wmax;
 };
 
 static inline int live_list_capacity(const mipme_mesh_t* m, int64_t N) {
@@ -26,10 +31,22 @@
   const BrickGeom bg = make_brick_geom(m);
   return int64_t(bg.nb) * bin_capacity(bg.nb, N) + N;
 }
+static inline int live_plane_capacity(const mipme_mesh_t* m, int64_t N) {
+  const bool pow2 = (m->ny & (m->ny - 1)) == 0 && (m->nz & (m->nz - 1)) == 0 && m->nz >= 4 && m->ny >= 2;
+  if (m->n_channels != 1 || N <= 0 || !pow2 || m->nx < 2 * BRICK || m->order < 3 || m->order > 5) return 0;
+  const int64_t lists = int64_t(m->nx) * kPlaneSub, mean = (N + lists - 1) / lists, all = (N + 15) / 16 * 16;
+  return int(std::min<int64_t>((4 * mean + 32 + 15) / 16 * 16, all));
+}
+static inline int64_t live_plane_ints(const mipme_mesh_t* m, int64_t N) {
+  const int pcap = live_plane_capacity(m, N);
+  if (pcap == 0) return 0;
+  const int64_t lists = int64_t(m->nx) * kPlaneSub;
+  return 2 * (lists + 1) + lists * pcap + N + (N + 63) / 64;
+}
 int64_t live_lists_ints(const mipme_mesh_t* m, int64_t N) {
   const BrickGeom bg = make_brick_geom(m);
   const int64_t head = ((8 + (bg.nb + 1) + bg.nb + int64_t(bg.nb) * live_list_capacity(m, N)) + 3) / 4 * 4;
-  return head + 4 * live_slots(m, N) + 4 * N;
+  return head + 4 * live_slots(m, N) + 4 * N + live_plane_ints(m, N);
 }
 static inline LiveLists live_view(const mipme_mesh_t* m, int64_t N, void* lists, void* host_flags) {
   const BrickGeom bg = make_brick_geom(m);
@@ -43,47 +60,33 @@
   l.rec_now = (int4*)(b + head);
   l.home_rec = l.rec_now + live_slots(m, N);
   l.host_flags = (int*)host_flags;
+  const int64_t n_pl = int64_t(m->nx) * kPlaneSub;
+  l.pcap = live_plane_capacity(m, N);
+  l.pl_live = (int*)(l.home_rec + N);
+  l.pl_count = l.pl_live + (n_pl + 1);
+  l.pl_atoms = l.pl_count + (n_pl + 1);
+  l.pl_over = l.pl_atoms + n_pl * l.pcap;
+  l.wmax = (float*)(l.pl_over + N);
   return l;
-}
-
-template <int N, bool DERIV, typename T>
-__device__ __forceinline__ void live_axis(int scheme, T x, T (&w)[N], T (&dw)[N]) {
-  if constexpr (N <= 2) {
-    weights_1d<MIPME_P3M, N, DERIV, T>(x, w, dw);
-  } else if constexpr (N >= 6) {
-    weights_1d<MIPME_LAGRANGE, N, DERIV, T>(x, w, dw);
-  } else {
-    if (scheme == MIPME_P3M)
-      weights_1d<MIPME_P3M, N, DERIV, T>(x, w, dw);
-    else
-      weights_1d<MIPME_LAGRANGE, N, DERIV, T>(x, w, dw);
-  }
-}
-template <int N, typename T>
-__device__ __forceinline__ void live_coords(const Geom& g, const AtomRecord<T>& r, int& mx, int& my, int& mz, T& x0, T& x1, T& x2) {
-  const double rx = double(r.x), ry = double(r.y), rz = double(r.z);
-  const double ux = double(g.nx) * (rx * g.inv[0] + ry * g.inv[3] + rz * g.inv[6]);
-  const double uy = double(g.ny) * (rx * g.inv[1] + ry * g.inv[4] + rz * g.inv[7]);
-  const double uz = double(g.nz) * (rx * g.inv[2] + ry * g.inv[5] + rz * g.inv[8]);
-  int m;
-  double x;
-  split_runtime(ux, (N % 2) == 0, m, x);
-  mx = posmod(m, g.nx);
-  x0 = T(x);
-  split_runtime(uy, (N % 2) == 0, m, x);
-  my = posmod(m, g.ny);
-  x1 = T(x);
-  split_runtime(uz, (N % 2) == 0, m, x);
-  mz = posmod(m, g.nz);
-  x2 = T(x);
 }
 
 template <typename T>
 __global__ __launch_bounds__(256) void live_bin_kernel(Geom g, BrickGeom bg, bool even, BinIndex bi, int* __restrict__ counters,
                                                       int64_t Natoms, const AtomRecord<T>* __restrict__ rec4,
                                                       int* __restrict__ over_brick, int4* __restrict__ rec,
-                                                      int4* __restrict__ home_rec) {
+                                                      int4* __restrict__ home_rec, LiveLists ll) {
   const int64_t i = int64_t(blockIdx.x) * blockDim.x + threadIdx.x;
+  if (ll.pcap > 0) {
+    const float q = i < Natoms ? float(rec4[i].w) : 0.f;
+    float a = fabsf(q);
+    a = fmaxf(a, dpp_mov<0xB1>(a));
+    a = fmaxf(a, dpp_mov<0x4E>(a));
+    a = fmaxf(a, dpp_mov<0x141>(a));
+    a = fmaxf(a, dpp_mov<0x140>(a));
+    a = fmaxf(fmaxf(read_lane(a, 0), read_lane(a, 16)), fmaxf(read_lane(a, 32), read_lane(a, 48)));
+    if (__builtin_amdgcn_ballot_w64(q != q) != 0) a = __builtin_nanf("");
+    if ((threadIdx.x & 63) == 0 && i < Natoms) ll.wmax[i >> 6] = a;
+  }
   if (i >= Natoms) return;
   const AtomRecord<T> r = rec4[i];
   const T p3[3] = {r.x, r.y, r.z};
@@ -119,11 +122,42 @@
   }
   rec[dst] = make_int4(m[0], m[1], m[2], int(i));
   home_rec[i] = make_int4(m[0], m[1], m[2], int(dst));
-}
-
-__global__ void live_snapshot_kernel(BinIndex bi, int* __restrict__ counters) {
+  if (ll.pcap > 0) {
+    const int list = m[0] * kPlaneSub + int((i >> 6) & (kPlaneSub - 1));
+    unsigned long long rem = __ballot(true);
+    int pl_leader = lane, pl_rank = 0, pl_count = 1;
+    while (rem) {
+      const int leader = __ffsll((long long)rem) - 1;
+      const int l0 = __shfl(list, leader, 64);
+      const unsigned long long peers = __ballot(list == l0) & rem;
+      if (list == l0) {
+        pl_leader = leader;
+        pl_rank = __popcll(peers & ((1ull << lane) - 1ull));
+        pl_count = __popcll(peers);
+      }
+      rem &= ~peers;
+    }
+    int pl_base = 0;
+    if (pl_leader == lane) pl_base = atomicAdd(&ll.pl_live[list], pl_count);
+    const int k = __shfl(pl_base, pl_leader, 64) + pl_rank;
+    if (k < ll.pcap)
+      ll.pl_atoms[int64_t(list) * ll.pcap + k] = int(i);
+    else
+      ll.pl_over[atomicAdd(&ll.pl_live[g.nx * kPlaneSub], 1)] = int(i);
+  }
+}
+
+__global__ void live_snapshot_kernel(BinIndex bi, int* __restrict__ counters, LiveLists ll, int n_plane) {
   const int b = blockIdx.x * blockDim.x + threadIdx.x;
-  if (b > bi.nb) return;
+  if (b > bi.nb) {
+    const int p = b - bi.nb - 1;
+    if (p >= n_plane) return;
+    const int c = ll.pl_live[p];
+    ll.pl_count[p] = p == n_plane - 1 ? c : min(c, ll.pcap);
+    ll.pl_live[p] = 0;
+    if (p == n_plane - 1 && c > 0 && ll.host_flags) atomicOr(ll.host_flags, kLivePlaneOverflow);
+    return;
+  }
   const int c = counters[b];
   bi.snap[b] = b == bi.nb ? c : min(c, bi.cap);
   counters[b] = 0;
@@ -218,10 +252,6 @@
   int mx, my, mz;
   T x0, x1, x2;
   live_coords<N, T>(g, r, mx, my, mz, x0, x1, x2);
-  T wx[N], wy[N], wz[N], dwx[N], dwy[N], dwz[N];
-  live_axis<N, true, T>(args.scheme, x0, wx, dwx);
-  live_axis<N, true, T>(args.scheme, x1, wy, dwy);
-  live_axis<N, true, T>(args.scheme, x2, wz, dwz);
   auto far = [](int now, int then, int n) {
     int d = now - then;
     d = d > n / 2 ? d - n : (d < -(n / 2) ? d + n : d);
@@ -230,6 +260,10 @@
   if ((far(mx, was.x, g.nx) || far(my, was.y, g.ny) || far(mz, was.z, g.nz)) && args.host_flags) atomicOr(args.host_flags, kLiveMoved);
   const int64_t slot = was.w;
   args.rec_now[slot] = make_int4(mx, my, mz, int(i));
+  T wx[N], wy[N], wz[N], dwx[N], dwy[N], dwz[N];
+  live_axis<N, true, T>(args.scheme, x0, wx, dwx);
+  live_axis<N, true, T>(args.scheme, x1, wy, dwy);
+  live_axis<N, true, T>(args.scheme, x2, wz, dwz);
   store_slot_weights<N, T>(args.wts + slot * wts_stride<N, T>(), wx, wy, wz, dwx, dwy, dwz);
 }
 
@@ -338,6 +372,18 @@
   const unsigned n = unsigned((n_atoms + SPREAD_THREADS - 1) / SPREAD_THREADS);
   return xcd ? (n + 7u) / 8u * 8u : n;
 }
+template <typename T, int PFAST, bool CELL>
+__device__ __forceinline__ void live_row_block(const FusedRowsArgs<T>& ra, unsigned r, char* smem_rows) {
+  AtomRecord<T>* tab = reinterpret_cast<AtomRecord<T>*>(smem_rows);
+  if constexpr (std::is_same<T, float>::value)
+    sr_rows_pk_body<PFAST, SPREAD_THREADS, CELL>(ra, r, tab);
+#if MIPME_ROW_LANES == 16
+  else if constexpr (PFAST == 1 || PFAST == 6)
+    sr_rows_f64_body<SPREAD_THREADS, CELL, PFAST>(ra, r, smem_rows);
+#endif
+  else if constexpr (!CELL)
+    sr_fused_rows_body<T, kPotForce, false, PFAST, false, true, SPREAD_THREADS, 0, true>(ra, r, tab);
+}
 template <int N, typename T, int PFAST, bool CELL = false>
 __global__ __launch_bounds__(SPREAD_THREADS, sizeof(T) == 4 ? (CELL ? MIPME_CELL_WAVES : 8) : 1) void live_spread_rows_kernel(LiveSpreadArgs<T> sa, FusedRowsArgs<T> ra,
                                                                                         unsigned n_spread, unsigned pattern) {
@@ -356,16 +402,27 @@
     const unsigned r = sa.bg.xcd ? xcd_contiguous(cs.slot, n_row_blocks) : cs.slot;
     if (r < n_row_blocks) {
       extern __shared__ __attribute__((aligned(16))) char smem_rows[];
-      AtomRecord<T>* tab = reinterpret_cast<AtomRecord<T>*>(smem_rows);
-      if constexpr (std::is_same<T, float>::value)
-        sr_rows_pk_body<PFAST, SPREAD_THREADS, CELL>(ra, r, tab);
-#if MIPME_ROW_LANES == 16
-      else if constexpr (PFAST == 1 || PFAST == 6)
-        sr_rows_f64_body<SPREAD_THREADS, CELL, PFAST>(ra, r, smem_rows);
-#endif
-      else if constexpr (!CELL)
-        sr_fused_rows_body<T, kPotForce, false, PFAST, false, true, SPREAD_THREADS, 0, true>(ra, r, tab);
-    }
+      live_row_block<T, PFAST, CELL>(ra, r, smem_rows);
+    }
+  }
+}
+
+template <int N, typename T, int PFAST>
+__global__ __launch_bounds__(SPREAD_THREADS, sizeof(T) == 4 ? 8 : 1) MIPME_SGPR_CAP void live_plane_rows_kernel(
+    LiveSpreadArgs<T> sa, LivePlaneArgs<T> la, PlaneArgs<T> pa, FusedRowsArgs<T> ra, unsigned n_planes, unsigned n_row_blocks) {
+  extern __shared__ __attribute__((aligned(16))) char smem_lp[];
+  const unsigned n_home = live_home_blocks(sa.n_atoms, true), n_pad = pad8(n_planes);
+  if (blockIdx.x < n_home) {
+    live_home_body<N, T>(sa, blockIdx.x);
+    return;
+  }
+  const unsigned b = blockIdx.x - n_home;
+  if (b < n_pad) {
+    const unsigned p = xcd_contiguous(b, n_planes);
+    if (p < n_planes) plane_spread_yz_body<MIPME_P3M, N, T, false, true>(la, pa, p, smem_lp);
+  } else {
+    const unsigned r = xcd_contiguous(b - n_pad, n_row_blocks);
+    if (r < n_row_blocks) live_row_block<T, PFAST, false>(ra, r, smem_lp);
   }
 }
 
@@ -548,19 +605,29 @@
   BinsView v = bins_view(m, N, dtype, bins);
   const LiveLists ll = live_view(m, N, lists, host_flags);
   live_bin_kernel<T><<<unsigned((N + 255) / 256), 256, 0, st>>>(g, bg, (m->order % 2) == 0, v.idx, ll.counters, N,
-                                                              (const AtomRecord<T>*)rec4, v.over_brick, v.rec, ll.home_rec);
+                                                              (const AtomRecord<T>*)rec4, v.over_brick, v.rec, ll.home_rec, ll);
   MIPME_LAUNCH_CHECK();
-  live_snapshot_kernel<<<unsigned((bg.nb + 1 + 255) / 256), 256, 0, st>>>(v.idx, ll.counters);
+  const int n_plane = ll.pcap > 0 ? m->nx * kPlaneSub + 1 : 0;
+  live_snapshot_kernel<<<unsigned((bg.nb + 1 + n_plane + 255) / 256), 256, 0, st>>>(v.idx, ll.counters, ll, n_plane);
   MIPME_LAUNCH_CHECK();
   MIPME_DISPATCH_ORDER(m->order, (live_lists_kernel<N><<<brick_grid(bg), SPREAD_THREADS, 0, st>>>(g, bg, v.idx, v.rec, ll)));
   MIPME_LAUNCH_CHECK();
   return MIPME_OK;
 }
 
+bool live_planes_run(const mipme_mesh_t* m, int64_t N, int dtype, const mipme_sr_job_t* job, const PlaneHost* ph,
+                     const void* host_flags) {
+  static const bool planes_env = env_flag("MIPME_LIVE_PLANES", true);
+  if (!planes_env || !host_flags || live_plane_capacity(m, N) == 0 || (m->nx & (m->nx - 1)) != 0) return false;
+  if ((*(const volatile int*)host_flags & kLivePlaneOverflow) != 0) return false;
+  return plane_spread_runs(m, N, dtype, job, ph, true) && plane_fits_cosched(m, dtype);
+}
+
 template <typename T>
 int live_spread(hipStream_t st, const mipme_mesh_t* m, int64_t N, const void* rec4, void* bins, void* lists, void* mesh,
-                const mipme_sr_job_t* job, void* host_flags, double* cpart) {
+                const mipme_sr_job_t* job, void* host_flags, double* cpart, const PlaneHost* ph, bool* used_planes) {
   const int dtype = dtype_of<T>();
+  if (used_planes) *used_planes = false;
   const BrickGeom bg = make_brick_geom(m);
   const BinsView v = bins_view(m, N, dtype, bins);
   const LiveLists ll = live_view(m, N, lists, nullptr);
@@ -597,6 +664,53 @@
   MIPME_REQUIRE(!cpart || rows_cell_supported<T>(pfast, job->shift_format, job->dist_out),
                 "the cell sums of the pair kernel need 4-byte entries and 1/r or 1/r^6");
   const unsigned n_row_blocks = unsigned((job->n_atoms + kRowsPerSpreadBlock - 1) / kRowsPerSpreadBlock);
+  if (used_planes && !cpart && live_planes_run(m, N, dtype, job, ph, host_flags)) {
+    LivePlaneArgs<T> la;
+    la.g = sa.g;
+    la.bins = v.idx;
+    la.bins.plive = ll.pl_count;
+    la.bins.plist = ll.pl_atoms;
+    la.bins.pover = ll.pl_over;
+    la.bins.pcap = ll.pcap;
+    la.bins.wmax = ll.wmax;
+    la.bins.n_wmax = int((N + 63) / 64);
+    la.scheme = m->scheme;
+    la.rec4 = (const AtomRecord<T>*)rec4;
+    la.n_atoms = int(N);
+    for (int k = 0; k < 9; ++k) la.invn[k] = double(k % 3 == 0 ? m->nx : (k % 3 == 1 ? m->ny : m->nz)) * sa.g.inv[k];
+    PlaneArgs<T> pa;
+    size_t need = 0;
+    plane_lds_layout<T>(m->ny, m->nz, pa, need, true);
+    pa.hat = (Cplx<T>*)ph->hat;
+    pa.parts = (ph->parts > 1 && ph->hat_more) ? ph->parts : 1;
+    pa.hat_more = (Cplx<T>*)ph->hat_more;
+    pa.more_stride = ph->more_stride;
+    while ((1 << pa.logny) < m->ny) ++pa.logny;
+    while ((1 << pa.loglz) < m->nz / 2) ++pa.loglz;
+    ph->parts_used = pa.parts;
+    ph->ycols_pending = false;
+    const size_t plane_lds = std::max(need, sizeof(T) * size_t(SPREAD_WAVES) * BRICK_PTS);
+    const unsigned n_planes = unsigned(m->nx) * unsigned(pa.parts);
+    const unsigned pgrid = live_home_blocks(N, true) + pad8(n_planes) + pad8(n_row_blocks);
+#define MIPME_LIVE_PLANES(PF)                                                                                                   \
+  do {                                                                                                                          \
+    switch (m->order) {                                                                                                         \
+      case 3: live_plane_rows_kernel<3, T, PF><<<pgrid, SPREAD_THREADS, plane_lds, st>>>(sa, la, pa, ra, n_planes, n_row_blocks); break; \
+      case 4: live_plane_rows_kernel<4, T, PF><<<pgrid, SPREAD_THREADS, plane_lds, st>>>(sa, la, pa, ra, n_planes, n_row_blocks); break; \
+      case 5: live_plane_rows_kernel<5, T, PF><<<pgrid, SPREAD_THREADS, plane_lds, st>>>(sa, la, pa, ra, n_planes, n_row_blocks); break; \
+      default: set_error("no live plane kernel for interpolation order %d", int(m->order)); return MIPME_EINVAL;               \
+    }                                                                                                                           \
+  } while (0)
+    note_cosched_kernel("live_plane_rows_kernel");
+    if (pfast == 1)
+      MIPME_LIVE_PLANES(1);
+    else
+      MIPME_LIVE_PLANES(6);
+#undef MIPME_LIVE_PLANES
+    MIPME_LAUNCH_CHECK();
+    *used_planes = true;
+    return MIPME_OK;
+  }
   const unsigned n_spread = unsigned(bg.nb);
   const unsigned pattern = brick_pattern(bg, n_spread, n_row_blocks, sizeof(T) == 4);
   const unsigned grid = live_home_blocks(N, bg.xcd) +
@@ -644,9 +758,9 @@
 template int live_rebin<float>(hipStream_t, const mipme_mesh_t*, int64_t, const void*, void*, void*, void*);
 template int live_rebin<double>(hipStream_t, const mipme_mesh_t*, int64_t, const void*, void*, void*, void*);
 template int live_spread<float>(hipStream_t, const mipme_mesh_t*, int64_t, const void*, void*, void*, void*, const mipme_sr_job_t*,
-                                void*, double*);
+                                void*, double*, const PlaneHost*, bool*);
 template int live_spread<double>(hipStream_t, const mipme_mesh_t*, int64_t, const void*, void*, void*, void*, const mipme_sr_job_t*,
-                                 void*, double*);
+                                 void*, double*, const PlaneHost*, bool*);
 template int live_gather<float>(hipStream_t, const mipme_mesh_t*, int64_t, const void*, void*, void*, const void*, const void*,
                                 double, double, void*, void*, const GatherTailHost*, void*);
 template int live_gather<double>(hipStream_t, const mipme_mesh_t*, int64_t, const void*, void*, void*, const void*, const void*,
diff --git a/torch-pme_amd/graphed.py b/torch-pme_amd/graphed.py
--- a/torch-pme_amd/graphed.py
+++ b/torch-pme_amd/graphed.py
@@ -65,6 +65,7 @@
         self.flags_np = self.flags.numpy()
         self.nan_flag = calculator._nan_flag_ptr()
         calculator._nan_shape = [1, *geom.ns]
+        self.planes_off = self.recapture = False
         self.rows = None
         self.log = None
 
@@ -108,8 +109,10 @@
 
     def check(self):
         f = int(self.flags_np[0])
-        if f:
-            self.flags_np[0] = 0
+        if f & 4 and not self.planes_off:
+            self.planes_off = self.recapture = True
+        if f & 3:
+            self.flags_np[0] = f & 4
             if f & 2:
                 raise RuntimeError("GraphedEnergyForces: an atom has moved more than one mesh point since the last refresh(); "
                                    "the results of that step are invalid (its energy was returned as NaN) -- refresh the "
@@ -263,6 +266,10 @@
     def _deferred_check(self, recover: bool = False):
         if self._live is not None:
             self._live.check()
+            if self._live.recapture:
+                self._live.recapture = False
+                if getattr(self, "graph", None) is not None:
+                    self._capture_live()
         st = self.stream
         if st is None or not int(st._host_np[1]):
             return
@@ -382,6 +389,7 @@
         with torch.no_grad():
             if self._live is not None:
                 self._live.rec[:, 3] = charges.detach()[:, 0]
+                self._live.rebin()
             self.q.copy_(charges.detach())
 
     def __call__(self, positions: torch.Tensor | None = None, check: bool = False):
```

Result: no change. 600.1 million, median of 6 (+0.4%).
